# jmackey-astro/PION

Hardware: AMD Instinct MI355X
Metric: Mcell-updates/s on 3D ideal-MHD 512³ uniform grid; achieved HBM GB/s vs peak (higher is better)
Workload: dtype f64; 1 GPU; M1: 3-D GLM-MHD (nvar 9) Stone blast wave 512^3, HLLD + FKJ98 eta 0.1, periodic, OA2/OA2; nvar=9, decomposition=z-slab x1, transport=none; time loop and transport issued from C++ (libpion_host), fp_mode=fast (FMA contraction)

## Files before the change

include/pion_gpu.h:

```cpp
#ifndef PION_GPU_H
#define PION_GPU_H

#ifdef __cplusplus
extern "C" {
#endif

#define PION_MAX_NVAR 16
#define PION_MAX_DIM 3

#define PION_EQEUL 1
#define PION_EQMHD 2
#define PION_EQGLM 3

#define PION_FLUX_LF 0
#define PION_FLUX_RSlinear 1
#define PION_FLUX_RSexact 2
#define PION_FLUX_RShybrid 3
#define PION_FLUX_RSroe 4
#define PION_FLUX_RSroe_pv 5
#define PION_FLUX_FVS 6
#define PION_FLUX_RS_HLLD 7
#define PION_FLUX_RS_HLL 8

#define PION_AV_NONE 0
#define PION_AV_FKJ98_1D 1
#define PION_AV_HCORRECTION 3
#define PION_AV_HCORR_FKJ98 4

#define PION_BC_PERIODIC 1
#define PION_BC_OUTFLOW 2
#define PION_BC_INFLOW 3
#define PION_BC_REFLECTING 4
#define PION_BC_FIXED 5
#define PION_BC_ONEWAY_OUT 6
#define PION_BC_DMACH 7
#define PION_BC_DMACH2 8
#define PION_BC_STWIND 9
#define PION_BC_SLAB 10
#define PION_BC_JET 11
#define PION_BC_JETREFLECT 13
#define PION_BC_AXISYMMETRIC 12

#define PION_COOL_NONE 0
#define PION_COOL_WSS09_CIE_LINE_HEAT_COOL 8

#define PION_CELL_ISGD 1
#define PION_CELL_ISBD 2
#define PION_CELL_ISDOMAIN 4
#define PION_CELL_TIMESTEP 8
#define PION_CELL_ISLEAF 16

#define PION_GPU_OK 0
#define PION_GPU_EINVAL (-1)
#define PION_GPU_EDEVICE (-2)
#define PION_GPU_EPHYSICS (-3)
#define PION_GPU_ENOMEM (-4)

typedef struct pion_gpu_config {
  int ndim;
  int nvar;
  int ntracer;
  int eqntype;
  int solver;
  int artvisc;
  int sp_ooa;
  int tm_ooa;
  int coord_sys;
  int nbc;
  int ng[PION_MAX_DIM];
  double xmin[PION_MAX_DIM];
  double dx;
  double gamma;
  double cfl;
  double etav;
  double min_temp;
  double max_temp;
  double refvec[PION_MAX_NVAR];
  int bc_type[6];
  int bc_dmach2;
  int cooling;
  int mp_timestep_limit;
  int strict_fp;
} pion_gpu_config;


int pion_gpu_create(const pion_gpu_config *cfg, int device, void **handle);
void pion_gpu_destroy(void *handle);
int pion_gpu_last_error(void *handle, char *buf, int len);

long pion_gpu_ncell_all(void *handle);
int pion_gpu_ng_all(void *handle, int axis);


int pion_gpu_upload(void *handle, const double *P_soa);
int pion_gpu_download(void *handle, int which, double *P_soa);
int pion_gpu_bind_device_state(void *handle, void *dP, void *dPh);
void *pion_gpu_device_ptr(void *handle, int which);
int pion_gpu_set_stream(void *handle, void *stream);
int pion_gpu_set_comm_stream(void *handle, void *stream);
void *pion_gpu_get_stream(void *handle, int which);
int pion_gpu_synchronize(void *handle);

int pion_gpu_set_wind_cells(void *handle, long n, const long *idx, const double *states);

#define PION_MAX_WIND_SOURCES 8
typedef struct pion_gpu_wind_source {
  double pos[PION_MAX_DIM];
  double radius;
  int type;
  double mdot;
  double vinf, vrot;
  double Tw, Rstar, Bstar;
  double tracers[PION_MAX_NVAR];
  int npt;
  const double *evo_time, *evo_Teff, *evo_Mdot, *evo_vrot, *evo_vinf, *evo_R;
  const double *evo_X[7];
  int evo_tracer_elem[PION_MAX_NVAR];
  double t_now;
  double update_freq;
  double orbit_ecc_fac;
  double orbit_periastron[2];
  double orbit_period;
} pion_gpu_wind_source;

int pion_gpu_add_wind_source(void *handle, const pion_gpu_wind_source *src, int *id);
int pion_gpu_get_wind_source_pos(void *handle, int id, double *pos);
int pion_gpu_get_flags(void *handle, unsigned char *out);
int pion_gpu_wind_orbit_position(const pion_gpu_wind_source *src, int ndim, double simtime, double *pos);
int pion_gpu_add_rotating_wind_source(void *handle, const pion_gpu_wind_source *src, const double *evo_vcrit,
                                      double xi, int *id);
int pion_gpu_wind_angle_tables(double xi, double *theta, double *omega, double *Teff, double *delta, double *alpha);
int pion_gpu_get_wind_cells(void *handle, int id, long *n, long *idx, double *states);

int pion_gpu_set_jet(void *handle, int jetradius, const double *jetstate);

int pion_gpu_set_cooling_tables(void *handle, int nT, const double *T,
                                const double *tabs, const double *slopes);


int pion_gpu_update_bcs(void *handle, double simtime, int cstep, int maxstep, int assign);

int pion_gpu_calc_dt(void *handle, double *t_dyn, double *t_mp);
int pion_gpu_calc_dt_device(void *handle, void **dptr);
int pion_gpu_read_dt(void *handle, double *t_dyn, double *t_mp);
int pion_gpu_dt_request(void *handle);
int pion_gpu_dt_wait(void *handle, double *t_dyn, double *t_mp);

int pion_gpu_set_glm_speeds(void *handle, double dt, double dx, double cr);

int pion_gpu_stage(void *handle, double dt_stage, int space_ooa, int is_full_step);

#define PION_STAGE_WHOLE 0
#define PION_STAGE_INTERIOR 1
#define PION_STAGE_ZBOUNDARY 2
int pion_gpu_stage_part(void *handle, double dt_stage, int space_ooa, int is_full_step, int part);

int pion_gpu_advance_time(void *handle, double dt, double simtime);


long pion_gpu_halo_count(void *handle);
typedef struct {
  double *send_lo, *send_hi, *recv_lo, *recv_hi;
  long count_per_var, var_stride;
  int nvar;
} pion_gpu_halo_spans_t;
int pion_gpu_halo_spans(void *handle, int which, pion_gpu_halo_spans_t *out);
int pion_gpu_halo_begin(void *handle);
int pion_gpu_halo_end(void *handle);
int pion_gpu_pack_halo(void *handle, int which, int face, void *dbuf);
int pion_gpu_unpack_halo(void *handle, int which, int face, void *dbuf);


int pion_gpu_interface_flux(void *handle, int n, int axis, double dt, const double *Pl,
                            const double *Pr, const double *aux, double *F, double *Pstar);

int pion_gpu_cooling_update(void *handle, int n, double dt, const double *P_in, double *P_out);
int pion_gpu_cooling_edot(void *handle, int n, const double *rho, const double *T, double *edot);
int pion_gpu_cooling_timescale(void *handle, int n, const double *P_in, double *t_cool);

int pion_gpu_enable_timing(void *handle, int on);
int pion_gpu_get_timing(void *handle, double *out, int n);

#ifdef __cplusplus
}
#endif
#endif
```

pion_amd/csrc/kernels.h:

```cpp
#ifndef PION_KERNELS_H
#define PION_KERNELS_H

#include <hip/hip_runtime.h>
#include <stdint.h>

#include "dev_riemann.h"
#include "rows_tiling.h"

namespace pion {

#define PION_MAX_NTR 2
#define PION_COOL_NT_MAX 256

struct GridDesc {
  int ndim;
  int ng[3], nbc[3], nga[3];
  long ncell;
  long sy, sz;
  double dx;
  double xmin[3];
  int cyl;
  const double *sph_vol;
};

struct CoolDev {
  int NT;
  const double *T;
  const double *tab;
  const double *slope;
  double inv_Mu2, inv_Mu2_elec_H, Mu_tot_over_kB;
  double MinT_allowed, MaxT_allowed;
  float lg0, inv_dlg;
};

struct StageArgs {
  GridDesc g;
  const double *S;
  const double *Pc;
  double *out;
  const uint8_t *flags;
  const uint8_t *hllflag;
  const double *eta;
  int *errword;
  FluxCtx fc;
  int eqntype, ntracer, solver;
  int space_ooa;
  int cooling;
  double dt;
  double glm_damp;
  double max_temp;
  int use_march;
  int xwrap;
  int zslope_lds;
  double *dE;
  int zchunk;
  int nzb, zcmax;
  int rows;
  int rows_auto;
  int ncu;
  int kz0, kz1;
  int kz2, kz3;
  unsigned long long *dtres;
  double cfl;
  int dt_mp;
  int plain_cells;
  CoolDev cool;
};

struct PrepassArgs {
  GridDesc g;
  const double *S;
  uint8_t *hllflag;
  double *divv, *gradp;
  double *eta;
  int eqntype, nvar, space_ooa;
  double gamma;
  long c0, c1;
  long c2, c3;
};

struct DtArgs {
  GridDesc g;
  const double *P;
  const double *Ph;
  const uint8_t *flags;
  unsigned long long *result;
  int *errword;
  int eqntype, nvar;
  double gamma, cfl;
  int do_mp;
  CoolDev cool;
};

struct FluxTestArgs {
  int n, axis, eqntype, ntracer, solver;
  const double *Pl, *Pr, *aux;
  double *F, *Pstar;
  int *errword;
  FluxCtx fc;
};

struct CoolTestArgs {
  int n, nvar;
  double dt, gamma;
  const double *Pin;
  double *Pout;
  const double *rho, *T;
  double *edot;
  int *errword;
  CoolDev cool;
};

#define PION_DECLARE_FP(NS)                                        \
  namespace NS {                                                   \
  int launch_stage(const StageArgs &a, hipStream_t s);             \
  int launch_cooling_dE(const StageArgs &a, hipStream_t s);        \
  int launch_prepass(const PrepassArgs &a, hipStream_t s);         \
  int launch_dt(const DtArgs &a, hipStream_t s);                   \
  int launch_dt_mp(const DtArgs &a, hipStream_t s);                \
  int launch_flux_test(const FluxTestArgs &a, hipStream_t s);      \
  int launch_cool_update(const CoolTestArgs &a, hipStream_t s);    \
  int launch_cool_edot(const CoolTestArgs &a, hipStream_t s);      \
  int launch_cool_timescale(const CoolTestArgs &a, hipStream_t s); \
  const char *stage_kernel_name(int eq, int ntr, int solver);      \
  }

PION_DECLARE_FP(fp_strict)
PION_DECLARE_FP(fp_fast)

}
#endif
```

pion_amd/csrc/kernels_fp.hip:

```cpp
#include "dev_cooling.h"
#include "kernels.h"

#ifndef PION_FPNS
#error "PION_FPNS must be defined (fp_strict or fp_fast)"
#endif
#ifndef PION_EQSEL
#define PION_EQSEL 0
#endif

namespace pion {
namespace PION_FPNS {

template <bool MHD>
PDEV int rotvar(const int ax, const int s)
{
  if (s >= 2 && s <= 4) {
    int k = (s - 2) + ax;
    return 2 + (k >= 3 ? k - 3 : k);
  }
  if (MHD && s >= 5 && s <= 7) {
    int k = (s - 5) + ax;
    return 5 + (k >= 3 ? k - 3 : k);
  }
  return s;
// ... 510 lines not shown
#ifdef PION_FAST_MATH
    const double ro = a.Pc[qRO * nc + c], pg = a.Pc[qPG * nc + c];
    const double pnew = Cooling::time_update(cool, ro, pg, a.dt, g, err);
    dE = (pnew - pg) / (g - 1.0);
#else
    double P0[NV], pn[NV], ui[NV], uf[NV];
#pragma unroll
    for (int v = 0; v < NV; v++) pn[v] = P0[v] = a.Pc[v * nc + c];
    pn[qPG] = Cooling::time_update(cool, P0[qRO], P0[qPG], a.dt, g, err);
    E::PtoU(P0, ui, g);
    E::PtoU(pn, uf, g);
    dE = uf[uERG] - ui[uERG];
#endif
    if (err) atomicOr(a.errword, err);
  }
  a.dE[c] = dE;
}
template <int EQ, int NTR>
static int cooling_go(const StageArgs &a, hipStream_t s)
{
  const unsigned gx = (a.g.ng[0] + 63) / 64, gy = (a.g.ng[1] + 3) / 4;
  const unsigned np = (unsigned)(a.kz1 - a.kz0) + ((a.kz3 > a.kz2) ? (unsigned)(a.kz3 - a.kz2) : 0u);
  const unsigned ntile = gx * gy * np;
  hipLaunchKernelGGL((k_cooling_dE<EQ, NTR>), dim3(((ntile + 7) / 8) * 8), dim3(256), 0, s, a);
  return (int)hipGetLastError();
}

template <int EQ, int NTR, int SOLVER>
static int stage_go(const StageArgs &a, hipStream_t s)
{
  if (a.use_march != 0 && ((a.g.ndim == 3 && a.g.nbc[2] >= 2) || (a.g.ndim == 2 && a.g.cyl != 2 && a.g.nbc[1] >= 2)))
    return stage_rows2_go<EQ, NTR, SOLVER>(a, s);
  const int nbx = (a.g.ng[0] + 63) / 64, nby = (a.g.ng[1] + 3) / 4;
  const long ntiles = (long)nbx * nby * a.g.ng[2];
  const long nblocks = ((ntiles + 7) / 8) * 8;
  hipLaunchKernelGGL((k_stage<EQ, NTR, SOLVER>), dim3((unsigned)nblocks), dim3(256), 0, s, a);
  return (int)hipGetLastError();
}
template <int EQ, int NTR, int SOLVER>
static int flux_go(const FluxTestArgs &a, hipStream_t s)
{
  hipLaunchKernelGGL((k_flux_test<EQ, NTR, SOLVER>), dim3((a.n + 255) / 256), dim3(256), 0, s, a);
  return (int)hipGetLastError();
}

#define PION_SOLVER_CASES_HD(FN, EQ, NTR, A, S)          \
  switch (A.solver) {                                    \
    case 0: return FN<EQ, NTR, 0>(A, S);                 \
    case 1: return FN<EQ, NTR, 1>(A, S);                 \
    case 2: return FN<EQ, NTR, 2>(A, S);                 \
    case 3: return FN<EQ, NTR, 3>(A, S);                 \
    case 4: return FN<EQ, NTR, 4>(A, S);                 \
    case 5: return FN<EQ, NTR, 5>(A, S);                 \
    case 6: return FN<EQ, NTR, 6>(A, S);                 \
    case 8: return FN<EQ, NTR, 8>(A, S);                 \
    default: return -1;                                  \
  }
#define PION_SOLVER_CASES_MHD(FN, EQ, NTR, A, S)         \
  switch (A.solver) {                                    \
    case 0: return FN<EQ, NTR, 0>(A, S);                 \
    case 1: return FN<EQ, NTR, 1>(A, S);                 \
    case 4: return FN<EQ, NTR, 4>(A, S);                 \
    case 7: return FN<EQ, NTR, 7>(A, S);                 \
    case 8: return FN<EQ, NTR, 8>(A, S);                 \
    default: return -1;                                  \
  }

#if PION_EQSEL == 1
#define PION_EQ EQEUL
#define PION_CASES PION_SOLVER_CASES_HD
#define PION_SUFFIX hd
#elif PION_EQSEL == 2
#define PION_EQ EQMHD
#define PION_CASES PION_SOLVER_CASES_MHD
#define PION_SUFFIX mhd
#else
#define PION_EQ EQGLM
#define PION_CASES PION_SOLVER_CASES_MHD
#define PION_SUFFIX glm
#endif
#define PION_CAT2(a, b) a##b
#define PION_CAT(a, b) PION_CAT2(a, b)

#ifdef PION_PROBE
int PION_CAT(launch_stage_, PION_SUFFIX)(const StageArgs &a, hipStream_t s)
{
  return stage_rows2_go<PION_EQ, 0, (PION_EQSEL == 1 ? 4 : 7)>(a, s);
}
#else
int PION_CAT(launch_stage_, PION_SUFFIX)(const StageArgs &a, hipStream_t s)
{
  switch (a.ntracer) {
    case 0: PION_CASES(stage_go, PION_EQ, 0, a, s)
    case 1: PION_CASES(stage_go, PION_EQ, 1, a, s)
    case 2: PION_CASES(stage_go, PION_EQ, 2, a, s)
    default: return -1;
  }
}
int PION_CAT(launch_cooling_dE_, PION_SUFFIX)(const StageArgs &a, hipStream_t s)
{
  switch (a.ntracer) {
    case 0: return cooling_go<PION_EQ, 0>(a, s);
    case 1: return cooling_go<PION_EQ, 1>(a, s);
    case 2: return cooling_go<PION_EQ, 2>(a, s);
    default: return -1;
  }
}
int PION_CAT(launch_flux_test_, PION_SUFFIX)(const FluxTestArgs &a, hipStream_t s)
{
  switch (a.ntracer) {
    case 0: PION_CASES(flux_go, PION_EQ, 0, a, s)
    case 1: PION_CASES(flux_go, PION_EQ, 1, a, s)
    case 2: PION_CASES(flux_go, PION_EQ, 2, a, s)
    default: return -1;
  }
}
#endif

#else

int launch_stage_hd(const StageArgs &a, hipStream_t s);
int launch_stage_mhd(const StageArgs &a, hipStream_t s);
int launch_stage_glm(const StageArgs &a, hipStream_t s);
int launch_cooling_dE_hd(const StageArgs &a, hipStream_t s);
int launch_cooling_dE_mhd(const StageArgs &a, hipStream_t s);
int launch_cooling_dE_glm(const StageArgs &a, hipStream_t s);
int launch_flux_test_hd(const FluxTestArgs &a, hipStream_t s);
int launch_flux_test_mhd(const FluxTestArgs &a, hipStream_t s);
int launch_flux_test_glm(const FluxTestArgs &a, hipStream_t s);

int launch_stage(const StageArgs &a, hipStream_t s)
{
  if (a.eqntype == EQEUL) return launch_stage_hd(a, s);
  if (a.eqntype == EQMHD) return launch_stage_mhd(a, s);
  if (a.eqntype == EQGLM) return launch_stage_glm(a, s);
  return -1;
}
int launch_cooling_dE(const StageArgs &a, hipStream_t s)
{
  if (a.eqntype == EQEUL) return launch_cooling_dE_hd(a, s);
  if (a.eqntype == EQMHD) return launch_cooling_dE_mhd(a, s);
  if (a.eqntype == EQGLM) return launch_cooling_dE_glm(a, s);
  return -1;
}
int launch_flux_test(const FluxTestArgs &a, hipStream_t s)
{
  if (a.eqntype == EQEUL) return launch_flux_test_hd(a, s);
  if (a.eqntype == EQMHD) return launch_flux_test_mhd(a, s);
  if (a.eqntype == EQGLM) return launch_flux_test_glm(a, s);
  return -1;
}
const char *stage_kernel_name(int, int, int) { return "k_stage"; }

__global__ __launch_bounds__(256) void k_prepass_hlld(const PrepassArgs a)
{
  const long nc = a.g.ncell;
  const unsigned gx = (a.g.nga[0] + 63) / 64, gy = (a.g.nga[1] + 3) / 4;
  const long plane = (long)a.g.nga[0] * a.g.nga[1];
  const unsigned npl1 = (unsigned)((a.c1 - a.c0) / plane);
  const unsigned npl = npl1 + ((a.c3 > a.c2) ? (unsigned)((a.c3 - a.c2) / plane) : 0u);
  const unsigned ntile = gx * gy * npl;
  const unsigned t = (unsigned)xcd_tile(blockIdx.x, ntile);
  if (t >= ntile) return;
  int i[3];
  i[0] = (int)((t % gx) * 64 + (threadIdx.x & 63));
  i[1] = (int)(((t / gx) % gy) * 4 + (threadIdx.x >> 6));
  const unsigned pz = t / (gx * gy);
  i[2] = (pz < npl1) ? (int)(a.c0 / plane) + (int)pz : (int)(a.c2 / plane) + (int)(pz - npl1);
  if (i[0] >= a.g.nga[0] || i[1] >= a.g.nga[1]) return;
  const long c = (long)i[0] + a.g.sy * i[1] + a.g.sz * i[2];
  const double dx = a.g.dx;
  double divv = 0.0, gradp = 0.0;
  double pp3[3], pn3[3];
  bool steep = (a.gradp != nullptr);
  for (int v = 0; v < a.g.ndim; v++) {
    const long st = (v == 0) ? 1 : ((v == 1) ? a.g.sy : a.g.sz);
    const long n = (i[v] > 0) ? c - st : c;
    const long p = (i[v] < a.g.nga[v] - 1) ? c + st : c;
    pp3[v] = a.S[1 * nc + p];
    pn3[v] = a.S[1 * nc + n];
    if (!(fabs(pp3[v] - pn3[v]) <= 1.6 * fmin(pp3[v], pn3[v]))) steep = true;
  }
  if (steep) {
    for (int v = 0; v < a.g.ndim; v++) gradp += fabs(pp3[v] - pn3[v]) / fmin(pp3[v], pn3[v]);
  }
  if (gradp > 5. || a.divv) {
    for (int v = 0; v < a.g.ndim; v++) {
      const long st = (v == 0) ? 1 : ((v == 1) ? a.g.sy : a.g.sz);
      const long n = (i[v] > 0) ? c - st : c;
      const long p = (i[v] < a.g.nga[v] - 1) ? c + st : c;
      const double ddx = (n == c || p == c) ? dx : 2.0 * dx;
      if (a.g.cyl == 1 && v == 1) {
        const double rn = cyl_Rcom(cyl_R(a.g, (n == c) ? i[1] : i[1] - 1), dx);
        const double rp = cyl_Rcom(cyl_R(a.g, (p == c) ? i[1] : i[1] + 1), dx);
        divv += 2.0 * (rp * a.S[(2 + v) * nc + p] - rn * a.S[(2 + v) * nc + n]) / (rp * rp - rn * rn);
      }
      else divv += (a.S[(2 + v) * nc + p] - a.S[(2 + v) * nc + n]) / ddx;
    }
  }
  if (a.divv) a.divv[c] = divv;
  if (a.gradp) a.gradp[c] = gradp;
  a.hllflag[c] = (divv < 0. && gradp > 5.) ? 1 : 0;
}

#define PION_PREPASS_ZC 16
__global__ __launch_bounds__(256) void k_prepass_hlld_march(const PrepassArgs a)
{
  const long nc = a.g.ncell;
  const unsigned gx = (a.g.nga[0] + 61) / 62, gy = (a.g.nga[1] + 3) / 4;
  const long plane = (long)a.g.nga[0] * a.g.nga[1];
  const int kz0 = (int)(a.c0 / plane), kz1 = (int)(a.c1 / plane);
  const unsigned nch = (unsigned)((kz1 - kz0 + PION_PREPASS_ZC - 1) / PION_PREPASS_ZC);
  const unsigned ntile = gx * gy * nch;
  const unsigned t = (unsigned)xcd_tile(blockIdx.x, ntile);
  if (t >= ntile) return;
  const int lane = (int)(threadIdx.x & 63);
  int ix = (int)((t % gx) * 62) - 1 + lane;
  const bool xwriter = (lane >= 1 && lane <= 62 && ix < a.g.nga[0]);
  if (ix < 0) ix = 0;
  if (ix > a.g.nga[0] - 1) ix = a.g.nga[0] - 1;
  const int iy = (int)(((t / gx) % gy) * 4 + (threadIdx.x >> 6));
  const int k0 = kz0 + (int)(t / (gx * gy)) * PION_PREPASS_ZC;
  const int k1 = (k0 + PION_PREPASS_ZC < kz1) ? k0 + PION_PREPASS_ZC : kz1;
  if (iy >= a.g.nga[1]) return;
  const long sy = a.g.sy, sz = a.g.sz;
  const double dx = a.g.dx;
  const double *P = a.S + 1 * nc;
  const bool xl = ix > 0, xh = ix < a.g.nga[0] - 1, yl = iy > 0, yh = iy < a.g.nga[1] - 1;
  const unsigned cb = (unsigned)((long)ix + sy * iy);
  const unsigned o0 = cb * 8u;
  const unsigned oym = yl ? o0 - (unsigned)sy * 8u : o0, oyp = yh ? o0 + (unsigned)sy * 8u : o0;
  const char *Pk = reinterpret_cast<const char *>(P) + sz * 8 * k0;
  char *Hk = reinterpret_cast<char *>(a.hllflag) + sz * k0;
  double p0 = ldu(Pk, o0), pm = (k0 > 0) ? ldu(Pk - sz * 8, o0) : p0;
  for (int k = k0; k < k1; k++, Pk += sz * 8, Hk += sz) {
    const bool zl = k > 0, zh = k < a.g.nga[2] - 1;
    const unsigned q0 = pin_v(o0), qym = pin_v(oym), qyp = pin_v(oyp);
    const double pz = zh ? ldu(Pk + sz * 8, q0) : p0;
    double pn3[3], pp3[3];
    const double pl_ = lane_prev(p0), pr_ = lane_next(p0);
    pn3[0] = xl ? pl_ : p0;
    pp3[0] = xh ? pr_ : p0;
    pn3[1] = ldu(Pk, qym);
    pp3[1] = ldu(Pk, qyp);
    pn3[2] = zl ? pm : p0;
    pp3[2] = pz;
    bool steep = false;
#pragma unroll
    for (int v = 0; v < 3; v++) {
      const double d = fabs(pp3[v] - pn3[v]);
      if (!(d <= 1.6 * pp3[v]) || !(d <= 1.6 * pn3[v])) steep = true;
    }
    uint8_t flag = 0;
    if (steep) {
      double gradp = 0.0, divv = 0.0;
      for (int v = 0; v < 3; v++) gradp += fabs(pp3[v] - pn3[v]) / fmin(pp3[v], pn3[v]);
      if (gradp > 5.) {
        const long c = (long)cb + sz * ((long)k + opaque_zero());
        const bool lo[3] = {xl, yl, zl}, hi[3] = {xh, yh, zh};
        for (int v = 0; v < 3; v++) {
          const long st = (v == 0) ? 1 : ((v == 1) ? sy : sz);
          const long n = lo[v] ? c - st : c, p = hi[v] ? c + st : c;
          const double ddx = (n == c || p == c) ? dx : 2.0 * dx;
          divv += (a.S[(2 + v) * nc + p] - a.S[(2 + v) * nc + n]) / ddx;
        }
        flag = (divv < 0.) ? 1 : 0;
      }
    }
    if (xwriter) stub(Hk, pin_v(cb), flag);
    pm = p0;
    p0 = pz;
  }
}

template <int NVMAX>
__global__ __launch_bounds__(256) void k_prepass_hcorr(const PrepassArgs a)
{
  const long c = a.c0 + (long)blockIdx.x * blockDim.x + threadIdx.x;
  const long nc = a.g.ncell;
  if (c >= a.c1) return;
  int i[3];
  i[0] = (int)(c % a.g.nga[0]);
  i[1] = (int)((c / a.g.nga[0]) % a.g.nga[1]);
  i[2] = (int)(c / ((long)a.g.nga[0] * a.g.nga[1]));
  const double dx = a.g.dx, g = a.gamma;
  const bool mhd = (a.eqntype != EQEUL);
  const bool oa2 = (a.space_ooa == 2);
  for (int ax = 0; ax < a.g.ndim; ax++) {
    const long st = (ax == 0) ? 1 : ((ax == 1) ? a.g.sy : a.g.sz);
    const int n = a.g.nga[ax], k = i[ax];
    double eta = 0.0;
    if (k < n - 1) {
      double eL[8], eR[8];
      const int nvs = mhd ? 8 : 5;
      for (int s = 0; s < 8; s++) {
        if (s >= nvs) {
          eL[s] = eR[s] = 0.0;
          continue;
        }
        const double *b = a.S + (long)(mhd ? rotvar<true>(ax, s) : rotvar<false>(ax, s)) * nc + c;
        const double q0 = b[0], q1 = b[st];
        double s0 = 0.0, s1 = 0.0;
        if (oa2 && a.g.cyl == 2) {
          const double R0 = sph_R(a.g, k), R1 = sph_R(a.g, k + 1);
          const double c0 = sph_Rcom(R0, dx), c1 = sph_Rcom(R1, dx);
          if (k > 0) s0 = avg_falle((q0 - b[-st]) / (c0 - sph_Rcom(sph_R(a.g, k - 1), dx)), (q1 - q0) / (c1 - c0));
          if (k + 1 < n - 1) s1 = avg_falle((q1 - q0) / (c1 - c0), (b[2 * st] - q1) / (sph_Rcom(sph_R(a.g, k + 2), dx) - c1));
          eL[s] = q0 + s0 * (R0 + 0.5 * dx - c0);
          eR[s] = q1 + s1 * (R1 - 0.5 * dx - c1);
        }
        else if (oa2 && a.g.cyl == 1 && ax == 1) {
          const double R0 = cyl_R(a.g, k), R1 = cyl_R(a.g, k + 1);
          const double c0 = cyl_Rcom(R0, dx), c1 = cyl_Rcom(R1, dx);
          if (k > 0) s0 = avg_falle((q0 - b[-st]) / (c0 - cyl_Rcom(cyl_R(a.g, k - 1), dx)), (q1 - q0) / (c1 - c0));
          if (k + 1 < n - 1) s1 = avg_falle((q1 - q0) / (c1 - c0), (b[2 * st] - q1) / (cyl_Rcom(cyl_R(a.g, k + 2), dx) - c1));
          eL[s] = q0 + s0 * (R0 + dx * 0.5 - c0);
          eR[s] = q1 + s1 * (R1 - dx * 0.5 - c1);
        }
        else if (oa2) {
          if (k > 0) s0 = avg_falle((q0 - b[-st]) / dx, (q1 - q0) / dx);
          if (k + 1 < n - 1) s1 = avg_falle((q1 - q0) / dx, (b[2 * st] - q1) / dx);
          eL[s] = q0 + s0 * dx * 0.5;
          eR[s] = q1 - s1 * dx * 0.5;
        }
        else {
          eL[s] = q0;
          eR[s] = q1;
        }
      }
      double msL, msR;
      if (mhd) {
        msL = Eqn<EQMHD, 0>::cfast(eL, g);
        msR = Eqn<EQMHD, 0>::cfast(eR, g);
      }
      else {
        msL = Eqn<EQEUL, 0>::chydro(eL, g);
        msR = Eqn<EQEUL, 0>::chydro(eR, g);
      }
      eta = 0.5 * (fabs(eR[qVN] - eL[qVN]) + fabs(msR - msL));
    }
    a.eta[ax * nc + c] = eta;
  }
}

int launch_prepass(const PrepassArgs &a, hipStream_t s)
{
  const unsigned nb = (unsigned)((a.c1 - a.c0 + 255) / 256);
  if (a.hllflag) {
    const long plane = (long)a.g.nga[0] * a.g.nga[1];
    const unsigned npl = (unsigned)((a.c1 - a.c0) / plane) + ((a.c3 > a.c2) ? (unsigned)((a.c3 - a.c2) / plane) : 0u);
    const unsigned ntile = (unsigned)((a.g.nga[0] + 63) / 64) * ((a.g.nga[1] + 3) / 4) * npl;
    if (a.g.ndim == 3 && a.g.cyl == 0 && !a.divv && !a.gradp && a.c3 <= a.c2 && npl >= PION_PREPASS_ZC
        && a.g.ncell * 8L < (1L << 32)) {
      const unsigned nch = (npl + PION_PREPASS_ZC - 1) / PION_PREPASS_ZC;
      const unsigned nt = (unsigned)((a.g.nga[0] + 61) / 62) * ((a.g.nga[1] + 3) / 4) * nch;
      hipLaunchKernelGGL(k_prepass_hlld_march, dim3(((nt + 7) / 8) * 8), dim3(256), 0, s, a);
    }
    else hipLaunchKernelGGL(k_prepass_hlld, dim3(((ntile + 7) / 8) * 8), dim3(256), 0, s, a);
  }
  if (a.eta) hipLaunchKernelGGL((k_prepass_hcorr<8>), dim3(nb), dim3(256), 0, s, a);
  return (int)hipGetLastError();
}

PDEV double wave_min(double v)
{
#pragma unroll
  for (int off = 32; off > 0; off >>= 1) {
    const double o = __shfl_xor(v, off, 64);
    v = (o < v) ? o : v;
  }
  return v;
}

__global__ __launch_bounds__(256) void k_dt(const DtArgs a)
{
  const long nc = a.g.ncell;
  const long non = (long)a.g.ng[0] * a.g.ng[1] * a.g.ng[2];
  double tdyn = 1.e100, tmp = 1.0e99;
  int err = 0;
  const bool mhd = (a.eqntype != EQEUL);
  const double g = a.gamma;
  for (long k = (long)blockIdx.x * blockDim.x + threadIdx.x; k < non; k += (long)gridDim.x * blockDim.x) {
    const int ix = (int)(k % a.g.ng[0]), iy = (int)((k / a.g.ng[0]) % a.g.ng[1]),
              iz = (int)(k / ((long)a.g.ng[0] * a.g.ng[1]));
    const long c = (long)(ix + a.g.nbc[0]) + a.g.sy * (iy + a.g.nbc[1]) + a.g.sz * (iz + a.g.nbc[2]);
    const uint8_t fl = a.flags[c];
    if ((fl & 8 ) && !(fl & 2 )) {
      double p[8];
      const int nvs = mhd ? 8 : 5;
      for (int v = 0; v < 8; v++) p[v] = (v < nvs) ? a.P[v * nc + c] : 0.0;
      const double t = mhd ? cell_dt<EQMHD>(p, a.g.ndim, g, a.g.dx, a.cfl) : cell_dt<EQEUL>(p, a.g.ndim, g, a.g.dx, a.cfl);
      if (!(t > 0.0)) err |= ERR_BAD_DT;
      tdyn = (t < tdyn) ? t : tdyn;
    }
    if (a.do_mp && !(fl & 2) && (fl & 16)) {
      const double t = Cooling::timescale(a.cool, a.Ph[0 * nc + c], a.Ph[1 * nc + c], g);
      tmp = (t < tmp) ? t : tmp;
    }
  }
  tdyn = wave_min(tdyn);
  tmp = wave_min(tmp);
  if ((threadIdx.x & 63) == 0) {
    atomicMin(&a.result[0], (unsigned long long)__double_as_longlong(tdyn));
    atomicMin(&a.result[1], (unsigned long long)__double_as_longlong(tmp));
  }
  if (err) atomicOr(a.errword, err);
}

__global__ __launch_bounds__(256) void k_dt_mp(const DtArgs a)
{
  __shared__ double ctab[11 * PION_COOL_NT_MAX];
  const int NT = a.cool.NT;
  for (int i = threadIdx.x; i < NT; i += 256) ctab[i] = a.cool.T[i];
  for (int i = threadIdx.x; i < 5 * NT; i += 256) {
    ctab[NT + i] = a.cool.tab[i];
    ctab[6 * NT + i] = a.cool.slope[i];
  }
  __syncthreads();
  CoolDev cool = a.cool;
  cool.T = ctab;
  cool.tab = ctab + NT;
  cool.slope = ctab + 6 * NT;
  const long nc = a.g.ncell;
  const long non = (long)a.g.ng[0] * a.g.ng[1] * a.g.ng[2];
  double tmp = 1.0e99;
  for (long k = (long)blockIdx.x * blockDim.x + threadIdx.x; k < non; k += (long)gridDim.x * blockDim.x) {
    const int ix = (int)(k % a.g.ng[0]), iy = (int)((k / a.g.ng[0]) % a.g.ng[1]),
              iz = (int)(k / ((long)a.g.ng[0] * a.g.ng[1]));
    const long c = (long)(ix + a.g.nbc[0]) + a.g.sy * (iy + a.g.nbc[1]) + a.g.sz * (iz + a.g.nbc[2]);
    const uint8_t fl = a.flags[c];
    if (!(fl & 2) && (fl & 16)) {
      const double t = Cooling::timescale(cool, a.Ph[0 * nc + c], a.Ph[1 * nc + c], a.gamma);
      tmp = (t < tmp) ? t : tmp;
    }
  }
  tmp = wave_min(tmp);
  if ((threadIdx.x & 63) == 0) atomicMin(&a.result[1], (unsigned long long)__double_as_longlong(tmp));
}
int launch_dt_mp(const DtArgs &a, hipStream_t s)
{
  const long non = (long)a.g.ng[0] * a.g.ng[1] * a.g.ng[2];
  long nb = (non + 255) / 256;
  if (nb > 2048) nb = 2048;
  hipLaunchKernelGGL(k_dt_mp, dim3((unsigned)nb), dim3(256), 0, s, a);
  return (int)hipGetLastError();
}

int launch_dt(const DtArgs &a, hipStream_t s)
{
  const long non = (long)a.g.ng[0] * a.g.ng[1] * a.g.ng[2];
  long nb = (non + 255) / 256;
  if (nb > 2048) nb = 2048;
  hipLaunchKernelGGL(k_dt, dim3((unsigned)nb), dim3(256), 0, s, a);
  return (int)hipGetLastError();
}

__global__ void k_cool_update(const CoolTestArgs a)
{
  const int i = blockIdx.x * blockDim.x + threadIdx.x;
  if (i >= a.n) return;
  int err = 0;
  const double *p = a.Pin + (long)i * a.nvar;
  double *o = a.Pout + (long)i * a.nvar;
  for (int v = 0; v < a.nvar; v++) o[v] = p[v];
  o[1] = Cooling::time_update(a.cool, p[0], p[1], a.dt, a.gamma, err);
  if (err) atomicOr(a.errword, err);
}
__global__ void k_cool_edot(const CoolTestArgs a)
{
  const int i = blockIdx.x * blockDim.x + threadIdx.x;
  if (i >= a.n) return;
  a.edot[i] = Cooling::edot(a.cool, a.rho[i], a.T[i]);
}
__global__ void k_cool_timescale(const CoolTestArgs a)
{
  const int i = blockIdx.x * blockDim.x + threadIdx.x;
  if (i >= a.n) return;
  const double *p = a.Pin + (long)i * a.nvar;
  a.edot[i] = Cooling::timescale(a.cool, p[0], p[1], a.gamma);
}
int launch_cool_timescale(const CoolTestArgs &a, hipStream_t s)
{
  hipLaunchKernelGGL(k_cool_timescale, dim3((a.n + 255) / 256), dim3(256), 0, s, a);
  return (int)hipGetLastError();
}
int launch_cool_update(const CoolTestArgs &a, hipStream_t s)
{
  hipLaunchKernelGGL(k_cool_update, dim3((a.n + 255) / 256), dim3(256), 0, s, a);
  return (int)hipGetLastError();
}
int launch_cool_edot(const CoolTestArgs &a, hipStream_t s)
{
  hipLaunchKernelGGL(k_cool_edot, dim3((a.n + 255) / 256), dim3(256), 0, s, a);
  return (int)hipGetLastError();
}
#endif

}
}
```

pion_amd/csrc/pion_gpu.hip:

```cpp
#include <hip/hip_runtime.h>

#include <cmath>
#include <cstdio>
#include <cstdlib>
#include <cstring>
#include <string>
#include <vector>

#include <hipcub/hipcub.hpp>

#include "../../include/pion_gpu.h"
#include "dev_wind.h"
#include "kernels.h"

using namespace pion;

namespace {

struct BCArgs {
  GridDesc g;
  double *T;
  int nvar, dir, type, eqntype, ntracer;
  double refval[PION_MAX_NVAR];
  double dmr_a0, dmr_t3;
// ... 274 lines not shown
    case PION_BC_INFLOW:
    case PION_BC_FIXED:
      for (int v = 0; v < a.nvar; v++) T[v * nc + c] = a.refval[v];
      break;
    case PION_BC_DMACH: {
      const double x = a.g.xmin[0] + (2 * i[0] + 1) * (0.5 * a.g.dx);
      const double y = a.g.xmin[1] + (2 * i[1] + 1) * (0.5 * a.g.dx);
      const double bpos = a.dmr_a0 + 1.0 / 6.0 + y / a.dmr_t3;
      if (x <= bpos) {
        T[0 * nc + c] = 8.0;
        T[1 * nc + c] = 116.5;
        T[2 * nc + c] = 7.14470958;
        T[3 * nc + c] = -4.125;
        T[4 * nc + c] = 0.0;
        for (int v = a.nvar - a.ntracer; v < a.nvar; v++) T[v * nc + c] = 1.0;
      }
      else {
        for (int v = 0; v < a.nvar; v++) T[v * nc + c] = a.refval[v];
      }
      break;
    }
    default:
      break;
  }
}

__global__ void k_bc_dmr2(const BCArgs a, const int ncols)
{
  const int t = blockIdx.x * blockDim.x + threadIdx.x;
  const int nb = a.g.nbc[1];
  if (t >= ncols * nb) return;
  const int ix = t % ncols, iy = -1 - (t / ncols);
  const long nc = a.g.ncell;
  const long c = (long)(ix + a.g.nbc[0]) + a.g.sy * (iy + a.g.nbc[1]);
  for (int v = 0; v < a.nvar; v++) a.T[v * nc + c] = a.refval[v];
}

__global__ void k_wind(double *T, const long *idx, const double *states, const long n, const int nvar,
                       const long nc)
{
  const long t = (long)blockIdx.x * blockDim.x + threadIdx.x;
  if (t >= n) return;
  const long c = idx[t];
  for (int v = 0; v < nvar; v++) T[v * nc + c] = states[t * nvar + v];
}

__global__ void k_halo(double *A, double *buf, const GridDesc g, const int nvar, const int face, const int pack)
{
  const long plane = (long)g.nga[0] * g.nga[1];
  const long per = plane * g.nbc[2];
  const long t = (long)blockIdx.x * blockDim.x + threadIdx.x;
  if (t >= per * nvar) return;
  const int v = (int)(t / per);
  const long r = t % per;
  const int k = (int)(r / plane);
  const long xy = r % plane;
  int izall;
  if (pack) izall = (face == 4) ? g.nbc[2] + k : g.ng[2] + k;
  else izall = (face == 4) ? k : g.nbc[2] + g.ng[2] + k;
  const long c = xy + plane * izall;
  if (pack) buf[t] = A[v * g.ncell + c];
  else A[v * g.ncell + c] = buf[t];
}

struct AngleTables {
  double xi = 0.0;
  double theta[PION_ANGLE_NTHETA], omega[PION_ANGLE_NOMEGA], Teff[PION_ANGLE_NTEFF];
  std::vector<double> delta;
  std::vector<double> alpha;
};

struct WindSource {
  int type = 0;
  double pos[3] = {0.0, 0.0, 0.0};
  double radius = 0.0, Bstar = 0.0;
  std::vector<double> t, Teff, Mdot, vrot, vinf, R, X[7];
  std::vector<double> vcrit;
  int elem[PION_MAX_NVAR];
  double Mdot_c = 0.0, Vinf_c = 0.0, vrot_c = 0.0, Tw_c = 0.0, Rstar_c = 0.0;
  double vcrit_c = 0.0;
  double tr[PION_MAX_NVAR];
  bool active = true;
  double tstart = 0.0, tfinish = 0.0, t_next_update = 1.0e99;
  long off = 0, n = 0;
  bool moving = false;
  pion_gpu_wind_source orbit;
  int box_w[3] = {1, 1, 1};
  long *dn = nullptr;
  void *dscan = nullptr;
  size_t scan_bytes = 0;
};

struct Handle {
  pion_gpu_config cfg;
  GridDesc g;
  int device = 0;
  int ncu = 0;
  hipStream_t stream = 0;
  hipStream_t comm_stream = 0;
  hipEvent_t ev_packed_src = nullptr, ev_unpacked = nullptr;
  hipStream_t bstream = 0;
  hipEvent_t ev_pre = nullptr, ev_bdone = nullptr;
  bool ev_pre_valid = false;
  bool concurrent_strips = true;
  bool ev_unpacked_valid = false;
  double *dP = nullptr, *dPh = nullptr;
  bool own_state = true;
  uint8_t *dflags = nullptr, *dhll = nullptr;
  double *deta = nullptr;
  double *dsphvol = nullptr;
  int *derr = nullptr;
  unsigned long long *ddt = nullptr;
  unsigned long long *ddt_init = nullptr;
  double *hdt = nullptr;
  hipEvent_t ev_dt = nullptr;
  bool dt_requested = false;
  std::vector<uint8_t> hflags;
  double refval[6][PION_MAX_NVAR];
  int dmr2_cols = 0;
  long nwind = 0;
  long njet = 0;
  long *djet_idx = nullptr;
  double *djet_state = nullptr;
  long *dwind_idx = nullptr;
  double *dwind_state = nullptr;
  std::vector<WindSource> wsrc;
  long nws = 0;
  long *dws_idx = nullptr;
  double *dws_dist = nullptr, *dws_off = nullptr, *dws_state = nullptr;
  double *dws_theta = nullptr;
  bool have_angle = false;
  AngleTables angle;
  CoolDev cool;
  double *dcoolT = nullptr, *dcooltab = nullptr, *dcoolslope = nullptr;
  bool have_tables = false;
  double glm_chyp = 0.0, glm_cr = 0.0;
  double refvec_avg[PION_MAX_NVAR];
  bool ph_valid = false;
  bool dt_cached = false;
  std::string err;
  bool timing = false;
  std::vector<hipEvent_t> ev[4];
  double Mu_tot_over_kB = 0.0;
  int use_march = 3, zchunk = 0, rows = 0;
  int rows1 = 0;
  const double *xghost_fresh = nullptr;
  int zslope_lds = 1;
  double *ddE = nullptr;
  bool fuse_dt = true;
  bool uneven_chunks = true;
  bool dt_mp_pending = false;
  bool split_dt_mp = true;
  bool fuse_bc = true;
};

#define HCHECK(h, call)                                                            \
  do {                                                                             \
    hipError_t e_ = (call);                                                        \
    if (e_ != hipSuccess) {                                                        \
      (h)->err = std::string(#call) + ": " + hipGetErrorString(e_);                \
      return PION_GPU_EDEVICE;                                                     \
    }                                                                              \
  } while (0)

static inline Handle *use(void *handle)
{
  Handle *h = (Handle *)handle;
  if (h) (void)hipSetDevice(h->device);
  return h;
}

int order_after_unpack(Handle *h)
{
  if (h->comm_stream && h->comm_stream != h->stream && h->ev_unpacked_valid) {
    HCHECK(h, hipStreamWaitEvent(h->stream, h->ev_unpacked, 0));
    h->ev_unpacked_valid = false;
  }
  return 0;
}

long cell_id(const GridDesc &g, int ix, int iy, int iz)
{
  return (long)(ix + g.nbc[0]) + g.sy * (iy + g.nbc[1]) + g.sz * (iz + g.nbc[2]);
}

void time_begin(Handle *h, int slot)
{
  if (!h->timing) return;
  hipEvent_t e;
  hipEventCreate(&e);
  hipEventRecord(e, h->stream);
  h->ev[slot].push_back(e);
}
void time_end(Handle *h, int slot) { time_begin(h, slot); }

FluxCtx make_fluxctx(const Handle *h, double fv_dt)
{
  FluxCtx fc;
  fc.gamma = h->cfg.gamma;
  fc.dx = h->cfg.dx;
  fc.fv_dt = fv_dt;
  fc.etav = h->cfg.etav;
  fc.chyp = h->glm_chyp;
  fc.min_temp = h->cfg.min_temp;
  fc.refRO = h->refvec_avg[0];
  fc.refPG = h->refvec_avg[1];
  fc.refV = h->refvec_avg[2];
  fc.refB = h->refvec_avg[5];
  fc.gndim = h->cfg.ndim;
  fc.artvisc = h->cfg.artvisc;
  fc.mp.present = (h->cfg.cooling != 0);
  fc.mp.Mu_tot_over_kB = h->Mu_tot_over_kB;
  return fc;
}

int check_errword(Handle *h)
{
  int e = 0;
  HCHECK(h, hipMemcpyAsync(&e, h->derr, sizeof(int), hipMemcpyDeviceToHost, h->stream));
  HCHECK(h, hipStreamSynchronize(h->stream));
  if (e) {
    char b[400];
    snprintf(b, sizeof b, "device physics error word 0x%x:%s%s%s%s%s", e,
             (e & ERR_NEG_DENSITY) ? " negative density (reference: rep.error -> exit)" : "",
             (e & ERR_RIEMANN_INPUT) ? " density/pressure too small in Riemann solver" : "",
             (e & ERR_COOLING) ? " cooling integration failed" : "", (e & ERR_BAD_DT) ? " invalid cell timestep" : "",
             (e & ERR_MHD_RIEMANN) ? " linear MHD Riemann solver: bad wave speeds (reference: rep.error -> exit)" : "");
    h->err = b;
    int z = 0;
    hipMemcpyAsync(h->derr, &z, sizeof(int), hipMemcpyHostToDevice, h->stream);
    return PION_GPU_EPHYSICS;
  }
  return 0;
}

static inline bool mp_dt_limited(const pion_gpu_config &cfg)
{
  return cfg.cooling != 0 && cfg.mp_timestep_limit >= 1 && cfg.mp_timestep_limit <= 3;
}

static inline bool any_wind(const Handle *h) { return h->nwind > 0 || h->nws > 0; }

static bool equalD(const double a, const double b)
{
  if (a == b) return true;
  if (fabs(a) + fabs(b) < 1.0e-100) return true;
  return (fabs(a - b) / (fabs(a) + fabs(b) + 1.0e-100)) < 1.0e-12;
}

static double root_find_linear_vec(const std::vector<double> &xarr, const std::vector<double> &yarr, const double xreq)
{
  const size_t len = xarr.size();
  size_t ihi = len - 1, ilo = 0, imid = 0;
  do {
    imid = ilo + (size_t)floor((ihi - ilo) / 2.0);
    if (xarr[imid] < xreq) ilo = imid;
    else ihi = imid;
  } while (ihi - ilo > 1);
  double xval = 0.0;
  if (xreq > xarr[ihi]) xval = xarr[ihi];
  else if (xreq < xarr[ilo]) xval = xarr[ilo];
  else xval = xreq;
  return yarr[ilo] + (yarr[ihi] - yarr[ilo]) * (xval - xarr[ilo]) / (xarr[ihi] - xarr[ilo]);
}

static int wind_lists_grow(Handle *h, const long n)
{
  const long o = h->nws, ntot = o + n;
  const int nvar = h->cfg.nvar;
  long *nidx = nullptr;
  double *ndist = nullptr, *noff = nullptr, *nstate = nullptr, *ntheta = nullptr;
  if (ntot > 0) {
    HCHECK(h, hipMalloc(&nidx, sizeof(long) * ntot));
    HCHECK(h, hipMalloc(&ndist, sizeof(double) * ntot));
    HCHECK(h, hipMalloc(&ntheta, sizeof(double) * ntot));
    HCHECK(h, hipMemsetAsync(ntheta, 0, sizeof(double) * ntot, h->stream));
    HCHECK(h, hipMalloc(&noff, sizeof(double) * 3 * ntot));
    HCHECK(h, hipMalloc(&nstate, sizeof(double) * ntot * nvar));
    HCHECK(h, hipMemsetAsync(nstate, 0, sizeof(double) * ntot * nvar, h->stream));
  }
  if (o > 0) {
    HCHECK(h, hipMemcpyAsync(nidx, h->dws_idx, sizeof(long) * o, hipMemcpyDeviceToDevice, h->stream));
    HCHECK(h, hipMemcpyAsync(ndist, h->dws_dist, sizeof(double) * o, hipMemcpyDeviceToDevice, h->stream));
    HCHECK(h, hipMemcpyAsync(ntheta, h->dws_theta, sizeof(double) * o, hipMemcpyDeviceToDevice, h->stream));
    for (int a = 0; a < 3; a++)
      HCHECK(h, hipMemcpyAsync(noff + a * ntot, h->dws_off + a * o, sizeof(double) * o, hipMemcpyDeviceToDevice,
                               h->stream));
    HCHECK(h, hipMemcpyAsync(nstate, h->dws_state, sizeof(double) * o * nvar, hipMemcpyDeviceToDevice, h->stream));
  }
  HCHECK(h, hipStreamSynchronize(h->stream));
  hipFree(h->dws_idx);
  hipFree(h->dws_dist);
  hipFree(h->dws_off);
  hipFree(h->dws_state);
  hipFree(h->dws_theta);
  h->dws_idx = nidx;
  h->dws_theta = ntheta;
  h->dws_dist = ndist;
  h->dws_off = noff;
  h->dws_state = nstate;
  h->nws = ntot;
  return 0;
}

static void wind_orbit_position(const pion_gpu_wind_source &s, const int ndim, const double simtime, double *pos)
{
#pragma clang fp contract(off)
// ... 89 lines not shown

static void setup_tables(const double xi, AngleTables &T)
{
#pragma clang fp contract(off)
  T.xi = xi;
  const int nth = PION_ANGLE_NTHETA, nom = PION_ANGLE_NOMEGA, nT = PION_ANGLE_NTEFF;
  const double theta_min = 0.1, theta_mid = 60.0, theta_max = 89.9;
  for (int k = 0; k < nth; k++) {
    if (k <= 4) T.theta[k] = (theta_min + k * ((theta_mid - theta_min) / 4.0)) * (pi / 180.0);
    else T.theta[k] = (theta_mid + (k - 4) * ((theta_max - theta_mid) / (nth - 5))) * (pi / 180.0);
  }
  double log_mu[PION_ANGLE_NOMEGA];
  for (int i = 0; i < nom; i++) log_mu[nom - i - 1] = -4.0 + i * (4.0 / (nom - 1));
  for (int j = 0; j < nom; j++) T.omega[j] = 1 - pow_fast(10, log_mu[j]);
  const double T0 = 1000.0, T1 = 3600.0, T2 = 6000.0, T3 = 8000.0, T4 = 10000.0, T5 = 20000.0, T6 = 22000.0,
               T7 = 150000.0;
  for (int i = 0; i < nT; i++) {
    if (i == 0) T.Teff[i] = T0;
    if (i == 1) T.Teff[i] = T1;
    if (2 <= i && i <= 6) T.Teff[i] = T1 + i * ((T2 - T1) / 6);
    if (i == 7) T.Teff[i] = T2;
    if (8 <= i && i <= 10) T.Teff[i] = T2 + (i - 6) * ((T3 - T2) / 4);
    if (i == 11) T.Teff[i] = T3;
    if (12 <= i && i <= 14) T.Teff[i] = T3 + (i - 10) * ((T4 - T3) / 4);
    if (i == 15) T.Teff[i] = T4;
    if (i == 16) T.Teff[i] = T5;
    if (17 <= i && i <= 19) T.Teff[i] = T5 + (i - 15) * ((T6 - T5) / 4);
    if (i == 20) T.Teff[i] = T6;
    if (i == 21) T.Teff[i] = T7;
  }
  T.delta.assign((size_t)nom * nT, 0.0);
  for (int i = 0; i < nom; i++)
    for (int j = 0; j < nT; j++) T.delta[(size_t)i * nT + j] = fn_delta(T.omega[i], T.Teff[j], xi);
  T.alpha.assign((size_t)nom * nth * nT, 0.0);
  for (int i = 0; i < nom; i++)
    for (int j = 0; j < nth; j++)
      for (int k = 0; k < nT; k++) T.alpha[((size_t)i * nth + j) * nT + k] = fn_alpha(T.omega[i], T.theta[j], T.Teff[k]);
}

static double delta_interp(const AngleTables &T, const double xr, const double yr)
{
#pragma clang fp contract(off)
  const double *x = T.omega, *y = T.Teff;
  size_t ihi = PION_ANGLE_NOMEGA - 1, jhi = PION_ANGLE_NTEFF - 1, ilo = 0, jlo = 0, imid = 0, jmid = 0;
  do {
    imid = ilo + (size_t)floor((ihi - ilo) / 2.0);
    if (x[imid] < xr) ilo = imid;
    else ihi = imid;
  } while (ihi - ilo > 1);
  do {
    jmid = jlo + (size_t)floor((jhi - jlo) / 2.0);
    if (y[jmid] < yr) jlo = jmid;
    else jhi = jmid;
  } while (jhi - jlo > 1);
  double xval, yval;
  if (xr > x[ihi]) xval = x[ihi];
  else if (xr < x[ilo]) xval = x[ilo];
  else xval = xr;
  if (yr > y[jhi]) yval = y[jhi];
  else if (yr < y[jlo]) yval = y[jlo];
  else yval = yr;
  const size_t nT = PION_ANGLE_NTEFF;
  const std::vector<double> &f = T.delta;
  double result = (f[ilo * nT + jlo] * (x[ihi] - xval) * (y[jhi] - yval) + f[ihi * nT + jlo] * (xval - x[ilo]) * (y[jhi] - yval) +
                   f[ilo * nT + jhi] * (x[ihi] - xval) * (yval - y[jlo]) + f[ihi * nT + jhi] * (xval - x[ilo]) * (yval - y[jlo]));
  result /= ((x[ihi] - x[ilo]) * (y[jhi] - y[jlo]));
  return result;
}
}

static WindBox wind_box(const Handle *h, const WindSource &W, const double *pos)
{
  const GridDesc &g = h->g;
  WindBox b;
  b.n = 1;
  for (int a = 0; a < 3; a++) {
    b.w[a] = W.box_w[a];
    b.lo[a] = 0;
    if (a < g.ndim && b.w[a] < g.nga[a]) {
      double t = (pos[a] - W.radius - g.xmin[a]) / g.dx - 0.5 + g.nbc[a];
      if (!(t == t)) t = 0.0;
      t = std::min(std::max(t, -2.0 * g.nga[a]), 2.0 * g.nga[a]);
      b.lo[a] = (int)floor(t) - 1;
    }
    b.n *= b.w[a];
  }
  return b;
}

static WindMember wind_member(const Handle *h, const WindSource &W)
{
  WindMember m;
  m.g = h->g;
  for (int a = 0; a < 3; a++) m.pos[a] = W.pos[a];
  m.radius = W.radius;
  return m;
}

typedef hipcub::TransformInputIterator<long, WindBoxCell, hipcub::CountingInputIterator<long>> WindBoxIter;

static int wind_add_cells_box(Handle *h, const WindSource &W)
{
  const WindMember m = wind_member(h, W);
  WindBoxCell bc;
  bc.g = h->g;
  bc.b = wind_box(h, W, W.pos);
  WindBoxMember pred;
  pred.m = m;
  WindBoxIter cells(hipcub::CountingInputIterator<long>(0), bc);
  size_t bytes = W.scan_bytes;
  HCHECK(h, hipcub::DeviceSelect::If(W.dscan, bytes, cells, h->dws_idx + W.off, W.dn, (int)W.n, pred, h->stream));
  hipLaunchKernelGGL(k_wind_cells_dn, dim3((unsigned)((W.n + 255) / 256)), dim3(256), 0, h->stream, m,
                     h->dws_idx + W.off, W.dn, h->dws_dist + W.off, h->dws_off + W.off, h->nws, h->dflags);
  return 0;
}

static int add_moving_wind_source(Handle *h, WindSource &W, int *id)
{
  const GridDesc &g = h->g;
  long cap = 1;
  for (int a = 0; a < 3; a++) {
    W.box_w[a] = 1;
    if (a < g.ndim) {
      const double w = floor(2.0 * W.radius / g.dx) + 5.0;
      W.box_w[a] = (w >= (double)g.nga[a]) ? g.nga[a] : (int)w;
    }
    cap *= W.box_w[a];
  }
  if (cap > 0x7fffffffL) {
    h->err = "wind source: the orbit box is too large";
    return PION_GPU_EINVAL;
  }
  if (int rc = wind_lists_grow(h, cap)) return rc;
  W.off = h->nws - cap;
  W.n = cap;
  HCHECK(h, hipMalloc(&W.dn, sizeof(long)));
  HCHECK(h, hipMemsetAsync(W.dn, 0, sizeof(long), h->stream));
  {
    WindBoxCell bc;
    bc.g = g;
    bc.b = wind_box(h, W, W.pos);
    WindBoxMember pred;
    pred.m = wind_member(h, W);
    WindBoxIter cells(hipcub::CountingInputIterator<long>(0), bc);
    W.scan_bytes = 0;
    HCHECK(h, hipcub::DeviceSelect::If(nullptr, W.scan_bytes, cells, h->dws_idx + W.off, W.dn, (int)cap, pred,
                                       h->stream));
    HCHECK(h, hipMalloc(&W.dscan, W.scan_bytes > 0 ? W.scan_bytes : 1));
  }
  h->wsrc.push_back(W);
  if (int rc = wind_add_cells_box(h, h->wsrc.back())) return rc;
  HCHECK(h, hipGetLastError());
  HCHECK(h, hipStreamSynchronize(h->stream));
  h->dt_cached = false;
  if (id) *id = (int)h->wsrc.size() - 1;
  return 0;
}

static int wind_sources_move(Handle *h, const double simtime)
{
  bool moved = false;
  for (size_t s = 0; s < h->wsrc.size(); s++) {
    WindSource &W = h->wsrc[s];
    if (!W.moving) continue;
    const WindBox ob = wind_box(h, W, W.pos);
    hipLaunchKernelGGL(k_wind_unflag, dim3((unsigned)((ob.n + 255) / 256)), dim3(256), 0, h->stream,
                       wind_member(h, W), ob, h->dflags);
    double np[3];
    wind_orbit_position(W.orbit, h->cfg.ndim, simtime, np);
    for (int a = 0; a < 3; a++) {
      moved = moved || !(np[a] == W.pos[a]);
      W.pos[a] = np[a];
    }
    if (int rc = wind_add_cells_box(h, W)) return rc;
  }
  if (moved) h->dt_cached = false;
  return 0;
}

static double angle_omega(const double vrot, const double vcrit)
{
  const double r = vrot / vcrit;
  const double o = (r < 0.9999) ? r : 0.9999;
  return (0.999 < o) ? 0.999 : o;
}

static bool angle_values_at(const Handle *h, const WindSource &W, const double simtime, double *Tw, double *omega)
{
  const bool due = simtime >= W.t_next_update;
  if (!(W.active || due)) return false;
  double tw = W.Tw_c, vrot = W.vrot_c, vcrit = W.vcrit_c;
  if (due) {
    const double T = root_find_linear_vec(W.t, W.Teff, simtime), Tmax = h->angle.Teff[PION_ANGLE_NTEFF - 1];
    tw = (Tmax < T) ? Tmax : T;
    vrot = root_find_linear_vec(W.t, W.vrot, simtime);
    vcrit = root_find_linear_vec(W.t, W.vcrit, simtime);
  }
  *Tw = tw;
  *omega = angle_omega(vrot, vcrit);
  return true;
}

static int wind_angle_check(Handle *h, const double simtime)
{
  for (size_t s = 0; s < h->wsrc.size(); s++) {
    const WindSource &W = h->wsrc[s];
    double Tw, omega;
    if (W.type != 2 || !angle_values_at(h, W, simtime, &Tw, &omega)) continue;
    if (!(omega > h->angle.omega[0]) || !(Tw > h->angle.Teff[0])) {
      h->err = "rotating wind source: omega <= 0 or Tw <= 1000 K (stellar_wind_angle look-up out of range)";
      return PION_GPU_EINVAL;
    }
  }
  return 0;
}

static void wind_angle_launch(Handle *h, const WindSource &W, const WindStateArgs &a)
{
#pragma clang fp contract(off)
  const AngleTables &T = h->angle;
  WindAngleArgs g;
  memset(&g, 0, sizeof g);
  g.P = a.P;
  g.Ph = a.Ph;
  g.states = a.states;
  g.idx = a.idx;
  g.dist = a.dist;
  g.off = a.off;
  g.theta = h->dws_theta;
  g.ntot = a.ntot;
  g.ncell = a.ncell;
  g.nvar = a.nvar;
  g.ntracer = a.ntracer;
  g.ndim = a.ndim;
  g.eqntype = a.eqntype;
  g.cooling = a.cooling;
  g.Tmin = a.Tmin;
  g.Mu_tot_over_kB = a.Mu_tot_over_kB;
  WindAngleDev &d = g.s;
  d.Mdot = W.Mdot_c;
  d.Vinf = W.Vinf_c;
  d.v_rot = W.vrot_c;
  d.Tw = W.Tw_c;
  d.Rstar = W.Rstar_c;
  d.Bstar = W.Bstar;
  d.radius = W.radius;
  d.xi = T.xi;
  const double om = angle_omega(W.vrot_c, W.vcrit_c), Tw = W.Tw_c;
  d.omega = om;
  d.delta = lgm99::delta_interp(T, om, Tw);
  int xi = 0, zi = 0;
  while (xi < PION_ANGLE_NOMEGA - 1 && om > T.omega[xi]) xi++;
  while (zi < PION_ANGLE_NTEFF - 1 && Tw > T.Teff[zi]) zi++;
  xi = std::max(xi, 1);
  zi = std::max(zi, 1);
  d.dx = (om - T.omega[xi - 1]) / (T.omega[xi] - T.omega[xi - 1]);
  d.dz = (Tw - T.Teff[zi - 1]) / (T.Teff[zi] - T.Teff[zi - 1]);
  const int nth = PION_ANGLE_NTHETA, nT = PION_ANGLE_NTEFF;
  for (int j = 0; j < nth; j++) {
    d.theta[j] = T.theta[j];
    d.a[0][j] = T.alpha[((size_t)(xi - 1) * nth + j) * nT + zi - 1];
    d.a[1][j] = T.alpha[((size_t)(xi - 1) * nth + j) * nT + zi];
    d.a[2][j] = T.alpha[((size_t)xi * nth + j) * nT + zi - 1];
    d.a[3][j] = T.alpha[((size_t)xi * nth + j) * nT + zi];
  }
  for (int v = 0; v < PION_MAX_NTR; v++) d.tr[v] = (v < h->cfg.ntracer) ? W.tr[v] : 0.0;
  d.off = W.off;
  d.n = W.n;
  hipLaunchKernelGGL(k_wind_state_angle, dim3((unsigned)((W.n + 255) / 256)), dim3(256), 0, h->stream, g);
}

int wind_sources_update(Handle *h, const double simtime)
{
  if (int rc = wind_sources_move(h, simtime)) return rc;
  WindStateArgs a;
  memset(&a, 0, sizeof a);
  for (size_t s = 0; s < h->wsrc.size(); s++) {
    WindSource &W = h->wsrc[s];
    if ((W.type == 1 || W.type == 2) && simtime >= W.t_next_update) {
      W.active = true;
      W.t_next_update = std::min(simtime, W.tfinish);
      W.Tw_c = root_find_linear_vec(W.t, W.Teff, simtime);
      W.Mdot_c = root_find_linear_vec(W.t, W.Mdot, simtime);
      W.vrot_c = root_find_linear_vec(W.t, W.vrot, simtime);
      W.Vinf_c = root_find_linear_vec(W.t, W.vinf, simtime);
      W.Rstar_c = root_find_linear_vec(W.t, W.R, simtime);
      for (int v = 0; v < h->cfg.ntracer; v++)
        if (W.elem[v] >= 0) W.tr[v] = root_find_linear_vec(W.t, W.X[W.elem[v]], simtime);
      if (W.type == 2) {
        const double Tmax = h->angle.Teff[PION_ANGLE_NTEFF - 1];
        W.Tw_c = (Tmax < W.Tw_c) ? Tmax : W.Tw_c;
        W.vcrit_c = root_find_linear_vec(W.t, W.vcrit, simtime);
      }
    }
    WindSrcDev &d = a.s[s];
    d.Mdot = W.Mdot_c;
    d.Vinf = W.Vinf_c;
    d.v_rot = W.vrot_c;
    d.Tw = W.Tw_c;
    d.Rstar = W.Rstar_c;
    d.Bstar = W.Bstar;
    d.radius = W.radius;
    for (int v = 0; v < PION_MAX_NTR; v++) d.tr[v] = (v < h->cfg.ntracer) ? W.tr[v] : 0.0;
    d.off = W.off;
    d.n = W.n;
    d.dn = W.moving ? W.dn : nullptr;
    d.active = W.active ? 1 : 0;
  }
  a.P = h->dP;
  a.Ph = h->dPh;
  a.states = h->dws_state;
  a.idx = h->dws_idx;
  a.dist = h->dws_dist;
  a.off = h->dws_off;
  a.ntot = h->nws;
  a.ncell = h->g.ncell;
  a.nsrc = (int)h->wsrc.size();
  a.nvar = h->cfg.nvar;
  a.ntracer = h->cfg.ntracer;
  a.ndim = h->cfg.ndim;
  a.cart2d = (h->cfg.ndim == 2 && h->cfg.coord_sys == 1) ? 1 : 0;
  a.eqntype = h->cfg.eqntype;
  a.cooling = (h->cfg.cooling != 0) ? 1 : 0;
  a.Tmin = h->cfg.min_temp;
  a.Mu_tot_over_kB = h->Mu_tot_over_kB;
  for (int s = 0; s < a.nsrc; s++) {
    if (!(a.s[s].active && a.s[s].n > 0)) continue;
    if (h->wsrc[s].type == 2) wind_angle_launch(h, h->wsrc[s], a);
    else hipLaunchKernelGGL(k_wind_state, dim3((unsigned)((a.s[s].n + 255) / 256)), dim3(256), 0, h->stream, a, s);
  }
  return 0;
}

static int add_fixed_wind_source(Handle *h, WindSource &W, int *id)
{
  const GridDesc &g = h->g;
  const WindMember m = wind_member(h, W);
  unsigned long long *dcount = nullptr;
  HCHECK(h, hipMalloc(&dcount, sizeof(unsigned long long)));
  HCHECK(h, hipMemsetAsync(dcount, 0, sizeof(unsigned long long), h->stream));
  hipLaunchKernelGGL(k_wind_count, dim3((unsigned)((g.ncell + 255) / 256)), dim3(256), 0, h->stream, m, dcount);
  unsigned long long cnt = 0;
  HCHECK(h, hipMemcpyAsync(&cnt, dcount, sizeof cnt, hipMemcpyDeviceToHost, h->stream));
  HCHECK(h, hipStreamSynchronize(h->stream));
  hipFree(dcount);
  const long n = (long)cnt;
  if (int rc = wind_lists_grow(h, n)) return rc;
  const long o = h->nws - n, ntot = h->nws;
  if (n > 0) {
    hipcub::CountingInputIterator<long> cells(0);
    long *dsel = nullptr;
    HCHECK(h, hipMalloc(&dsel, sizeof(long)));
    size_t tmp_bytes = 0;
    HCHECK(h, hipcub::DeviceSelect::If(nullptr, tmp_bytes, cells, h->dws_idx + o, dsel, g.ncell, m, h->stream));
    void *tmp = nullptr;
    HCHECK(h, hipMalloc(&tmp, tmp_bytes));
    HCHECK(h, hipcub::DeviceSelect::If(tmp, tmp_bytes, cells, h->dws_idx + o, dsel, g.ncell, m, h->stream));
    long nsel = 0;
    HCHECK(h, hipMemcpyAsync(&nsel, dsel, sizeof nsel, hipMemcpyDeviceToHost, h->stream));
    HCHECK(h, hipStreamSynchronize(h->stream));
    hipFree(tmp);
    hipFree(dsel);
    if (nsel != n) {
      h->err = "wind source: membership count and compaction disagree";
      return PION_GPU_EDEVICE;
    }
    hipLaunchKernelGGL(k_wind_cells, dim3((unsigned)((n + 255) / 256)), dim3(256), 0, h->stream, m, h->dws_idx + o,
                       n, h->dws_dist + o, h->dws_off + o, h->dws_theta + o, ntot, h->dflags);
  }
  HCHECK(h, hipGetLastError());
  HCHECK(h, hipStreamSynchronize(h->stream));
  W.off = o;
  W.n = n;
  h->wsrc.push_back(W);
  h->dt_cached = false;
  if (id) *id = (int)h->wsrc.size() - 1;
  return 0;
}

struct DevBuf {
  double *p = nullptr;
  ~DevBuf()
  {
    if (p) (void)hipFree(p);
  }
};

}

extern "C" {

int pion_gpu_create(const pion_gpu_config *cfg, int device, void **handle)
{
  if (!cfg || !handle) return PION_GPU_EINVAL;
  if (cfg->ndim < 1 || cfg->ndim > 3 || cfg->nvar > PION_MAX_NVAR) return PION_GPU_EINVAL;
  if (!(cfg->coord_sys == 1 || (cfg->coord_sys == 2 && cfg->ndim == 2)
        || (cfg->coord_sys == 3 && cfg->ndim == 1 && cfg->eqntype == PION_EQEUL)))
    return PION_GPU_EINVAL;
  for (int d = 0; d < 2 * cfg->ndim; d++)
    if (cfg->bc_type[d] == PION_BC_AXISYMMETRIC && !(cfg->coord_sys == 2 && d == 2)) return PION_GPU_EINVAL;
  const int base = (cfg->eqntype == PION_EQEUL) ? 5 : (cfg->eqntype == PION_EQMHD ? 8 : (cfg->eqntype == PION_EQGLM ? 9 : -1));
  if (base < 0 || cfg->nvar != base + cfg->ntracer || cfg->ntracer > PION_MAX_NTR) return PION_GPU_EINVAL;
  if (cfg->sp_ooa == 2 && cfg->nbc < 2) return PION_GPU_EINVAL;
  if (cfg->nbc < 1) return PION_GPU_EINVAL;
  if (cfg->eqntype == PION_EQEUL) {
    if (cfg->solver == 7 || cfg->solver < 0 || cfg->solver > 8) return PION_GPU_EINVAL;
  }
  else if (!(cfg->solver == 0 || cfg->solver == 1 || cfg->solver == 4 || cfg->solver == 7 || cfg->solver == 8))
    return PION_GPU_EINVAL;
  if (cfg->cooling != 0 && cfg->cooling != PION_COOL_WSS09_CIE_LINE_HEAT_COOL) return PION_GPU_EINVAL;
  if (cfg->mp_timestep_limit < 0 || cfg->mp_timestep_limit > 4) return PION_GPU_EINVAL;

  Handle *h = new Handle;
  h->cfg = *cfg;
  if (const char *e = getenv("PION_STAGE_KERNEL"))
    h->use_march = (strcmp(e, "cell") == 0) ? 0 : 3;
  if (const char *e = getenv("PION_ZSLOPE_LDS")) h->zslope_lds = (atoi(e) != 0);
  if (const char *e = getenv("PION_CONCURRENT_STRIPS")) h->concurrent_strips = (atoi(e) != 0);
  if (const char *e = getenv("PION_FUSE_DT")) h->fuse_dt = (atoi(e) != 0);
  if (const char *e = getenv("PION_FUSE_BC")) h->fuse_bc = (atoi(e) != 0);
  if (const char *e = getenv("PION_UNEVEN_CHUNKS")) h->uneven_chunks = (atoi(e) != 0);
  if (const char *e = getenv("PION_SPLIT_DT_MP")) h->split_dt_mp = (atoi(e) != 0);
  if (const char *e = getenv("PION_ROWS")) h->rows = h->rows1 = (atoi(e) >= 1 && atoi(e) <= 64) ? atoi(e) : 0;
  if (const char *e = getenv("PION_ROWS1")) h->rows1 = (atoi(e) >= 1 && atoi(e) <= 8) ? atoi(e) : 0;
  if (const char *e = getenv("PION_ZCHUNK")) h->zchunk = atoi(e) > 0 ? atoi(e) : 0;
  h->device = device;
  if (hipSetDevice(device) != hipSuccess) {
    delete h;
    return PION_GPU_EDEVICE;
  }
  {
    int ncu = 0;
    if (hipDeviceGetAttribute(&ncu, hipDeviceAttributeMultiprocessorCount, device) == hipSuccess) h->ncu = ncu;
  }
  GridDesc &g = h->g;
  g.ndim = cfg->ndim;
  g.ncell = 1;
  for (int a = 0; a < 3; a++) {
    g.ng[a] = (a < cfg->ndim) ? cfg->ng[a] : 1;
    g.nbc[a] = (a < cfg->ndim) ? cfg->nbc : 0;
    g.nga[a] = g.ng[a] + 2 * g.nbc[a];
    g.ncell *= g.nga[a];
    g.xmin[a] = cfg->xmin[a];
  }
  g.sy = g.nga[0];
  g.sz = (long)g.nga[0] * g.nga[1];
  g.dx = cfg->dx;
  g.cyl = (cfg->coord_sys == 2) ? 1 : ((cfg->coord_sys == 3) ? 2 : 0);
  g.sph_vol = nullptr;
  *handle = h;
  const bool rows3d = (g.ndim == 3 && g.nbc[2] >= 2);
  bool rows2d = (g.ndim == 2 && g.cyl != 2 && g.nbc[1] >= 2 && g.nbc[0] >= 2);
  if (const char *e = getenv("PION_ROWS_2D")) rows2d = rows2d && (atoi(e) != 0);
  if (!((rows3d || rows2d) && (unsigned long long)g.ncell * 8ull < (1ull << 32))) h->use_march = 0;

  const size_t nb = sizeof(double) * (size_t)cfg->nvar * g.ncell;
  HCHECK(h, hipMalloc(&h->dP, nb));
  HCHECK(h, hipMalloc(&h->dPh, nb));
  HCHECK(h, hipMemset(h->dP, 0, nb));
  HCHECK(h, hipMemset(h->dPh, 0, nb));
  HCHECK(h, hipMalloc(&h->dflags, g.ncell));
  if (g.cyl == 2) {
    std::vector<double> vol(g.nga[0]);
    for (int i = 0; i < g.nga[0]; i++) {
      double rc = g.xmin[0] + (2 * (i - g.nbc[0]) + 1) * (0.5 * g.dx);
      const double rp = rc + 0.5 * g.dx;
      const double rn = rp - g.dx;
      vol[i] = (pow(rp, 3.0) - pow(rn, 3.0)) / 3.0;
    }
    HCHECK(h, hipMalloc(&h->dsphvol, sizeof(double) * vol.size()));
    HCHECK(h, hipMemcpy(h->dsphvol, vol.data(), sizeof(double) * vol.size(), hipMemcpyHostToDevice));
    g.sph_vol = h->dsphvol;
  }
  HCHECK(h, hipMalloc(&h->derr, 64));
  HCHECK(h, hipMemset(h->derr, 0, 64));
  HCHECK(h, hipMalloc(&h->ddt, 2 * sizeof(unsigned long long)));
  HCHECK(h, hipMalloc(&h->ddt_init, 2 * sizeof(unsigned long long)));
  {
    const double init[2] = {1.e100, 1.0e99};
    HCHECK(h, hipMemcpy(h->ddt_init, init, sizeof init, hipMemcpyHostToDevice));
  }
  if (cfg->eqntype != PION_EQEUL && cfg->solver == PION_FLUX_RS_HLLD) {
    HCHECK(h, hipMalloc(&h->dhll, g.ncell));
    HCHECK(h, hipMemset(h->dhll, 0, g.ncell));
  }
  if (cfg->cooling != 0) {
    HCHECK(h, hipMalloc(&h->ddE, sizeof(double) * g.ncell));
    HCHECK(h, hipMemset(h->ddE, 0, sizeof(double) * g.ncell));
  }
  if (cfg->artvisc == PION_AV_HCORRECTION || cfg->artvisc == PION_AV_HCORR_FKJ98) {
    HCHECK(h, hipMalloc(&h->deta, sizeof(double) * cfg->ndim * g.ncell));
    HCHECK(h, hipMemset(h->deta, 0, sizeof(double) * cfg->ndim * g.ncell));
  }

  h->hflags.assign(g.ncell, 0);
  for (long c = 0; c < g.ncell; c++) {
    int i[3];
    i[0] = (int)(c % g.nga[0]) - g.nbc[0];
    i[1] = (int)((c / g.nga[0]) % g.nga[1]) - g.nbc[1];
    i[2] = (int)(c / g.sz) - g.nbc[2];
    bool on = true;
    bool all_periodic_offgrid = true;
    for (int a = 0; a < cfg->ndim; a++) {
      if (i[a] < 0) {
        on = false;
        if (cfg->bc_type[2 * a] != PION_BC_PERIODIC) all_periodic_offgrid = false;
      }
      else if (i[a] >= g.ng[a]) {
        on = false;
        if (cfg->bc_type[2 * a + 1] != PION_BC_PERIODIC) all_periodic_offgrid = false;
      }
    }
    uint8_t f = PION_CELL_ISLEAF | PION_CELL_TIMESTEP;
    if (on) f |= PION_CELL_ISGD | PION_CELL_ISDOMAIN;
    else {
      f |= PION_CELL_ISBD;
      (void)all_periodic_offgrid;
    }
    h->hflags[c] = f;
  }
  HCHECK(h, hipMemcpy(h->dflags, h->hflags.data(), g.ncell, hipMemcpyHostToDevice));

  const double m_p = 1.672621898e-24, kB = 1.38064852e-16;
  const double Mu = 1.40 * m_p, Mu_tot = 0.609 * m_p, Mu_elec = 1.167 * m_p;
  h->Mu_tot_over_kB = Mu_tot / kB;
  memset(&h->cool, 0, sizeof h->cool);
  h->cool.inv_Mu2 = 1.0 / (Mu * Mu);
  h->cool.inv_Mu2_elec_H = 1.0 / (Mu_elec * Mu);
  h->cool.Mu_tot_over_kB = h->Mu_tot_over_kB;
  h->cool.MinT_allowed = cfg->min_temp;
  h->cool.MaxT_allowed = cfg->max_temp;
  if (h->cool.MinT_allowed < 1.0 || h->cool.MinT_allowed > 1.0e6) h->cool.MinT_allowed = 1.0;
  if (h->cool.MaxT_allowed < 1.0e2 || h->cool.MaxT_allowed > 3.0e10) h->cool.MaxT_allowed = 1.0e8;

  for (int v = 0; v < PION_MAX_NVAR; v++) h->refvec_avg[v] = cfg->refvec[v];
  if (cfg->eqntype == PION_EQEUL) {
    const double refvel = sqrt(cfg->gamma * cfg->refvec[1] / cfg->refvec[0]);
    h->refvec_avg[2] = h->refvec_avg[3] = h->refvec_avg[4] = 0.1 * refvel;
  }
  else {
    double *rv = h->refvec_avg;
    const double gam = cfg->gamma;
    auto cfast = [&](const double *p) {
      const double ch = sqrt(gam * p[1] / p[0]);
      const double t1 = ch * ch + (p[5] * p[5] + p[6] * p[6] + p[7] * p[7]) / p[0];
      double t2 = 4. * ch * ch * p[5] * p[5] / p[0];
      t2 = std::max(5.e-16, t1 * t1 - t2);
      return sqrt((t1 + sqrt(t2)) / 2.);
    };
    auto rotate_xy = [&](double *v, double theta) {
      const double ct = cos(theta), st = sin(theta);
      double a = v[2] * ct - v[3] * st, b = v[2] * st + v[3] * ct;
      v[2] = a;
      v[3] = b;
      a = v[5] * ct - v[6] * st;
      b = v[5] * st + v[6] * ct;
      v[5] = a;
      v[6] = b;
    };
    double angle = rv[6] * rv[6] + rv[5] * rv[5], refvel;
    if (angle > 10. * 5.e-16) {
      angle = M_PI / 2. - asin(rv[6] / sqrt(angle));
      if (rv[5] < 0) angle = -angle;
      rotate_xy(rv, angle);
      refvel = cfast(rv);
      rotate_xy(rv, -angle);
    }
    else refvel = cfast(rv);
    const double refB = sqrt(rv[5] * rv[5] + rv[6] * rv[6] + rv[7] * rv[7]);
    rv[2] = rv[3] = rv[4] = 0.1 * refvel;
    rv[5] = rv[6] = rv[7] = refB;
  }
  for (int d = 0; d < 6; d++)
    for (int v = 0; v < PION_MAX_NVAR; v++) h->refval[d][v] = 0.0;

  if (cfg->bc_dmach2) {
    int n = 0;
    for (int ix = 0; ix < g.ng[0]; ix++) {
      const double x = g.xmin[0] + (2 * ix + 1) * (0.5 * g.dx);
      if (x <= 1. / 6.) n++;
      else break;
    }
    h->dmr2_cols = n;
  }
  return PION_GPU_OK;
}

void pion_gpu_destroy(void *handle)
{
  Handle *h = use(handle);
  if (!h) return;
  hipSetDevice(h->device);
  hipDeviceSynchronize();
  if (h->own_state) {
    hipFree(h->dP);
    hipFree(h->dPh);
  }
  hipFree(h->dflags);
  hipFree(h->dhll);
  hipFree(h->ddE);
  if (h->bstream) hipStreamDestroy(h->bstream);
  if (h->ev_pre) hipEventDestroy(h->ev_pre);
  if (h->ev_bdone) hipEventDestroy(h->ev_bdone);
  if (h->hdt) hipHostFree(h->hdt);
  if (h->ev_dt) hipEventDestroy(h->ev_dt);
  hipFree(h->deta);
  hipFree(h->dsphvol);
  hipFree(h->derr);
  hipFree(h->ddt);
  hipFree(h->ddt_init);
  hipFree(h->dwind_idx);
  hipFree(h->dwind_state);
  hipFree(h->dws_idx);
  hipFree(h->dws_dist);
  hipFree(h->dws_off);
  hipFree(h->dws_state);
  hipFree(h->dws_theta);
  for (WindSource &W : h->wsrc) {
    hipFree(W.dn);
    hipFree(W.dscan);
  }
  hipFree(h->djet_idx);
  hipFree(h->djet_state);
  hipFree(h->dcoolT);
  hipFree(h->dcooltab);
  hipFree(h->dcoolslope);
  for (int s = 0; s < 4; s++)
    for (hipEvent_t e : h->ev[s]) hipEventDestroy(e);
  if (h->ev_packed_src) hipEventDestroy(h->ev_packed_src);
  if (h->ev_unpacked) hipEventDestroy(h->ev_unpacked);
  delete h;
}

int pion_gpu_last_error(void *handle, char *buf, int len)
{
  Handle *h = use(handle);
  if (!h || !buf || len <= 0) return PION_GPU_EINVAL;
  snprintf(buf, len, "%s", h->err.c_str());
  return 0;
}

long pion_gpu_ncell_all(void *handle) { return ((Handle *)handle)->g.ncell; }
int pion_gpu_ng_all(void *handle, int axis) { return ((Handle *)handle)->g.nga[axis]; }

int pion_gpu_upload(void *handle, const double *P_soa)
{
  Handle *h = use(handle);
  h->xghost_fresh = nullptr;
  const size_t nb = sizeof(double) * (size_t)h->cfg.nvar * h->g.ncell;
  HCHECK(h, hipMemcpyAsync(h->dP, P_soa, nb, hipMemcpyHostToDevice, h->stream));
  HCHECK(h, hipMemcpyAsync(h->dPh, h->dP, nb, hipMemcpyDeviceToDevice, h->stream));
  HCHECK(h, hipStreamSynchronize(h->stream));
  h->ph_valid = false;
  h->dt_cached = false;
  h->dt_requested = false;
  h->dt_mp_pending = false;
  return 0;
}

int pion_gpu_download(void *handle, int which, double *P_soa)
{
  Handle *h = use(handle);
  const size_t nb = sizeof(double) * (size_t)h->cfg.nvar * h->g.ncell;
  const double *src = (which == 1 && h->ph_valid) ? h->dPh : h->dP;
  if (int rc = order_after_unpack(h)) return rc;
  HCHECK(h, hipMemcpyAsync(P_soa, src, nb, hipMemcpyDeviceToHost, h->stream));
  HCHECK(h, hipStreamSynchronize(h->stream));
  return check_errword(h);
}

int pion_gpu_bind_device_state(void *handle, void *dP, void *dPh)
{
  Handle *h = use(handle);
  h->xghost_fresh = nullptr;
  if (!dP || !dPh) return PION_GPU_EINVAL;
  if (h->own_state) {
    hipFree(h->dP);
    hipFree(h->dPh);
  }
  h->own_state = false;
  h->dP = (double *)dP;
  h->dPh = (double *)dPh;
  h->ph_valid = false;
  h->dt_cached = false;
  h->dt_requested = false;
  return 0;
}
void *pion_gpu_device_ptr(void *handle, int which)
{
  Handle *h = use(handle);
  h->xghost_fresh = nullptr;
  h->dt_cached = false;
  return which == 0 ? (void *)h->dP : (void *)h->dPh;
}
int pion_gpu_set_stream(void *handle, void *stream)
{
  ((Handle *)handle)->stream = (hipStream_t)stream;
  return 0;
}
int pion_gpu_set_comm_stream(void *handle, void *stream)
{
  Handle *h = use(handle);
  h->comm_stream = (hipStream_t)stream;
  h->ev_unpacked_valid = false;
  return 0;
}
int pion_gpu_synchronize(void *handle)
{
  Handle *h = use(handle);
  HCHECK(h, hipStreamSynchronize(h->stream));
  if (h->comm_stream && h->comm_stream != h->stream) HCHECK(h, hipStreamSynchronize(h->comm_stream));
  if (h->bstream) HCHECK(h, hipStreamSynchronize(h->bstream));
  return 0;
}

int pion_gpu_set_wind_cells(void *handle, long n, const long *idx, const double *states)
{
  Handle *h = use(handle);
  h->dt_cached = false;
  hipFree(h->dwind_idx);
  hipFree(h->dwind_state);
  h->dwind_idx = nullptr;
  h->dwind_state = nullptr;
  h->nwind = n;
  if (n > 0) {
    for (long k = 0; k < n; k++) {
      if (idx[k] < 0 || idx[k] >= h->g.ncell) {
        h->nwind = 0;
        return PION_GPU_EINVAL;
      }
    }
    HCHECK(h, hipMalloc(&h->dwind_idx, sizeof(long) * n));
    HCHECK(h, hipMalloc(&h->dwind_state, sizeof(double) * n * h->cfg.nvar));
    HCHECK(h, hipMemcpy(h->dwind_idx, idx, sizeof(long) * n, hipMemcpyHostToDevice));
    HCHECK(h, hipMemcpy(h->dwind_state, states, sizeof(double) * n * h->cfg.nvar, hipMemcpyHostToDevice));
    hipLaunchKernelGGL(k_flag_wind_list, dim3((unsigned)((n + 255) / 256)), dim3(256), 0, h->stream, h->dwind_idx, n,
                       h->dflags);
    HCHECK(h, hipGetLastError());
    HCHECK(h, hipStreamSynchronize(h->stream));
  }
  return 0;
}

int pion_gpu_add_wind_source(void *handle, const pion_gpu_wind_source *src, int *id)
{
  Handle *h = use(handle);
  if (!h || !src) return PION_GPU_EINVAL;
  const pion_gpu_config &cfg = h->cfg;
  const GridDesc &g = h->g;
  auto fail = [&](const char *m) {
    h->err = m;
    return PION_GPU_EINVAL;
  };
  if (h->wsrc.size() >= PION_MAX_WIND_SOURCES) return fail("wind source: at most PION_MAX_WIND_SOURCES sources");
  if (src->type == 2 || src->type == 3) return fail("wind source: angle / latitude-dependent winds are not supported");
  if (src->type != 0 && src->type != 1) return fail("What type of source is this?  add a new type?");
  if (src->type == 1)
    for (const WindSource &o : h->wsrc)
      if (o.type == 2) return fail("wind source: evolving and rotating sources cannot share a grid");
  if (!(src->radius > 0.0)) return fail("wind source: radius must be > 0");
  if (cfg.coord_sys == 3 && !equalD(src->pos[0], 0.0)) return fail("Spherical symmetry but source not at origin!");
  if (cfg.coord_sys == 2 && cfg.ndim == 2 && !equalD(src->pos[1], 0.0))
    return fail("Axisymmetry but source not at R=0!");
  if (cfg.ndim == 1 && cfg.eqntype != PION_EQEUL) return fail("1D spherical but MHD?");
  if (src->orbit_period != 0 && (cfg.ndim < 2 || cfg.coord_sys != 1))
    return fail("wind source: orbital motion needs a 2-D or 3-D Cartesian grid");
  if (src->type == 1) {
    if (src->npt < 2) return fail("evolving wind source: the table needs at least 2 rows");
    if (!src->evo_time || !src->evo_Teff || !src->evo_Mdot || !src->evo_vrot || !src->evo_vinf || !src->evo_R)
      return fail("evolving wind source: missing table column");
    for (int v = 0; v < cfg.ntracer; v++) {
      const int e = src->evo_tracer_elem[v];
      if (e < -1 || e > 6 || (e >= 0 && !src->evo_X[e])) return fail("evolving wind source: bad tracer selector");
    }
  }
  WindSource W;
  W.type = src->type;
  for (int a = 0; a < 3; a++) W.pos[a] = (a < cfg.ndim) ? src->pos[a] : 0.0;
  W.radius = src->radius;
  W.Bstar = src->Bstar;
  for (int v = 0; v < PION_MAX_NVAR; v++) {
    W.tr[v] = (v < cfg.ntracer) ? src->tracers[v] : 0.0;
    W.elem[v] = (src->type == 1 && v < cfg.ntracer) ? src->evo_tracer_elem[v] : -1;
  }
  double mdot = src->mdot, vinf = src->vinf, vrot = src->vrot, Tw = src->Tw, Rstar = src->Rstar;
  if (src->type == 1) {
    const int n = src->npt;
    W.t.assign(src->evo_time, src->evo_time + n);
    W.Teff.assign(src->evo_Teff, src->evo_Teff + n);
    W.Mdot.assign(src->evo_Mdot, src->evo_Mdot + n);
    W.vrot.assign(src->evo_vrot, src->evo_vrot + n);
    W.vinf.assign(src->evo_vinf, src->evo_vinf + n);
    W.R.assign(src->evo_R, src->evo_R + n);
    for (int e = 0; e < 7; e++)
      if (src->evo_X[e]) W.X[e].assign(src->evo_X[e], src->evo_X[e] + n);
    W.tstart = W.t[0];
    W.tfinish = W.t[n - 1];
    const double t_now = src->t_now;
    W.t_next_update = std::max(W.tstart, t_now);
    double x[7] = {0, 0, 0, 0, 0, 0, 0};
    if (((t_now + src->update_freq) > W.tstart || equalD(W.tstart, t_now)) && t_now < W.tfinish) {
      W.active = true;
      Tw = root_find_linear_vec(W.t, W.Teff, t_now);
      mdot = root_find_linear_vec(W.t, W.Mdot, t_now);
      vinf = root_find_linear_vec(W.t, W.vinf, t_now);
      vrot = root_find_linear_vec(W.t, W.vrot, t_now);
      Rstar = root_find_linear_vec(W.t, W.R, t_now);
      for (int e = 0; e < 7; e++)
        if (!W.X[e].empty()) x[e] = root_find_linear_vec(W.t, W.X[e], t_now);
    }
    else {
      W.active = false;
      mdot = -100.0;
      vinf = -100.0;
      Tw = -100.0;
      vrot = 0.0;
      Rstar = 0.0;
    }
    for (int v = 0; v < cfg.ntracer; v++)
      if (W.elem[v] >= 0) W.tr[v] = x[W.elem[v]];
  }
  W.Mdot_c = mdot * 1.9891e33 / 3.1558150e7;
  W.Vinf_c = vinf * 1.0e5;
  W.vrot_c = vrot * 1.0e5;
  W.Tw_c = Tw;
  W.Rstar_c = Rstar;

  if (src->orbit_period != 0) {
    W.moving = true;
    W.orbit = *src;
    for (int a = 0; a < 3; a++) W.orbit.pos[a] = W.pos[a];
    return add_moving_wind_source(h, W, id);
  }

  return add_fixed_wind_source(h, W, id);
}

int pion_gpu_add_rotating_wind_source(void *handle, const pion_gpu_wind_source *src, const double *evo_vcrit,
                                      double xi, int *id)
{
  Handle *h = use(handle);
  if (!h || !src) return PION_GPU_EINVAL;
  const pion_gpu_config &cfg = h->cfg;
  auto fail = [&](const char *m) {
    h->err = m;
    return PION_GPU_EINVAL;
  };
  if (h->wsrc.size() >= PION_MAX_WIND_SOURCES) return fail("wind source: at most PION_MAX_WIND_SOURCES sources");
  if (src->type != 2) return fail("Bad wind type for evolving stellar wind (rotating star)!");
  if (cfg.ndim < 2) return fail("rotating wind source: needs a 2-D or 3-D grid (theta = 0 in 1-D)");
  if (cfg.coord_sys == 2 && !equalD(src->pos[1], 0.0)) return fail("Axisymmetry but source not at R=0!");
  if (src->orbit_period != 0) return fail("rotating wind source: add_rotating_source takes no orbit");
  if (!(src->radius > 0.0)) return fail("wind source: radius must be > 0");
  if (src->npt < 2) return fail("evolving wind source: the table needs at least 2 rows");
  if (!src->evo_time || !src->evo_Teff || !src->evo_Mdot || !src->evo_vrot || !src->evo_vinf || !src->evo_R ||
      !evo_vcrit)
    return fail("evolving wind source: missing table column");
  for (int v = 0; v < cfg.ntracer; v++) {
    const int e = src->evo_tracer_elem[v];
    if (e < -1 || e > 6 || (e >= 0 && !src->evo_X[e])) return fail("evolving wind source: bad tracer selector");
  }
  for (const WindSource &o : h->wsrc) {
    if (o.type == 1) return fail("wind source: evolving and rotating sources cannot share a grid");
    if (o.type == 2 && !(xi == h->angle.xi)) return fail("rotating wind source: xi differs from an earlier source's");
  }
  if (!h->have_angle || !(xi == h->angle.xi)) {
    lgm99::setup_tables(xi, h->angle);
    h->have_angle = true;
  }
  const AngleTables &T = h->angle;
  WindSource W;
  W.type = 2;
  for (int a = 0; a < 3; a++) W.pos[a] = (a < cfg.ndim) ? src->pos[a] : 0.0;
  W.radius = src->radius;
  W.Bstar = src->Bstar;
  for (int v = 0; v < PION_MAX_NVAR; v++) {
    W.tr[v] = (v < cfg.ntracer) ? src->tracers[v] : 0.0;
    W.elem[v] = (v < cfg.ntracer) ? src->evo_tracer_elem[v] : -1;
  }
  {
    const WindMember m = wind_member(h, W);
    unsigned long long *dcount = nullptr, cnt = 0;
    HCHECK(h, hipMalloc(&dcount, sizeof(unsigned long long)));
    HCHECK(h, hipMemsetAsync(dcount, 0, sizeof(unsigned long long), h->stream));
    hipLaunchKernelGGL(k_wind_theta_bad, dim3((unsigned)((h->g.ncell + 255) / 256)), dim3(256), 0, h->stream, m,
                       T.theta[0], T.theta[PION_ANGLE_NTHETA - 1], dcount);
    HCHECK(h, hipGetLastError());
    HCHECK(h, hipMemcpyAsync(&cnt, dcount, sizeof cnt, hipMemcpyDeviceToHost, h->stream));
    HCHECK(h, hipStreamSynchronize(h->stream));
    hipFree(dcount);
    if (cnt > 0) return fail("rotating wind source: a member cell's theta lies outside the LGM99 table");
  }
  const int n = src->npt;
  W.t.assign(src->evo_time, src->evo_time + n);
  W.Teff.assign(src->evo_Teff, src->evo_Teff + n);
  W.Mdot.assign(src->evo_Mdot, src->evo_Mdot + n);
  W.vrot.assign(src->evo_vrot, src->evo_vrot + n);
  W.vinf.assign(src->evo_vinf, src->evo_vinf + n);
  W.vcrit.assign(evo_vcrit, evo_vcrit + n);
  W.R.assign(src->evo_R, src->evo_R + n);
  for (int e = 0; e < 7; e++)
    if (src->evo_X[e]) W.X[e].assign(src->evo_X[e], src->evo_X[e] + n);
  W.tstart = W.t[0];
  W.tfinish = W.t[n - 1];
  const double t_now = src->t_now;
  W.t_next_update = std::max(W.tstart, t_now);
  double mdot = 0.0, vinf = 0.0, Twind = 0.0, vrot = 0.0, rstar = 0.0, vcrt = 0.0;
  double x[7] = {0, 0, 0, 0, 0, 0, 0};
  if (((t_now + src->update_freq) > W.tstart || equalD(W.tstart, t_now)) && t_now < W.tfinish) {
    W.active = true;
    Twind = root_find_linear_vec(W.t, W.Teff, t_now);
    mdot = root_find_linear_vec(W.t, W.Mdot, t_now);
    vinf = root_find_linear_vec(W.t, W.vinf, t_now);
    vrot = root_find_linear_vec(W.t, W.vrot, t_now);
    vcrt = root_find_linear_vec(W.t, W.vcrit, t_now);
    rstar = root_find_linear_vec(W.t, W.R, t_now);
    for (int e = 0; e < 7; e++)
      if (!W.X[e].empty()) x[e] = root_find_linear_vec(W.t, W.X[e], t_now);
  }
  else {
    W.active = false;
    mdot = -100.0;
    vinf = -100.0;
    vrot = -100.0;
    Twind = -100.0;
  }
  for (int v = 0; v < cfg.ntracer; v++)
    if (W.elem[v] >= 0) W.tr[v] = x[W.elem[v]];
  const double Tmax = T.Teff[PION_ANGLE_NTEFF - 1];
  W.Mdot_c = mdot;
  W.Vinf_c = vinf;
  W.vrot_c = vrot;
  W.vcrit_c = vcrt;
  W.Tw_c = (Tmax < Twind) ? Tmax : Twind;
  W.Rstar_c = rstar;
  return add_fixed_wind_source(h, W, id);
}

int pion_gpu_wind_angle_tables(double xi, double *theta, double *omega, double *Teff, double *delta, double *alpha)
{
  AngleTables T;
  lgm99::setup_tables(xi, T);
  if (theta) memcpy(theta, T.theta, sizeof T.theta);
  if (omega) memcpy(omega, T.omega, sizeof T.omega);
  if (Teff) memcpy(Teff, T.Teff, sizeof T.Teff);
  if (delta) memcpy(delta, T.delta.data(), sizeof(double) * T.delta.size());
  if (alpha) memcpy(alpha, T.alpha.data(), sizeof(double) * T.alpha.size());
  return 0;
}

int pion_gpu_get_wind_source_pos(void *handle, int id, double *pos)
{
  Handle *h = use(handle);
  if (!h || !pos || id < 0 || id >= (int)h->wsrc.size()) return PION_GPU_EINVAL;
  for (int a = 0; a < PION_MAX_DIM; a++) pos[a] = (a < 3) ? h->wsrc[id].pos[a] : 0.0;
  return 0;
}

int pion_gpu_get_flags(void *handle, unsigned char *out)
{
  Handle *h = use(handle);
  if (!h || !out) return PION_GPU_EINVAL;
  HCHECK(h, hipMemcpyAsync(out, h->dflags, h->g.ncell, hipMemcpyDeviceToHost, h->stream));
  HCHECK(h, hipStreamSynchronize(h->stream));
  return 0;
}

int pion_gpu_wind_orbit_position(const pion_gpu_wind_source *src, int ndim, double simtime, double *pos)
{
  if (!src || !pos || ndim < 2 || ndim > 3) return PION_GPU_EINVAL;
  double p[3];
  wind_orbit_position(*src, ndim, simtime, p);
  for (int a = 0; a < PION_MAX_DIM; a++) pos[a] = (a < 3) ? p[a] : 0.0;
  return 0;
}

int pion_gpu_get_wind_cells(void *handle, int id, long *n, long *idx, double *states)
{
  Handle *h = use(handle);
  if (!h || !n || id < 0 || id >= (int)h->wsrc.size()) return PION_GPU_EINVAL;
  const WindSource &W = h->wsrc[id];
  long cnt = W.n;
  if (W.moving) {
    HCHECK(h, hipMemcpyAsync(&cnt, W.dn, sizeof cnt, hipMemcpyDeviceToHost, h->stream));
    HCHECK(h, hipStreamSynchronize(h->stream));
    if (cnt < 0 || cnt > W.n) {
      h->err = "wind source: device cell count out of range";
      return PION_GPU_EDEVICE;
    }
  }
  *n = cnt;
  if (!idx || cnt == 0) return 0;
  HCHECK(h, hipMemcpyAsync(idx, h->dws_idx + W.off, sizeof(long) * cnt, hipMemcpyDeviceToHost, h->stream));
  if (states)
    HCHECK(h, hipMemcpyAsync(states, h->dws_state + W.off * h->cfg.nvar, sizeof(double) * cnt * h->cfg.nvar,
                             hipMemcpyDeviceToHost, h->stream));
  HCHECK(h, hipStreamSynchronize(h->stream));
  return 0;
}

int pion_gpu_set_jet(void *handle, int jetradius, const double *jetstate)
{
  Handle *h = use(handle);
  h->dt_cached = false;
  const pion_gpu_config &cfg = h->cfg;
  const GridDesc &g = h->g;
  const bool cart3d = (cfg.ndim == 3 && cfg.coord_sys == 1 && cfg.eqntype == PION_EQEUL);
  const bool cyl2d = (cfg.ndim == 2 && cfg.coord_sys == 2);
  if ((!cart3d && !cyl2d) || !jetstate) {
    h->err = "jet boundary: 3-D Cartesian Euler or 2-D cylindrical only (jet_boundaries.cpp:88-91,203-206)";
    return PION_GPU_EINVAL;
  }
  std::vector<long> idx;
  if (cart3d) {
    const double jr = jetradius * g.dx;
    for (int iz = 0; iz < g.ng[2]; iz++)
      for (int iy = 0; iy < g.ng[1]; iy++) {
        const double y = g.xmin[1] + (2 * iy + 1) * (0.5 * g.dx), z = g.xmin[2] + (2 * iz + 1) * (0.5 * g.dx);
        if (sqrt(y * y + z * z) <= jr)
          for (int k = 1; k <= g.nbc[0]; k++) idx.push_back(cell_id(g, -k, iy, iz));
      }
  }
  else {
    if (jetradius > g.ng[1]) {
      h->err = "Not enough cells for jet";
      return PION_GPU_EINVAL;
    }
    for (int iy = 0; iy < jetradius; iy++)
      for (int k = 1; k <= g.nbc[0]; k++) idx.push_back(cell_id(g, -k, iy, 0));
  }
  std::vector<double> rv(jetstate, jetstate + cfg.nvar);
  if (cfg.eqntype != PION_EQEUL) {
    rv[5] = jetstate[5];
    rv[6] = 0.0;
    rv[7] = jetstate[6];
  }
  hipFree(h->djet_idx);
  hipFree(h->djet_state);
  h->djet_idx = nullptr;
  h->djet_state = nullptr;
  h->njet = (long)idx.size();
  std::vector<double> st((size_t)h->njet * cfg.nvar);
  for (long k = 0; k < h->njet; k++)
    for (int v = 0; v < cfg.nvar; v++) st[(size_t)k * cfg.nvar + v] = rv[v];
  if (h->njet > 0) {
    HCHECK(h, hipMalloc(&h->djet_idx, sizeof(long) * h->njet));
    HCHECK(h, hipMalloc(&h->djet_state, sizeof(double) * st.size()));
    HCHECK(h, hipMemcpy(h->djet_idx, idx.data(), sizeof(long) * h->njet, hipMemcpyHostToDevice));
    HCHECK(h, hipMemcpy(h->djet_state, st.data(), sizeof(double) * st.size(), hipMemcpyHostToDevice));
  }
  return 0;
}

int pion_gpu_set_cooling_tables(void *handle, int nT, const double *T, const double *tabs, const double *slopes)
{
  Handle *h = use(handle);
  h->dt_cached = false;
  if (nT < 2 || nT > PION_COOL_NT_MAX) {
    h->err = "cooling tables: 2 <= nT <= 256 required";
    return PION_GPU_EINVAL;
  }
  hipFree(h->dcoolT);
  hipFree(h->dcooltab);
  hipFree(h->dcoolslope);
  HCHECK(h, hipMalloc(&h->dcoolT, sizeof(double) * nT));
  HCHECK(h, hipMalloc(&h->dcooltab, sizeof(double) * 5 * nT));
  HCHECK(h, hipMalloc(&h->dcoolslope, sizeof(double) * 5 * nT));
  HCHECK(h, hipMemcpy(h->dcoolT, T, sizeof(double) * nT, hipMemcpyHostToDevice));
  HCHECK(h, hipMemcpy(h->dcooltab, tabs, sizeof(double) * 5 * nT, hipMemcpyHostToDevice));
  HCHECK(h, hipMemcpy(h->dcoolslope, slopes, sizeof(double) * 5 * nT, hipMemcpyHostToDevice));
  h->cool.lg0 = 0.0f;
  h->cool.inv_dlg = 0.0f;
  if (T[0] > 0.0 && T[nT - 1] > T[0]) {
    const double l0 = log2(T[0]), inv = (nT - 1) / (log2(T[nT - 1]) - l0);
    bool ok = true;
    for (int i = 0; i < nT && ok; i++) {
      if (!(T[i] > 0.0) || (i > 0 && !(T[i] > T[i - 1]))) ok = false;
      else if (fabs((log2(T[i]) - l0) * inv - i) > 0.25) ok = false;
    }
    if (ok) {
      h->cool.lg0 = (float)l0;
      h->cool.inv_dlg = (float)inv;
    }
  }
  if (const char *e = getenv("PION_COOL_BISECT")) {
    if (atoi(e) != 0) h->cool.inv_dlg = 0.0f;
  }
  h->cool.NT = nT;
  h->cool.T = h->dcoolT;
  h->cool.tab = h->dcooltab;
  h->cool.slope = h->dcoolslope;
  h->have_tables = true;
  return 0;
}

int pion_gpu_update_bcs(void *handle, double simtime, int cstep, int maxstep, int assign)
{
  Handle *h = use(handle);
  const pion_gpu_config &cfg = h->cfg;
  const GridDesc &g = h->g;
  const bool full = (cstep == maxstep);
  double *T = full ? h->dP : h->dPh;
  if (h->nws > 0 && h->have_angle) {
    if (int rc = wind_angle_check(h, simtime)) return rc;
  }
  time_begin(h, 2);

  if (h->nwind > 0) {
    hipLaunchKernelGGL(k_wind, dim3((unsigned)((h->nwind + 255) / 256)), dim3(256), 0, h->stream, T, h->dwind_idx,
                       h->dwind_state, h->nwind, cfg.nvar, g.ncell);
  }
  if (h->nws > 0) {
    if (int rc = wind_sources_update(h, simtime)) return rc;
  }
  bool all_periodic = (!any_wind(h) && !cfg.bc_dmach2 && h->fuse_bc);
  for (int d = 0; d < 2 * cfg.ndim && all_periodic; d++) {
    const bool zface = (d >= 4);
    if (!(cfg.bc_type[d] == PION_BC_PERIODIC || (zface && cfg.bc_type[d] == PION_BC_SLAB))) all_periodic = false;
  }
  if (all_periodic && cfg.ndim == 3 && cfg.bc_type[4] != cfg.bc_type[5]) all_periodic = false;
  if (all_periodic) {
    const int zwrap = (cfg.ndim == 3 && cfg.bc_type[4] == PION_BC_PERIODIC) ? 1 : 0;
    const int skipx = (h->xghost_fresh == T) ? 1 : 0;
    const long n = (zwrap ? (long)2 * g.nbc[2] * g.nga[0] * g.nga[1] : 0) + (long)g.ng[2] * 2 * g.nbc[1] * g.nga[0]
                   + (skipx ? 0 : (long)g.ng[2] * g.ng[1] * 2 * g.nbc[0]);
    hipLaunchKernelGGL(k_bc_periodic_all, dim3((unsigned)((n + 255) / 256)), dim3(256), 0, h->stream, T, g, cfg.nvar,
                       zwrap, skipx);
  }
  h->xghost_fresh = nullptr;
  const bool one_launch = (!all_periodic && !assign && h->fuse_bc);
  if (one_launch) {
    BCAllArgs a;
    a.g = g;
    a.T = T;
    a.nvar = cfg.nvar;
    a.eqntype = cfg.eqntype;
    a.ntracer = cfg.ntracer;
    a.ndim = cfg.ndim;
    for (int d = 0; d < 6; d++) {
      a.type[d] = (d < 2 * cfg.ndim) ? cfg.bc_type[d] : 0;
      for (int v = 0; v < PION_MAX_NVAR; v++) a.refval[d][v] = h->refval[d][v];
    }
    a.dmr_a0 = 10.0 * simtime / sin(M_PI / 3.0);
    a.dmr_t3 = tan(M_PI / 3.0);
    a.dmr2_cols = (cfg.bc_dmach2 && h->dmr2_cols > 0) ? h->dmr2_cols : 0;
    for (int v = 0; v < PION_MAX_NVAR; v++) a.dmr2_val[v] = 0.0;
    a.dmr2_val[0] = 8.0;
    a.dmr2_val[1] = 116.5;
    a.dmr2_val[2] = 7.14470958;
    a.dmr2_val[3] = -4.125;
    for (int v = cfg.nvar - cfg.ntracer; v < cfg.nvar; v++) a.dmr2_val[v] = 1.0;
    const long n = ((cfg.ndim == 3) ? (long)2 * g.nbc[2] * g.nga[0] * g.nga[1] : 0)
                   + ((cfg.ndim >= 2) ? (long)g.ng[2] * 2 * g.nbc[1] * g.nga[0] : 0) + (long)g.ng[2] * g.ng[1] * 2 * g.nbc[0];
    hipLaunchKernelGGL(k_bc_all, dim3((unsigned)((n + 255) / 256)), dim3(256), 0, h->stream, a);
  }
  for (int d = 0; d < 2 * cfg.ndim && !all_periodic && !one_launch; d++) {
    const int type = cfg.bc_type[d];
    if (type == 0 || type == PION_BC_SLAB) continue;
    if (assign) {
      const int ax = d / 2;
      const bool pos = d & 1;
      if (type == PION_BC_INFLOW || type == PION_BC_FIXED) {
        int i[3] = {0, 0, 0};
        const bool last = (type == PION_BC_INFLOW);
        for (int a = 0; a < 3; a++) {
          if (a == ax) i[a] = pos ? g.ng[a] - 1 : 0;
          else if (a < ax || a >= cfg.ndim) i[a] = last ? g.ng[a] + g.nbc[a] - 1 : -g.nbc[a];
          else i[a] = last ? g.ng[a] - 1 : 0;
        }
        const long c = cell_id(g, i[0], i[1], i[2]);
        HCHECK(h, hipStreamSynchronize(h->stream));
        for (int v = 0; v < cfg.nvar; v++)
          HCHECK(h, hipMemcpy(&h->refval[d][v], h->dP + v * g.ncell + c, sizeof(double), hipMemcpyDeviceToHost));
      }
      else if (type == PION_BC_DMACH) {
        for (int v = 0; v < PION_MAX_NVAR; v++) h->refval[d][v] = 0.0;
        h->refval[d][0] = 1.4;
        h->refval[d][1] = 1.0;
        for (int v = cfg.nvar - cfg.ntracer; v < cfg.nvar; v++) h->refval[d][v] = -1.0;
      }
    }
    BCArgs a;
    a.g = g;
    a.T = T;
    a.nvar = cfg.nvar;
    a.dir = d;
    a.type = type;
    a.eqntype = cfg.eqntype;
    a.ntracer = cfg.ntracer;
    for (int v = 0; v < PION_MAX_NVAR; v++) a.refval[v] = h->refval[d][v];
    a.dmr_a0 = 10.0 * simtime / sin(M_PI / 3.0);
    a.dmr_t3 = tan(M_PI / 3.0);
    const int ax = d / 2;
    long total = g.nbc[ax];
    for (int a2 = 0; a2 < 3; a2++) {
      if (a2 == ax) continue;
      total *= (a2 < ax || a2 >= cfg.ndim) ? g.nga[a2] : g.ng[a2];
    }
    hipLaunchKernelGGL(k_bc_face, dim3((unsigned)((total + 255) / 256)), dim3(256), 0, h->stream, a);
  }
  if (cfg.bc_dmach2 && h->dmr2_cols > 0 && !one_launch) {
    BCArgs a;
    a.g = g;
    a.T = T;
    a.nvar = cfg.nvar;
    a.dir = -1;
    a.type = PION_BC_DMACH2;
    a.eqntype = cfg.eqntype;
    a.ntracer = cfg.ntracer;
    for (int v = 0; v < PION_MAX_NVAR; v++) a.refval[v] = 0.0;
    a.refval[0] = 8.0;
    a.refval[1] = 116.5;
    a.refval[2] = 7.14470958;
    a.refval[3] = -4.125;
    a.refval[4] = 0.0;
    for (int v = cfg.nvar - cfg.ntracer; v < cfg.nvar; v++) a.refval[v] = 1.0;
    a.dmr_a0 = a.dmr_t3 = 0.0;
    const int n = h->dmr2_cols * g.nbc[1];
    hipLaunchKernelGGL(k_bc_dmr2, dim3((n + 255) / 256), dim3(256), 0, h->stream, a, h->dmr2_cols);
  }
  if (h->njet > 0) {
    hipLaunchKernelGGL(k_wind, dim3((unsigned)((h->njet + 255) / 256)), dim3(256), 0, h->stream, T, h->djet_idx,
                       h->djet_state, h->njet, cfg.nvar, g.ncell);
  }
  time_end(h, 2);
  HCHECK(h, hipGetLastError());
  if (full) h->ph_valid = false;
  return 0;
}

int pion_gpu_calc_dt_device(void *handle, void **dptr)
{
  Handle *h = use(handle);
  DtArgs a;
  a.g = h->g;
  a.P = h->dP;
  a.Ph = h->ph_valid ? h->dPh : h->dP;
  a.flags = h->dflags;
  a.result = h->ddt;
  a.errword = h->derr;
  a.eqntype = h->cfg.eqntype;
  a.nvar = h->cfg.nvar;
  a.gamma = h->cfg.gamma;
  a.cfl = h->cfg.cfl;
  a.do_mp = mp_dt_limited(h->cfg) ? 1 : 0;
  a.cool = h->cool;
  if (a.do_mp && !h->have_tables) {
    h->err = "cooling tables not set";
    return PION_GPU_EINVAL;
  }
  if (!h->dt_cached) {
    HCHECK(h, hipMemcpyAsync(h->ddt, h->ddt_init, 2 * sizeof(double), hipMemcpyDeviceToDevice, h->stream));
    time_begin(h, 3);
    const int rc = h->cfg.strict_fp ? fp_strict::launch_dt(a, h->stream) : fp_fast::launch_dt(a, h->stream);
    time_end(h, 3);
    if (rc != 0) {
      h->err = "dt kernel launch failed";
      return PION_GPU_EDEVICE;
    }
    h->dt_cached = true;
  }
  if (dptr) *dptr = h->ddt;
  return 0;
}

int pion_gpu_dt_request(void *handle)
{
  Handle *h = use(handle);
  if (!h->hdt) HCHECK(h, hipHostMalloc((void **)&h->hdt, 4 * sizeof(double), hipHostMallocDefault));
  if (!h->ev_dt) HCHECK(h, hipEventCreateWithFlags(&h->ev_dt, hipEventDisableTiming));
  HCHECK(h, hipMemcpyAsync(h->hdt, h->ddt, 2 * sizeof(double), hipMemcpyDeviceToHost, h->stream));
  HCHECK(h, hipMemcpyAsync(h->hdt + 2, h->derr, sizeof(int), hipMemcpyDeviceToHost, h->stream));
  HCHECK(h, hipEventRecord(h->ev_dt, h->stream));
  h->dt_requested = true;
  return 0;
}

int pion_gpu_dt_wait(void *handle, double *t_dyn, double *t_mp)
{
  Handle *h = use(handle);
  if (!h->dt_requested) {
    h->err = "pion_gpu_dt_wait without pion_gpu_dt_request";
    return PION_GPU_EINVAL;
  }
  HCHECK(h, hipEventSynchronize(h->ev_dt));
  h->dt_requested = false;
  *t_dyn = h->hdt[0];
  *t_mp = h->hdt[1];
  int e;
  memcpy(&e, h->hdt + 2, sizeof e);
  if (e) return check_errword(h);
  return 0;
}

int pion_gpu_read_dt(void *handle, double *t_dyn, double *t_mp)
{
  if (int rc = pion_gpu_dt_request(handle)) return rc;
  return pion_gpu_dt_wait(handle, t_dyn, t_mp);
}

int pion_gpu_calc_dt(void *handle, double *t_dyn, double *t_mp)
{
  if (int rc = pion_gpu_calc_dt_device(handle, nullptr)) return rc;
  return pion_gpu_read_dt(handle, t_dyn, t_mp);
}

void *pion_gpu_get_stream(void *handle, int which)
{
  Handle *h = use(handle);
  return (void *)(which == 0 ? h->stream : (h->comm_stream ? h->comm_stream : h->stream));
}

int pion_gpu_set_glm_speeds(void *handle, double dt, double dx, double cr)
{
  Handle *h = use(handle);
  h->glm_chyp = h->cfg.cfl * dx / dt;
  h->glm_cr = cr;
  return 0;
}

static bool stage_can_split(const Handle *h)
{
  return h->use_march != 0 && !h->deta && h->g.ndim == 3
         && h->g.ng[2] > 2 * h->g.nbc[2] && !(h->cfg.tm_ooa == 1 && h->cfg.sp_ooa == 1);
}

static int launch_cooling_time(Handle *h, hipStream_t s)
{
  const pion_gpu_config &cfg = h->cfg;
  DtArgs d;
  d.g = h->g;
  d.P = h->dP;
  d.Ph = h->dP;
  d.flags = h->dflags;
  d.result = h->ddt;
  d.errword = h->derr;
  d.eqntype = cfg.eqntype;
  d.nvar = cfg.nvar;
  d.gamma = cfg.gamma;
  d.cfl = cfg.cfl;
  d.do_mp = 1;
  d.cool = h->cool;
  time_begin(h, 3);
  const int rc = cfg.strict_fp ? fp_strict::launch_dt_mp(d, s) : fp_fast::launch_dt_mp(d, s);
  time_end(h, 3);
  if (rc != 0) {
    h->err = "cooling-time kernel launch failed";
    return PION_GPU_EDEVICE;
  }
  return 0;
}

static int stage_launch(Handle *h, double dt_stage, int space_ooa, int is_full_step, int kz0, int kz1,
                        bool first, bool last, int kz2 = 0, int kz3 = 0, hipStream_t ls = 0, bool use_ls = false)
{
  if (!use_ls) ls = h->stream;
  const pion_gpu_config &cfg = h->cfg;
  if (cfg.cooling != 0 && !h->have_tables) {
    h->err = "cooling tables not set";
    return PION_GPU_EINVAL;
  }
  const double *S = h->ph_valid ? h->dPh : h->dP;
  int rc = 0;
  if (h->dhll || h->deta) {
    PrepassArgs p;
    p.g = h->g;
    p.S = S;
    p.hllflag = h->dhll;
    p.divv = nullptr;
    p.gradp = nullptr;
    p.eta = h->deta;
    p.eqntype = cfg.eqntype;
    p.nvar = cfg.nvar;
    p.space_ooa = space_ooa;
    p.gamma = cfg.gamma;
    p.c0 = 0;
    p.c1 = h->g.ncell;
    p.c2 = p.c3 = 0;
    if (!(first && last)) {
      const int nb = h->g.nbc[2], nz = h->g.ng[2];
      int lo = kz0 - 1, hi = kz1 + 1;
      if (kz0 == 0) {
        lo = -1;
        hi = nb - 1;
      }
      else if (kz1 == nz) {
        lo = nz - nb + 1;
        hi = nz + 1;
      }
      p.c0 = (long)(lo + nb) * h->g.sz;
      p.c1 = (long)(hi + nb) * h->g.sz;
    }
    if (kz3 > kz2) {
      const int nb = h->g.nbc[2], nz = h->g.ng[2];
      p.c2 = (long)(nz - nb + 1 + nb) * h->g.sz;
      p.c3 = (long)(nz + 1 + nb) * h->g.sz;
    }
    time_begin(h, 1);
    rc = cfg.strict_fp ? fp_strict::launch_prepass(p, ls) : fp_fast::launch_prepass(p, ls);
    time_end(h, 1);
    if (rc != 0) {
      h->err = "prepass launch failed";
      return PION_GPU_EDEVICE;
    }
  }
  StageArgs a;
  a.g = h->g;
  a.S = S;
  a.Pc = h->dP;
  a.out = is_full_step ? h->dP : h->dPh;
  if (is_full_step && !h->ph_valid && cfg.sp_ooa == 2 && space_ooa == 2) {
    h->err = "full-step stage requires a preceding half-step stage";
    return PION_GPU_EINVAL;
  }
  if (is_full_step && S == h->dP) {
    a.out = h->dPh;
  }
  a.flags = h->dflags;
  a.hllflag = h->dhll;
  a.eta = h->deta;
  a.errword = h->derr;
  a.fc = make_fluxctx(h, dt_stage);
  a.eqntype = cfg.eqntype;
  a.ntracer = cfg.ntracer;
  a.solver = cfg.solver;
  a.space_ooa = space_ooa;
  a.cooling = cfg.cooling;
  a.dt = dt_stage;
  a.glm_damp = exp(-dt_stage * h->glm_chyp * h->glm_cr);
  a.max_temp = cfg.max_temp;
  a.cool = h->cool;
  a.use_march = h->use_march;
  a.kz0 = kz0;
  a.kz1 = kz1;
  a.kz2 = kz2;
  a.kz3 = (kz3 > kz2) ? kz3 : kz2;
  a.zslope_lds = h->zslope_lds;
  a.plain_cells = any_wind(h) ? 0 : 1;
  a.dE = nullptr;
  a.xwrap = (a.use_march != 0 && h->fuse_bc && cfg.bc_type[0] == PION_BC_PERIODIC
             && cfg.bc_type[1] == PION_BC_PERIODIC && h->g.ng[0] >= 2 * h->g.nbc[0]) ? 1 : 0;
  a.ncu = h->ncu;
  {
    Rows2PlanIn p;
    p.ndim = h->g.ndim;
    p.nx = h->g.ng[0];
    p.ny = h->g.ng[1];
    p.np = kz1 - kz0;
    p.ncu = h->ncu;
    p.nv = cfg.nvar;
    p.euler = (cfg.eqntype == PION_EQEUL);
    p.march = (a.use_march != 0);
    p.zslope_lds = (a.zslope_lds != 0);
    p.second_order = (space_ooa == 2);
    p.uneven = h->uneven_chunks;
    p.want_rows = h->rows;
    p.want_rows1 = h->rows1;
    p.want_zchunk = h->zchunk;
    const Rows2Plan pl = rows2_plan(p);
    a.rows = pl.rows;
    a.rows_auto = pl.rows_auto;
    a.zchunk = pl.zchunk;
    a.zcmax = pl.zcmax;
    a.nzb = pl.nzb;
  }
  if (cfg.cooling != 0 && a.use_march != 0) {
    a.dE = h->ddE;
    time_begin(h, 1);
    rc = cfg.strict_fp ? fp_strict::launch_cooling_dE(a, ls) : fp_fast::launch_cooling_dE(a, ls);
    time_end(h, 1);
    if (rc != 0) {
      h->err = "cooling kernel launch failed";
      return PION_GPU_EDEVICE;
    }
  }
  const bool fuse_dt = h->fuse_dt && is_full_step && space_ooa == 2 && a.use_march != 0
                       && ((h->g.ndim == 3 && h->g.nbc[2] >= 2) || h->g.ndim == 2) && a.out == h->dP;
  a.dtres = nullptr;
  a.cfl = cfg.cfl;
  const bool split_mp = fuse_dt && mp_dt_limited(cfg) && h->split_dt_mp;
  a.dt_mp = (mp_dt_limited(cfg) && !split_mp) ? 1 : 0;
  h->dt_cached = false;
  if (fuse_dt) {
    if (first)
      HCHECK(h, hipMemcpyAsync(h->ddt, h->ddt_init, 2 * sizeof(double), hipMemcpyDeviceToDevice, ls));
    a.dtres = h->ddt;
  }
  if (first && !last && h->concurrent_strips && !h->timing && h->comm_stream && h->comm_stream != h->stream) {
    if (!h->ev_pre) HCHECK(h, hipEventCreateWithFlags(&h->ev_pre, hipEventDisableTiming));
    HCHECK(h, hipEventRecord(h->ev_pre, ls));
    h->ev_pre_valid = true;
  }
  time_begin(h, 0);
  rc = cfg.strict_fp ? fp_strict::launch_stage(a, ls) : fp_fast::launch_stage(a, ls);
  time_end(h, 0);
  if (rc != 0) {
    h->err = "stage kernel launch failed (unsupported eqn/solver/tracer combination?)";
    return PION_GPU_EDEVICE;
  }
  if (!last) return 0;
  if (split_mp) {
    if (use_ls) h->dt_mp_pending = true;
    else if (int rc2 = launch_cooling_time(h, ls)) return rc2;
  }
  if (is_full_step && a.out == h->dPh) {
    const size_t nb = sizeof(double) * (size_t)cfg.nvar * h->g.ncell;
    HCHECK(h, hipMemcpyAsync(h->dP, h->dPh, nb, hipMemcpyDeviceToDevice, ls));
  }
  h->ph_valid = !is_full_step;
  h->dt_cached = fuse_dt;
  h->xghost_fresh = a.xwrap ? ((is_full_step && a.out == h->dPh) ? h->dP : a.out) : nullptr;
  return 0;
}

int pion_gpu_stage_part(void *handle, double dt_stage, int space_ooa, int is_full_step, int part)
{
  Handle *h = use(handle);
  const int nz = h->g.ng[2], nb = h->g.nbc[2];
  if (part == PION_STAGE_WHOLE) {
    if (int rc = order_after_unpack(h)) return rc;
    return stage_launch(h, dt_stage, space_ooa, is_full_step, 0, nz, true, true);
  }
  const bool split = stage_can_split(h);
  if (part == PION_STAGE_INTERIOR) {
    if (!split) return 0;
    return stage_launch(h, dt_stage, space_ooa, is_full_step, nb, nz - nb, true, false);
  }
  if (part != PION_STAGE_ZBOUNDARY) return PION_GPU_EINVAL;
  if (split && h->ev_pre_valid && h->ev_unpacked_valid) {
    h->ev_pre_valid = false;
    if (!h->bstream) HCHECK(h, hipStreamCreateWithFlags(&h->bstream, hipStreamNonBlocking));
    if (!h->ev_bdone) HCHECK(h, hipEventCreateWithFlags(&h->ev_bdone, hipEventDisableTiming));
    HCHECK(h, hipStreamWaitEvent(h->bstream, h->ev_pre, 0));
    HCHECK(h, hipStreamWaitEvent(h->bstream, h->ev_unpacked, 0));
    const int rc = stage_launch(h, dt_stage, space_ooa, is_full_step, 0, nb, false, true, nz - nb, nz, h->bstream, true);
    if (rc) return rc;
    HCHECK(h, hipEventRecord(h->ev_bdone, h->bstream));
    HCHECK(h, hipStreamWaitEvent(h->stream, h->ev_bdone, 0));
    if (h->dt_mp_pending) {
      h->dt_mp_pending = false;
      if (int rc2 = launch_cooling_time(h, h->stream)) return rc2;
    }
    return order_after_unpack(h);
  }
  h->ev_pre_valid = false;
  if (int rc = order_after_unpack(h)) return rc;
  if (!split) return stage_launch(h, dt_stage, space_ooa, is_full_step, 0, nz, true, true);
  return stage_launch(h, dt_stage, space_ooa, is_full_step, 0, nb, false, true, nz - nb, nz);
}

int pion_gpu_stage(void *handle, double dt_stage, int space_ooa, int is_full_step)
{
  return pion_gpu_stage_part(handle, dt_stage, space_ooa, is_full_step, PION_STAGE_WHOLE);
}

int pion_gpu_advance_time(void *handle, double dt, double simtime)
{
  Handle *h = use(handle);
  int rc;
  if (h->cfg.tm_ooa == 1 && h->cfg.sp_ooa == 1) {
    if ((rc = pion_gpu_stage(handle, dt, 1, 1))) return rc;
    return pion_gpu_update_bcs(handle, simtime, 1, 1, 0);
  }
  if (h->cfg.tm_ooa == 2 && h->cfg.sp_ooa == 2) {
    if ((rc = pion_gpu_stage(handle, 0.5 * dt, 1, 0))) return rc;
    if ((rc = pion_gpu_update_bcs(handle, simtime, 1, 2, 0))) return rc;
    if ((rc = pion_gpu_stage(handle, dt, 2, 1))) return rc;
    return pion_gpu_update_bcs(handle, simtime, 2, 2, 0);
  }
  h->err = "Bad OOA requests; choose (1,1) or (2,2)";
  return PION_GPU_EINVAL;
}

long pion_gpu_halo_count(void *handle)
{
  Handle *h = use(handle);
  return (long)h->cfg.nvar * h->g.nbc[2] * h->g.nga[0] * h->g.nga[1];
}
static int halo_go(Handle *h, int which, int face, void *dbuf, int pack)
{
  if (h->cfg.ndim != 3 || (face != 4 && face != 5)) return PION_GPU_EINVAL;
  double *A = (which == 0) ? h->dP : h->dPh;
  const long n = pion_gpu_halo_count(h);
  hipStream_t cs = h->comm_stream ? h->comm_stream : h->stream;
  if (cs != h->stream && pack) {
    if (!h->ev_packed_src) HCHECK(h, hipEventCreateWithFlags(&h->ev_packed_src, hipEventDisableTiming));
    HCHECK(h, hipEventRecord(h->ev_packed_src, h->stream));
    HCHECK(h, hipStreamWaitEvent(cs, h->ev_packed_src, 0));
  }
  hipLaunchKernelGGL(k_halo, dim3((unsigned)((n + 255) / 256)), dim3(256), 0, cs, A, (double *)dbuf, h->g,
                     h->cfg.nvar, face, pack);
  HCHECK(h, hipGetLastError());
  if (cs != h->stream && !pack) {
    if (!h->ev_unpacked) HCHECK(h, hipEventCreateWithFlags(&h->ev_unpacked, hipEventDisableTiming));
    HCHECK(h, hipEventRecord(h->ev_unpacked, cs));
    h->ev_unpacked_valid = true;
  }
  return 0;
}
int pion_gpu_halo_spans(void *handle, int which, pion_gpu_halo_spans_t *out)
{
  Handle *h = use(handle);
  if (h->cfg.ndim != 3 || !out) return PION_GPU_EINVAL;
  double *A = (which == 0) ? h->dP : h->dPh;
  const long nb = h->g.nbc[2], nz = h->g.ng[2], sz = h->g.sz;
  out->recv_lo = A;
  out->send_lo = A + nb * sz;
  out->send_hi = A + nz * sz;
  out->recv_hi = A + (nz + nb) * sz;
  out->count_per_var = nb * sz;
  out->var_stride = h->g.ncell;
  out->nvar = h->cfg.nvar;
  return 0;
}
int pion_gpu_halo_begin(void *handle)
{
  Handle *h = use(handle);
  hipStream_t cs = h->comm_stream ? h->comm_stream : h->stream;
  if (cs != h->stream) {
    if (!h->ev_packed_src) HCHECK(h, hipEventCreateWithFlags(&h->ev_packed_src, hipEventDisableTiming));
    HCHECK(h, hipEventRecord(h->ev_packed_src, h->stream));
    HCHECK(h, hipStreamWaitEvent(cs, h->ev_packed_src, 0));
  }
  return 0;
}
int pion_gpu_halo_end(void *handle)
{
  Handle *h = use(handle);
  hipStream_t cs = h->comm_stream ? h->comm_stream : h->stream;
  if (cs != h->stream) {
    if (!h->ev_unpacked) HCHECK(h, hipEventCreateWithFlags(&h->ev_unpacked, hipEventDisableTiming));
    HCHECK(h, hipEventRecord(h->ev_unpacked, cs));
    h->ev_unpacked_valid = true;
  }
  return 0;
}
int pion_gpu_pack_halo(void *handle, int which, int face, void *dbuf) { return halo_go(use(handle), which, face, dbuf, 1); }
int pion_gpu_unpack_halo(void *handle, int which, int face, void *dbuf) { return halo_go(use(handle), which, face, dbuf, 0); }

int pion_gpu_interface_flux(void *handle, int n, int axis, double dt, const double *Pl, const double *Pr,
                            const double *aux, double *F, double *Pstar)
{
  Handle *h = use(handle);
  const int nv = h->cfg.nvar;
  DevBuf bl, br, ba, bf, bp;
  const size_t nb = sizeof(double) * (size_t)n * nv;
  HCHECK(h, hipMalloc(&bl.p, nb));
  HCHECK(h, hipMalloc(&br.p, nb));
  HCHECK(h, hipMalloc(&bf.p, nb));
  HCHECK(h, hipMalloc(&bp.p, nb));
  HCHECK(h, hipMalloc(&ba.p, sizeof(double) * 4 * n));
  double *dl = bl.p, *dr = br.p, *da = ba.p, *df = bf.p, *dp = bp.p;
  HCHECK(h, hipMemcpy(dl, Pl, nb, hipMemcpyHostToDevice));
  HCHECK(h, hipMemcpy(dr, Pr, nb, hipMemcpyHostToDevice));
  HCHECK(h, hipMemcpy(da, aux, sizeof(double) * 4 * n, hipMemcpyHostToDevice));
  FluxTestArgs a;
  a.n = n;
  a.axis = axis;
  a.eqntype = h->cfg.eqntype;
  a.ntracer = h->cfg.ntracer;
  a.solver = h->cfg.solver;
  a.Pl = dl;
  a.Pr = dr;
// ... 118 lines not shown
```

pion_amd/csrc/stage_helpers.h:

```cpp
#ifndef PION_STAGE_HELPERS_H
#define PION_STAGE_HELPERS_H

template <int NV, bool MHD>
PDEV void load_rot(const double *S, const long nc, const int ax, const long c, double *q)
{
#pragma unroll
  for (int s = 0; s < NV; s++) q[s] = S[(long)rotvar<MHD>(ax, s) * nc + c];
}

template <int NV>
PDEV void slope3(const double *qm, const double *q0, const double *qp, const double dx, const bool oa2, double *s)
{
#pragma unroll
  for (int v = 0; v < NV; v++) s[v] = oa2 ? avg_falle((q0[v] - qm[v]) / dx, (qp[v] - q0[v]) / dx) : 0.0;
}

template <int EQ, int NV>
PDEV void apply_axis(double *d, const double *q0, const double bnm, const double sim, const double bnp,
                     const double sip, const double *Fm, const double *Fp, const double dt, const double dx)
{
#ifdef PION_FAST_MATH
  const double dtdx = dt / dx;
  if constexpr (EQ != EQEUL) {
    const double uB = q0[qBN] * q0[qVN] + q0[qBT1] * q0[qVT1] + q0[qBT2] * q0[qVT2];
    const double kb = dtdx * (0.5 * (bnm - bnp));
    d[uMN] += kb * q0[qBN];
    d[uMT1] += kb * q0[qBT1];
    d[uMT2] += kb * q0[qBT2];
    d[uERG] += kb * uB;
    d[uBN] += kb * q0[qVN];
    d[uBT1] += kb * q0[qVT1];
    d[uBT2] += kb * q0[qVT2];
    if constexpr (EQ == EQGLM) {
      const double ks = dtdx * (0.5 * (sim - sip)) * q0[qVN];
      d[uERG] += ks * q0[qSI];
      d[uPSI] += ks;
    }
  }
#pragma unroll
  for (int s = 0; s < NV; s++) d[s] += dtdx * (Fm[s] - Fp[s]);
  return;
#endif
  if constexpr (EQ != EQEUL) {
    const double uB = q0[qBN] * q0[qVN] + q0[qBT1] * q0[qVT1] + q0[qBT2] * q0[qVT2];
    const double bm0 = 0.5 * (bnm + q0[qBN]);
    d[uMN] += dt * bm0 * (q0[qBN]) / dx;
    d[uMT1] += dt * bm0 * (q0[qBT1]) / dx;
    d[uMT2] += dt * bm0 * (q0[qBT2]) / dx;
    d[uERG] += dt * bm0 * (uB) / dx;
    d[uBN] += dt * bm0 * (q0[qVN]) / dx;
    d[uBT1] += dt * bm0 * (q0[qVT1]) / dx;
    d[uBT2] += dt * bm0 * (q0[qVT2]) / dx;
    if constexpr (EQ == EQGLM) {
      const double sm0 = 0.5 * (sim + q0[qSI]);
      d[uERG] += dt * sm0 * (q0[qVN] * q0[qSI]) / dx;
      d[uPSI] += dt * sm0 * q0[qVN] / dx;
    }
    const double bm1 = 0.5 * (q0[qBN] + bnp);
    d[uMN] -= dt * bm1 * (q0[qBN]) / dx;
    d[uMT1] -= dt * bm1 * (q0[qBT1]) / dx;
    d[uMT2] -= dt * bm1 * (q0[qBT2]) / dx;
    d[uERG] -= dt * bm1 * (uB) / dx;
    d[uBN] -= dt * bm1 * (q0[qVN]) / dx;
    d[uBT1] -= dt * bm1 * (q0[qVT1]) / dx;
    d[uBT2] -= dt * bm1 * (q0[qVT2]) / dx;
    if constexpr (EQ == EQGLM) {
      const double sm1 = 0.5 * (q0[qSI] + sip);
      d[uERG] -= dt * sm1 * (q0[qVN] * q0[qSI]) / dx;
      d[uPSI] -= dt * sm1 * q0[qVN] / dx;
    }
  }
#pragma unroll
  for (int s = 0; s < NV; s++) {
    const double u1 = (Fm[s] - Fp[s]) / dx;
    d[s] += dt * u1;
  }
}

template <int EQ, int NTR>
PDEV void cell_update(const StageArgs &a, const double *P0, const double *dU, int &err, double *Pf,
                      const bool no_mp = false)
{
  typedef Eqn<EQ, NTR> E;
  constexpr int NV = E::NV;
  const double g = a.fc.gamma;
  double u1[NV];
  MPd mp = a.fc.mp;
  if (no_mp) mp.present = false;
  if (mp.present) {
    double Pi[NV];
#pragma unroll
    for (int v = 0; v < NV; v++) Pi[v] = P0[v];
    E::apply_sCMA(Pi);
    E::PtoU(Pi, u1, g);
  }
  else E::PtoU(P0, u1, g);
#pragma unroll
  for (int v = 0; v < NV; v++) u1[v] += dU[v];
  E::UtoP(u1, Pf, a.fc.min_temp, g, mp, err);
  if (mp.present) E::apply_sCMA(Pf);
  if constexpr (EQ == EQGLM) Pf[qSI] *= a.glm_damp;
  if (mp.present) {
    const double T = Pf[qPG] * mp.Mu_tot_over_kB / Pf[qRO];
    if (T > a.max_temp) Pf[qPG] = Pf[qRO] * a.max_temp / mp.Mu_tot_over_kB;
  }
}
template <int EQ, int NTR>
PDEV void cell_update_store(const StageArgs &a, const long c, const double *P0, const double *dU, int &err,
                           double *Pfout = nullptr, const bool no_mp = false)
{
  constexpr int NV = Eqn<EQ, NTR>::NV;
  const long nc = a.g.ncell;
  double Pf[NV];
  cell_update<EQ, NTR>(a, P0, dU, err, Pf, no_mp);
#pragma unroll
  for (int v = 0; v < NV; v++) a.out[v * nc + c] = Pf[v];
  if (Pfout) {
#pragma unroll
    for (int v = 0; v < NV; v++) Pfout[v] = Pf[v];
  }
}

PDEV double wave_min64(double v)
{
#pragma unroll
  for (int o = 32; o > 0; o >>= 1) {
    const double w = __shfl_xor(v, o, 64);
    v = (w < v) ? w : v;
  }
  return v;
}

#endif
```

pion_amd/csrc/stage_rows2.h:

```cpp
#ifndef PION_STAGE_ROWS2_H
#define PION_STAGE_ROWS2_H

#ifndef PION_ROWS2_NT
#define PION_ROWS2_NT 1
#endif

PDEV void stu(char *ubase, const unsigned off, const double x)
{
  typedef __attribute__((address_space(1))) char *gc;
  typedef __attribute__((address_space(1))) double *gp;
#if PION_ROWS2_NT
  __builtin_nontemporal_store(x, (gp)((gc)uni(ubase) + off));
#else
  *(gp)((gc)uni(ubase) + off) = x;
#endif
}
PDEV double ldu_once(const char *ubase, const unsigned off)
{
  typedef const __attribute__((address_space(1))) char *gc;
  typedef const __attribute__((address_space(1))) double *gp;
#if PION_ROWS2_NT
  return __builtin_nontemporal_load((gp)((gc)uni(ubase) + off));
#else
  return *(gp)((gc)uni(ubase) + off);
// ... 16 lines not shown
PDEV void hslope3(const double *qm, const double *q0, const double *qp, const double dx, const double thr, double *hs)
{
#pragma unroll
  for (int v = 0; v < NV; v++) {
#ifdef PION_FAST_MATH
    const double a = q0[v] - qm[v], b = qp[v] - q0[v];
    hs[v] = fmx(fmn(a, b), fmn(fmx(a, b), 0.0));
#else
    hs[v] = avg_falle((q0[v] - qm[v]) / dx, (qp[v] - q0[v]) / dx) * dx;
#endif
  }
}

template <int NV>
PDEV void cyl_slope3(const double *qm, const double *q0, const double *qp, const double cm, const double c0, const double cp,
                     const bool oa2, double *s)
{
#pragma unroll
  for (int v = 0; v < NV; v++) s[v] = oa2 ? avg_falle((q0[v] - qm[v]) / (c0 - cm), (qp[v] - q0[v]) / (cp - c0)) : 0.0;
}
template <int EQ, int NV>
PDEV void apply_axis_cyl(double *d, const double *q0, const double bnm, const double sim, const double bnp, const double sip,
                         const double *Fm, const double *Fp, const double *s0, const double dt, const double dx,
                         const double Rm1, const double R0, const double Rc, const bool oa2, const double chyp)
{
  constexpr bool MHD = (EQ != EQEUL);
#ifdef PION_FAST_MATH
  {
    const double rn = R0 - dx * 0.5, rp = R0 + dx * 0.5;
    const double idn = 2.0 * dt / (rp * rp - rn * rn);
    const double wn = idn * rn, wp = idn * rp;
    if constexpr (MHD) {
      const double uB = q0[qBN] * q0[qVN] + q0[qBT1] * q0[qVT1] + q0[qBT2] * q0[qVT2];
      const double kb = wn * (0.5 * (bnm + q0[qBN])) - wp * (0.5 * (q0[qBN] + bnp));
      d[uMN] += kb * q0[qBN];
      d[uMT1] += kb * q0[qBT1];
      d[uMT2] += kb * q0[qBT2];
      d[uERG] += kb * uB;
      d[uBN] += kb * q0[qVN];
      d[uBT1] += kb * q0[qVT1];
      d[uBT2] += kb * q0[qVT2];
      if constexpr (EQ == EQGLM) {
        const double ks = (dt / dx) * (0.5 * (sim - sip)) * q0[qVN];
        d[uERG] += ks * q0[qSI];
        d[uPSI] += ks;
      }
    }
#pragma unroll
    for (int s = 0; s < NV; s++) d[s] += wn * Fm[s] - wp * Fp[s];
    const double iR0 = dt / R0;
    if constexpr (!MHD) {
      d[uMN] += iR0 * (oa2 ? (q0[qPG] + (R0 - Rc) * s0[qPG]) : q0[qPG]);
    }
    else {
      const double pm = (q0[qBN] * q0[qBN] + q0[qBT1] * q0[qBT1] + q0[qBT2] * q0[qBT2]) * 0.5;
      if (oa2) {
        d[uMN] += iR0 * (q0[qPG] + pm + (R0 - Rc) * (s0[qPG] + q0[qBN] * s0[qBN] + q0[qBT1] * s0[qBT1] + q0[qBT2] * s0[qBT2]));
        if constexpr (EQ == EQGLM) d[uBN] += iR0 * chyp * (q0[qSI] + (R0 - Rc) * s0[qSI]);
      }
      else {
        d[uMN] += iR0 * (q0[qPG] + pm);
        if constexpr (EQ == EQGLM) d[uBN] += iR0 * chyp * q0[qSI];
      }
    }
    return;
  }
#endif
  if constexpr (MHD) {
    const double uB = q0[qBN] * q0[qVN] + q0[qBT1] * q0[qVT1] + q0[qBT2] * q0[qVT2];
    const double bm0 = 0.5 * (bnm + q0[qBN]);
    {
      double rp = Rm1 + dx * 0.5;
      const double rn = rp;
      rp += dx;
      d[uMN] += dt * bm0 * (q0[qBN]) * 2.0 * rn / (rp * rp - rn * rn);
      d[uMT1] += dt * bm0 * (q0[qBT1]) * 2.0 * rn / (rp * rp - rn * rn);
      d[uMT2] += dt * bm0 * (q0[qBT2]) * 2.0 * rn / (rp * rp - rn * rn);
      d[uERG] += dt * bm0 * (uB) * 2.0 * rn / (rp * rp - rn * rn);
      d[uBN] += dt * bm0 * (q0[qVN]) * 2.0 * rn / (rp * rp - rn * rn);
      d[uBT1] += dt * bm0 * (q0[qVT1]) * 2.0 * rn / (rp * rp - rn * rn);
      d[uBT2] += dt * bm0 * (q0[qVT2]) * 2.0 * rn / (rp * rp - rn * rn);
    }
    if constexpr (EQ == EQGLM) {
      const double sm0 = 0.5 * (sim + q0[qSI]);
      d[uERG] += dt * sm0 * (q0[qVN] * q0[qSI]) / dx;
      d[uPSI] += dt * sm0 * q0[qVN] / dx;
    }
    const double bm1 = 0.5 * (q0[qBN] + bnp);
    {
      const double rp = R0 + dx * 0.5;
      const double rn = rp - dx;
      d[uMN] -= dt * bm1 * (q0[qBN]) * 2.0 * rp / (rp * rp - rn * rn);
      d[uMT1] -= dt * bm1 * (q0[qBT1]) * 2.0 * rp / (rp * rp - rn * rn);
      d[uMT2] -= dt * bm1 * (q0[qBT2]) * 2.0 * rp / (rp * rp - rn * rn);
      d[uERG] -= dt * bm1 * (uB) * 2.0 * rp / (rp * rp - rn * rn);
      d[uBN] -= dt * bm1 * (q0[qVN]) * 2.0 * rp / (rp * rp - rn * rn);
      d[uBT1] -= dt * bm1 * (q0[qVT1]) * 2.0 * rp / (rp * rp - rn * rn);
      d[uBT2] -= dt * bm1 * (q0[qVT2]) * 2.0 * rp / (rp * rp - rn * rn);
    }
    if constexpr (EQ == EQGLM) {
      const double sm1g = 0.5 * (q0[qSI] + sip);
      d[uERG] -= dt * sm1g * (q0[qVN] * q0[qSI]) / dx;
      d[uPSI] -= dt * sm1g * q0[qVN] / dx;
    }
  }
  double u1[NV];
  const double rp = R0 + dx * 0.5;
  const double rn = rp - dx;
#pragma unroll
  for (int s = 0; s < NV; s++) u1[s] = 2.0 * (rn * Fm[s] - rp * Fp[s]) / (rp * rp - rn * rn);
  if constexpr (!MHD) {
    if (oa2) u1[uMN] += (q0[qPG] + (R0 - Rc) * s0[qPG]) / R0;
    else u1[uMN] += q0[qPG] / R0;
  }
  else {
    const double pm = (q0[qBN] * q0[qBN] + q0[qBT1] * q0[qBT1] + q0[qBT2] * q0[qBT2]) / 2.;
    if (oa2) {
      u1[uMN] += (q0[qPG] + pm +
                  (R0 - Rc) * (s0[qPG] + q0[qBN] * s0[qBN] + q0[qBT1] * s0[qBT1] + q0[qBT2] * s0[qBT2])) /
                 R0;
      if constexpr (EQ == EQGLM) u1[uBN] += chyp * (q0[qSI] + (R0 - Rc) * s0[qSI]) / R0;
    }
    else {
      u1[uMN] += (q0[qPG] + pm) / R0;
      if constexpr (EQ == EQGLM) u1[uBN] += chyp * q0[qSI] / R0;
    }
  }
#pragma unroll
  for (int s = 0; s < NV; s++) d[s] += dt * u1[s];
}

#ifndef PION_ROWS2_PF
#define PION_ROWS2_PF 1
#endif
#ifndef PION_ROWS2_COPIES
#define PION_ROWS2_COPIES 1
#endif
#ifndef PION_ROWS2_U0
#define PION_ROWS2_U0 2
#endif

#ifndef PION_ROWS2_MINWG
#define PION_ROWS2_MINWG(EQ) 2
#endif
template <int EQ, int NTR, int SOLVER, int OAMODE, bool PLAIN, bool ZSL, bool CYL = false>
__global__ __launch_bounds__(256, PION_ROWS2_MINWG(EQ)) void k_stage_rows2(const StageArgs a)
{
  typedef Eqn<EQ, NTR> E;
  typedef Flux<EQ, NTR, SOLVER> FX;
  constexpr int NV = E::NV;
  constexpr bool MHD = E::MHD;
  constexpr int NZ = ZSL ? 2 * NV : NV;
  constexpr bool PF = PION_ROWS2_PF && (OAMODE == 1);
  extern __shared__ double lds[];

  const int R = a.rows;
  const RowsTiling tl = rows_tiling(a);
  const int nyg = tl.nyg;
  const int nzc1 = (a.nzb > 0) ? a.nzb : (a.kz1 - a.kz0 + a.zchunk - 1) / a.zchunk;
  const int nzc = nzc1 + (a.kz3 - a.kz2 + a.zchunk - 1) / a.zchunk;
  const int wave = __builtin_amdgcn_readfirstlane((int)(threadIdx.x >> 6));
  const int nb4 = (tl.per_chunk + 3) / 4, nb8 = (nb4 + 7) / 8;
  const int lb = (int)(blockIdx.x >> 3);
  const int cz = lb / nb8, bq = (int)(blockIdx.x & 7) * nb8 + lb % nb8;
  const int tt = bq * 4 + wave;
  if (cz >= nzc || bq >= nb4 || tt >= tl.per_chunk) return;
  const int lane = threadIdx.x & 63;
  int ix, jg, jg_first;
  bool writer;
  if (tt < tl.nfull) {
#if PION_ROWS2_YWG
    const int per4 = 4 * tl.ntx_full, g4 = tt / per4, r4 = tt - g4 * per4;
    const int m = (nyg - 4 * g4 < 4) ? nyg - 4 * g4 : 4;
    const int tx = r4 / m;
    jg = jg_first = 4 * g4 + r4 % m;
#else
    const int tx = tt % tl.ntx_full;
    jg = jg_first = tt / tl.ntx_full;
#endif
    ix = tx * PION_MARCH_XT - 1 + lane;
    writer = (lane >= 1 && lane <= PION_MARCH_XT && ix < a.g.ng[0]);
  }
  else {
    const int seg = lane / (tl.rem + 2), pos = lane % (tl.rem + 2);
    jg_first = (tt - tl.nfull) * tl.spw;
    jg = jg_first + seg;
    ix = tl.ntx_full * PION_MARCH_XT - 1 + pos;
    writer = (seg < tl.spw && jg < nyg && pos >= 1 && pos <= tl.rem);
    if (jg >= nyg) jg = nyg - 1;
  }
  if (ix > a.g.ng[0]) ix = a.g.ng[0];
  const int j0 = jg * R;
  const int nrows = (jg_first * R + R <= a.g.ng[1]) ? R : a.g.ng[1] - jg_first * R;
  const int nrows_l = (j0 + R <= a.g.ng[1]) ? R : a.g.ng[1] - j0;
  int k0, k1;
  if (a.nzb > 0 && cz < nzc1) {
    zchunk_bounds(a.kz1 - a.kz0, a.zcmax, cz, &k0, &k1);
    k0 += a.kz0;
    k1 += a.kz0;
  }
  else {
    k0 = (cz < nzc1) ? a.kz0 + cz * a.zchunk : a.kz2 + (cz - nzc1) * a.zchunk;
    const int kend = (cz < nzc1) ? a.kz1 : a.kz3;
    k1 = (k0 + a.zchunk < kend) ? k0 + a.zchunk : kend;
  }

  const long nc = a.g.ncell, sy = a.g.sy, sz = a.g.sz;
  const long ncb = nc * 8, syb = sy * 8, szb = sz * 8;
  const char *const Sb = reinterpret_cast<const char *>(a.S);
  const char *const Hb = reinterpret_cast<const char *>(a.hllflag);
  const double g = a.fc.gamma, dx = a.g.dx, dt = a.dt;
  const bool oa2 = (OAMODE == 0) ? (a.space_ooa == 2) : (OAMODE == 2);
  const bool noz = (a.g.ndim == 2);
  const double thr = PION_VERY_TINY_VALUE * dx * dx;
  const bool hcorr = PLAIN ? false : (a.fc.artvisc == AV_HCORRECTION || a.fc.artvisc == AV_HCORR_FKJ98);
  const bool same_pc = (OAMODE == 1) ? true : (a.S == a.Pc);
  FluxCtx fc = a.fc;
  if (PLAIN) fc.mp.present = 0;
  int err = 0;
  double tdyn = 1.e100, tmp = 1.0e99;

  const int zbase = wave * R * NZ * 64 + lane;
#define ZS2(r, s) lds[zbase + ((r) * NZ + (s)) * 64]

  const long crow0 = (long)(ix + a.g.nbc[0]) + sy * (j0 + a.g.nbc[1]) + sz * (k0 - 1 + a.g.nbc[2]);

#pragma unroll 1
  for (int r = 0; r < (noz ? 0 : nrows); r++) {
    if constexpr (ZSL) {
      const long c = crow0 + sy * ((r < nrows_l) ? r : nrows_l - 1);
      const unsigned off = pin_v((unsigned)c * 8u);
      double qa[NV], qb[NV], qc[NV], s[NV];
      load_rot2<NV, MHD>(Sb, ncb, 2, -szb, off, qa);
      load_rot2<NV, MHD>(Sb, ncb, 2, 0, off, qb);
      load_rot2<NV, MHD>(Sb, ncb, 2, szb, off, qc);
      if (oa2) hslope3<NV>(qa, qb, qc, dx, thr, s);
      else {
#pragma unroll
        for (int v = 0; v < NV; v++) s[v] = 0.0;
      }
#pragma unroll
      for (int v = 0; v < NV; v++) ZS2(r, v) = s[v];
    }
#pragma unroll
    for (int v = 0; v < NV; v++) ZS2(r, NZ - NV + v) = 0.0;
  }

  double pf[NV], pfb = 0.0, pfs = 0.0;
  unsigned pfh = 0;
  bool pf_valid = false;
#pragma unroll
  for (int v = 0; v < NV; v++) pf[v] = 0.0;

#pragma unroll 1
  for (int k = noz ? k0 : k0 - 1; k < k1; k++) {
    const bool prime = !noz && (k == k0 - 1);
    double Fy[NV], ysn[NV];
#pragma unroll
    for (int v = 0; v < NV; v++) Fy[v] = ysn[v] = 0.0;
    double cyc[4] = {0.0, 0.0, 0.0, 0.0};

#pragma unroll 1
    for (int r = 0; r < nrows; r++) {
      const bool row_ok = (r < nrows_l);
      const long c = crow0 + sy * (row_ok ? r : nrows_l - 1) + sz * (k - (k0 - 1));
      const unsigned off_r = (unsigned)c * 8u, offb_r = (unsigned)c;
      const int jy_r = j0 + (row_ok ? r : nrows_l - 1) + a.g.nbc[1];
      if constexpr (CYL) {
        if (r == 0 || !row_ok) {
          cyc[0] = cyl_Rcom(cyl_R(a.g, jy_r - 1), dx);
          cyc[1] = cyl_Rcom(cyl_R(a.g, jy_r), dx);
          cyc[2] = cyl_Rcom(cyl_R(a.g, jy_r + 1), dx);
        }
        else {
          cyc[0] = cyc[1];
          cyc[1] = cyc[2];
          cyc[2] = cyc[3];
        }
        cyc[3] = cyl_Rcom(cyl_R(a.g, jy_r + 2), dx);
      }
      const double cy_m1 = cyc[0], cy_0 = cyc[1], cy_p1 = cyc[2], cy_p2 = cyc[3];
      const long cn = (r + 1 < nrows) ? crow0 + sy * ((r + 1 < nrows_l) ? r + 1 : nrows_l - 1) + sz * (k - (k0 - 1))
                                      : (noz ? c : crow0 + sz * (k + 1 - (k0 - 1)));
      const unsigned offn_r = (unsigned)cn * 8u, offnb_r = (unsigned)cn;
      const unsigned doff_n = offn_r - off_r, doffb_n = offnb_r - offb_r;
      double q0[NV], dU[NV];
      if (PF && pf_valid && !prime) {
#pragma unroll
        for (int v = 0; v < NV; v++) q0[v] = pf[v];
      }
      else {
        const unsigned o = pin_v(off_r);
#pragma unroll
        for (int v = 0; v < NV; v++) q0[v] = ldu(Sb + v * ncb, o);
      }
#pragma unroll
      for (int v = 0; v < NV; v++) dU[v] = 0.0;
#if defined(PION_FAST_MATH) && PION_ROWS2_U0
      const bool u0 = PLAIN && !same_pc && !prime && a.plain_cells;
#if PION_ROWS2_U0 == 1
      if (u0) {
        const unsigned o = pin_v(off_r);
        const unsigned zu0 = opaque_zero();
        const char *const Pcb0 = reinterpret_cast<const char *>(a.Pc) + zu0;
        double P0[NV];
#pragma unroll
        for (int v = 0; v < NV; v++) P0[v] = ldu_once(Pcb0 + v * ncb, o);
        E::PtoU(P0, dU, g);
      }
#endif
#else
      const bool u0 = false;
#endif
      if (!PLAIN && !prime && a.dE) {
        dU[uERG] += ldu(reinterpret_cast<const char *>(a.dE), pin_v(off_r));
      }

      auto task = [&, c, off_r, offb_r, doff_n, doffb_n, r, row_ok, prime, k, noz, u0, jy_r, cy_m1, cy_0, cy_p1, cy_p2](auto tc, const int t_run, const bool lower) __attribute__((always_inline)) {
        constexpr int TC = decltype(tc)::value;
        const int t = (TC < 0) ? t_run : TC;
        double eL[NV], eR[NV], f[NV], pstar[NV];
        double s0y[NV];
        if constexpr (CYL) {
#pragma unroll
          for (int v = 0; v < NV; v++) s0y[v] = 0.0;
        }
        double bnm = 0.0, sim = 0.0, bnp = 0.0, sip = 0.0;
        long cl, st;
        int ax;
        unsigned hfl = 0, hfr = 0;
        const unsigned zt = opaque_zero();
        const char *const St = Sb + zt, *const Ht = Hb + zt;
        if (t == 0) {
          const unsigned off = pin_v(off_r), offb = pin_v(offb_r);
          ax = 0;
          st = 1;
          cl = c;
          if constexpr (MHD && SOLVER == FLUX_RS_HLLD) {
            if (PF && pf_valid) hfl = pfh;
            else {
              hfl = ldub(Ht, offb);
              hfr = ldub(Ht + 1, offb);
            }
          }
          if (oa2) {
            double qm[NV], qp[NV], sx[NV];
#pragma unroll
            for (int v = 0; v < NV; v++) {
              qm[v] = ldu(St + v * ncb - 8, off);
              qp[v] = ldu(St + v * ncb + 8, off);
            }
#if defined(PION_FAST_MATH) && PION_ROWS2_U0 == 2
            if (u0) {
              const char *const Pcb0 = reinterpret_cast<const char *>(a.Pc) + zt;
#pragma unroll
              for (int v = 0; v < NV; v++) dU[v] = ldu_once(Pcb0 + v * ncb, off);
            }
#endif
            hslope3<NV>(qm, q0, qp, dx, thr, sx);
#pragma unroll
            for (int v = 0; v < NV; v++) {
              eL[v] = q0[v] + sx[v] * 0.5;
              const double em = q0[v] - sx[v] * 0.5;
              eR[v] = lane_next(em);
            }
            if constexpr (MHD) {
              bnm = qm[qBN];
              bnp = qp[qBN];
              if constexpr (EQ == EQGLM) {
                sim = qm[qSI];
                sip = qp[qSI];
              }
            }
// ... 176 lines not shown
          }
          if constexpr (MHD) {
            bnp = qp1[qBN];
            if constexpr (EQ == EQGLM) sip = qp1[qSI];
          }
        }

        double hc_eta = 0.0;
        if (hcorr) hc_eta = select_hcorr_eta(a, ax, cl, st);
        const bool use_hll = (hfl | hfr) != 0;
        if (PF) {
          const unsigned zp = opaque_zero();
          const char *const Sp = Sb + zp, *const Hp = Hb + zp;
          int pax;
          long psh, bsh = 0;
          long hs1, hs2;
          bool wb = true, nextcell = false;
          if (t == 3 || (noz && t == 2 && !lower)) {
            nextcell = true;
            if (prime && r + 1 < nrows) {
              pax = 2;
              psh = szb;
              bsh = -szb;
              hs1 = 0;
              hs2 = sz;
            }
            else {
              pax = 0;
              psh = 0;
              wb = false;
              hs1 = 0;
              hs2 = 1;
            }
          }
          else if (t == 0 && r == 0) {
            pax = 1;
            psh = -syb;
            wb = false;
            hs1 = -sy;
            hs2 = 0;
          }
          else if (t == 0 || lower) {
            pax = 1;
            psh = syb;
            bsh = -syb;
            hs1 = 0;
            hs2 = sy;
          }
          else {
            pax = 2;
            psh = szb;
            bsh = -szb;
            hs1 = 0;
            hs2 = sz;
          }
          const unsigned off = pin_v(off_r + (nextcell ? doff_n : 0u)), offb = pin_v(offb_r + (nextcell ? doffb_n : 0u));
          load_rot2<NV, MHD>(Sp, ncb, pax, psh, off, pf);
          if constexpr (MHD) {
            if (wb) {
              pfb = ldu(Sp + (long)rotvar<MHD>(pax, qBN) * ncb + bsh, off);
              if constexpr (EQ == EQGLM) pfs = ldu(Sp + (long)qSI * ncb + bsh, off);
            }
          }
          if constexpr (MHD && SOLVER == FLUX_RS_HLLD) pfh = ldub(Hp + hs1, offb) | ldub(Hp + hs2, offb);
          pf_valid = true;
        }
        FX::intercell_flux(eL, eR, f, pstar, fc, hc_eta, use_hll, err);

        if (t == 0) {
          double Fm[NV];
#pragma unroll
          for (int v = 0; v < NV; v++) Fm[v] = lane_prev(f[v]);
#if defined(PION_FAST_MATH) && PION_ROWS2_U0 == 2
          if (u0) {
            double P0[NV];
#pragma unroll
            for (int v = 0; v < NV; v++) P0[v] = dU[v];
            E::PtoU(P0, dU, g);
          }
#endif
          apply_axis<EQ, NV>(dU, q0, bnm, sim, bnp, sip, Fm, f, dt, dx);
        }
        else if (t == 2) {
          if (!lower) {
            double d[NV], yq0[NV];
            to_sweep<NV, MHD>(1, q0, yq0);
            to_sweep<NV, MHD>(1, dU, d);
            if constexpr (CYL)
              apply_axis_cyl<EQ, NV>(d, yq0, bnm, sim, bnp, sip, Fy, f, s0y, dt, dx, cyl_R(a.g, jy_r - 1), cyl_R(a.g, jy_r), cy_0,
                                     oa2, a.fc.chyp);
            else apply_axis<EQ, NV>(d, yq0, bnm, sim, bnp, sip, Fy, f, dt, dx);
            from_sweep<NV, MHD>(1, d, dU);
          }
#pragma unroll
          for (int v = 0; v < NV; v++) Fy[v] = f[v];
        }
        else {
          if (!prime) {
            double d[NV], zq0[NV], Fzl[NV];
            to_sweep<NV, MHD>(2, q0, zq0);
            to_sweep<NV, MHD>(2, dU, d);
#pragma unroll
            for (int v = 0; v < NV; v++) Fzl[v] = ZS2(r, NZ - NV + v);
            apply_axis<EQ, NV>(d, zq0, bnm, sim, bnp, sip, Fzl, f, dt, dx);
            from_sweep<NV, MHD>(2, d, dU);
          }
#pragma unroll
          for (int v = 0; v < NV; v++) ZS2(r, NZ - NV + v) = f[v];
        }
      };
#if PION_ROWS2_COPIES
      if (!prime) {
        task(std::integral_constant<int, 0>{}, 0, false);
#pragma unroll 1
        for (int m = (r == 0) ? 1 : 0; m >= 0; m--) task(std::integral_constant<int, 2>{}, 2, m != 0);
      }
      if (!noz) task(std::integral_constant<int, 3>{}, 3, false);
#else
#pragma unroll 1
      for (int t = prime ? 3 : 0; t < 4; t++) {
        if ((t == 1 && r > 0) || (t == 3 && noz)) continue;
        task(std::integral_constant<int, -1>{}, (t == 1) ? 2 : t, t == 1);
      }
#endif

      if (!prime && writer && row_ok) {
        const unsigned off = pin_v(off_r), offb = pin_v(offb_r);
        const unsigned zu = opaque_zero();
        const char *const Pcb = reinterpret_cast<const char *>(a.Pc) + zu;
        char *const Ob = reinterpret_cast<char *>(a.out) + zu;
        const unsigned fl = (PLAIN && a.plain_cells) ? 29u : ldub(reinterpret_cast<const char *>(a.flags) + zu, offb);
        double P0[NV], Pf[NV];
        if (u0) {
          E::UtoP(dU, Pf, a.fc.min_temp, g, MPd{}, err);
          if constexpr (EQ == EQGLM) Pf[qSI] *= a.glm_damp;
        }
        else {
        if (same_pc) {
#pragma unroll
          for (int v = 0; v < NV; v++) P0[v] = q0[v];
        }
        else {
#pragma unroll
          for (int v = 0; v < NV; v++) P0[v] = ldu_once(Pcb + v * ncb, off);
        }
        if (!(fl & 4) || !(fl & 16)) {
#pragma unroll
          for (int v = 0; v < NV; v++) Pf[v] = P0[v];
        }
        else cell_update<EQ, NTR>(a, P0, dU, err, Pf, PLAIN);
        }
#pragma unroll
        for (int v = 0; v < NV; v++) stu(Ob + v * ncb, off, Pf[v]);
        if (a.xwrap) {
          const long xs = (long)a.g.ng[0] * 8;
          if (ix < a.g.nbc[0]) {
#pragma unroll
            for (int v = 0; v < NV; v++) stu(Ob + v * ncb + xs, off, Pf[v]);
          }
          else if (ix >= a.g.ng[0] - a.g.nbc[0]) {
#pragma unroll
            for (int v = 0; v < NV; v++) stu(Ob + v * ncb - xs, off, Pf[v]);
          }
        }
        if (a.dtres) {
          if ((fl & 8) && !(fl & 2)) {
            const double t = cell_dt<EQ>(Pf, a.g.ndim, g, dx, a.cfl);
            if (!(t > 0.0)) err |= ERR_BAD_DT;
            tdyn = (t < tdyn) ? t : tdyn;
          }
          if (a.dt_mp && !(fl & 2) && (fl & 16)) {
            const double t = Cooling::timescale(a.cool, Pf[qRO], Pf[qPG], g);
            tmp = (t < tmp) ? t : tmp;
          }
        }
      }
    }
  }
#undef ZS2
  if (a.dtres) {
    tdyn = wave_min64(tdyn);
    tmp = wave_min64(tmp);
    if (lane == 0) {
      atomicMin(&a.dtres[0], (unsigned long long)__double_as_longlong(tdyn));
      atomicMin(&a.dtres[1], (unsigned long long)__double_as_longlong(tmp));
    }
  }
  if (err) atomicOr(a.errword, err);
}

template <int NV, bool ZSL>
__host__ inline int rows2_rmax()
{
  return rows2_rmax_lds(NV, ZSL);
}

template <void (*KERNEL)(const StageArgs)>
static int rows2_pick_rows_2d(const StageArgs &a)
{
  static int wg_per_cu = 0;
  if (wg_per_cu == 0) {
    int n = 0;
    if (hipOccupancyMaxActiveBlocksPerMultiprocessor(&n, KERNEL, 256, 0) != hipSuccess || n < 1) n = 2;
    wg_per_cu = n;
  }
  return rows2_pick_rows_2d_rule(a.g.ng[0], a.g.ng[1], a.rows, wg_per_cu, a.ncu);
}
template <void (*KERNEL)(const StageArgs)>
static int rows2_launch(StageArgs a, const int rmax, const size_t lds_bytes_per_row, hipStream_t s)
{
  const bool noz = (a.g.ndim == 2);
  if (noz && a.rows_auto) a.rows = rows2_pick_rows_2d<KERNEL>(a);
  if (a.rows > rmax) a.rows = rmax;
  if (a.rows < 1) a.rows = 1;
  const long nblocks = rows2_nblocks(a);
  const size_t shmem = noz ? 0 : lds_bytes_per_row * a.rows;
  hipLaunchKernelGGL(KERNEL, dim3((unsigned)nblocks), dim3(256), shmem, s, a);
  return (int)hipGetLastError();
}

template <int EQ, int NTR, int SOLVER, bool ZSL>
static int stage_rows2_go_z(const StageArgs &a, hipStream_t s)
{
  constexpr int NV = Eqn<EQ, NTR>::NV;
  constexpr int NZ = ZSL ? 2 * NV : NV;
  const bool noz = (a.g.ndim == 2);
  const int rmax = noz ? 64 : rows2_rmax<NV, ZSL>();
  constexpr size_t lds_row = sizeof(double) * 4 * NZ * 64, lds_row1 = sizeof(double) * 4 * NV * 64;
  const int rmax1 = noz ? 64 : rows2_rmax<NV, false>();
  constexpr bool specialise = (SOLVER == FLUX_RS_HLLD && EQ != EQEUL)
                              || ((SOLVER == FLUX_RSroe || SOLVER == FLUX_FVS) && EQ == EQEUL);
  if constexpr (specialise) {
    const bool plain = (a.cooling == 0 && !a.fc.mp.present && a.fc.artvisc != AV_HCORRECTION
                        && a.fc.artvisc != AV_HCORR_FKJ98);
    if (plain) {
      if (a.space_ooa == 2) return rows2_launch<k_stage_rows2<EQ, NTR, SOLVER, 2, true, ZSL>>(a, rmax, lds_row, s);
      return rows2_launch<k_stage_rows2<EQ, NTR, SOLVER, 1, true, false>>(a, rmax1, lds_row1, s);
    }
    if (a.space_ooa == 2) return rows2_launch<k_stage_rows2<EQ, NTR, SOLVER, 2, false, ZSL>>(a, rmax, lds_row, s);
    return rows2_launch<k_stage_rows2<EQ, NTR, SOLVER, 1, false, false>>(a, rmax1, lds_row1, s);
  }
  else
    return rows2_launch<k_stage_rows2<EQ, NTR, SOLVER, 0, false, ZSL>>(a, rmax, lds_row, s);
}

template <int EQ, int NTR, int SOLVER>
static int stage_rows2_go_cyl(const StageArgs &a, hipStream_t s)
{
  constexpr bool specialise = (SOLVER == FLUX_RS_HLLD && EQ != EQEUL)
                              || ((SOLVER == FLUX_RSroe || SOLVER == FLUX_FVS) && EQ == EQEUL);
  if constexpr (specialise) {
    const bool plain = (a.cooling == 0 && !a.fc.mp.present && a.fc.artvisc != AV_HCORRECTION
                        && a.fc.artvisc != AV_HCORR_FKJ98);
    if (plain && a.space_ooa == 2) return rows2_launch<k_stage_rows2<EQ, NTR, SOLVER, 2, true, false, true>>(a, 64, 0, s);
    if (plain && a.space_ooa == 1) return rows2_launch<k_stage_rows2<EQ, NTR, SOLVER, 1, true, false, true>>(a, 64, 0, s);
  }
  return rows2_launch<k_stage_rows2<EQ, NTR, SOLVER, 0, false, false, true>>(a, 64, 0, s);
}

template <int EQ, int NTR, int SOLVER>
static int stage_rows2_go(const StageArgs &a, hipStream_t s)
{
  if (a.g.ndim == 2 && a.g.cyl == 1) return stage_rows2_go_cyl<EQ, NTR, SOLVER>(a, s);
  if (a.zslope_lds && a.space_ooa == 2) return stage_rows2_go_z<EQ, NTR, SOLVER, true>(a, s);
  return stage_rows2_go_z<EQ, NTR, SOLVER, false>(a, s);
}

#endif
```

pion_amd/lib.py:

```python
import ctypes as C
import os

import numpy as np

from . import abi

_dp = C.POINTER(C.c_double)
_lib = None


class PionGpuError(RuntimeError):
    def __init__(self, what, rc, msg):
        super().__init__("pion_gpu_%s failed rc=%d: %s" % (what, rc, msg))
        self.rc = rc


def load_library():
    global _lib
    if _lib is not None:
        return _lib
    path = abi.library_path()
    if not os.path.exists(path):
        raise ImportError(
            "%s not found: build it with `make -C pion_amd/csrc` (or __graft_entry__.build()); "
            "pion_amd has no CPU fallback" % path)
    abi.share_torch_hip_runtime()
    lib = C.CDLL(path)
    lib.pion_gpu_create.argtypes = [C.POINTER(abi.PionGpuConfig), C.c_int, C.POINTER(C.c_void_p)]
    lib.pion_gpu_destroy.argtypes = [C.c_void_p]
    lib.pion_gpu_destroy.restype = None
    lib.pion_gpu_last_error.argtypes = [C.c_void_p, C.c_char_p, C.c_int]
    lib.pion_gpu_ncell_all.argtypes = [C.c_void_p]
    lib.pion_gpu_ncell_all.restype = C.c_long
    lib.pion_gpu_upload.argtypes = [C.c_void_p, _dp]
    lib.pion_gpu_download.argtypes = [C.c_void_p, C.c_int, _dp]
    lib.pion_gpu_bind_device_state.argtypes = [C.c_void_p, C.c_void_p, C.c_void_p]
    lib.pion_gpu_device_ptr.argtypes = [C.c_void_p, C.c_int]
    lib.pion_gpu_device_ptr.restype = C.c_void_p
    lib.pion_gpu_set_stream.argtypes = [C.c_void_p, C.c_void_p]
    lib.pion_gpu_set_comm_stream.argtypes = [C.c_void_p, C.c_void_p]
    lib.pion_gpu_set_jet.argtypes = [C.c_void_p, C.c_int, _dp]
    lib.pion_gpu_stage_part.argtypes = [C.c_void_p, C.c_double, C.c_int, C.c_int, C.c_int]
    lib.pion_gpu_synchronize.argtypes = [C.c_void_p]
    lib.pion_gpu_set_wind_cells.argtypes = [C.c_void_p, C.c_long, C.POINTER(C.c_long), _dp]
    lib.pion_gpu_add_wind_source.argtypes = [C.c_void_p, C.c_void_p, C.POINTER(C.c_int)]
    lib.pion_gpu_add_rotating_wind_source.argtypes = [C.c_void_p, C.c_void_p, _dp, C.c_double, C.POINTER(C.c_int)]
    lib.pion_gpu_wind_angle_tables.argtypes = [C.c_double, _dp, _dp, _dp, _dp, _dp]
    lib.pion_gpu_get_wind_cells.argtypes = [C.c_void_p, C.c_int, C.POINTER(C.c_long), C.POINTER(C.c_long), _dp]
    lib.pion_gpu_get_wind_source_pos.argtypes = [C.c_void_p, C.c_int, _dp]
    lib.pion_gpu_wind_orbit_position.argtypes = [C.c_void_p, C.c_int, C.c_double, _dp]
    lib.pion_gpu_get_flags.argtypes = [C.c_void_p, C.c_void_p]
    lib.pion_gpu_set_cooling_tables.argtypes = [C.c_void_p, C.c_int, _dp, _dp, _dp]
    lib.pion_gpu_update_bcs.argtypes = [C.c_void_p, C.c_double, C.c_int, C.c_int, C.c_int]
    lib.pion_gpu_calc_dt.argtypes = [C.c_void_p, _dp, _dp]
    lib.pion_gpu_set_glm_speeds.argtypes = [C.c_void_p, C.c_double, C.c_double, C.c_double]
    lib.pion_gpu_stage.argtypes = [C.c_void_p, C.c_double, C.c_int, C.c_int]
    lib.pion_gpu_advance_time.argtypes = [C.c_void_p, C.c_double, C.c_double]
    lib.pion_gpu_halo_count.argtypes = [C.c_void_p]
    lib.pion_gpu_halo_count.restype = C.c_long
    lib.pion_gpu_pack_halo.argtypes = [C.c_void_p, C.c_int, C.c_int, C.c_void_p]
    lib.pion_gpu_unpack_halo.argtypes = [C.c_void_p, C.c_int, C.c_int, C.c_void_p]
    lib.pion_gpu_interface_flux.argtypes = [C.c_void_p, C.c_int, C.c_int, C.c_double, _dp, _dp, _dp, _dp, _dp]
    lib.pion_gpu_cooling_update.argtypes = [C.c_void_p, C.c_int, C.c_double, _dp, _dp]
    lib.pion_gpu_cooling_edot.argtypes = [C.c_void_p, C.c_int, _dp, _dp, _dp]
    lib.pion_gpu_cooling_timescale.argtypes = [C.c_void_p, C.c_int, _dp, _dp]
    lib.pion_gpu_enable_timing.argtypes = [C.c_void_p, C.c_int]
    lib.pion_gpu_get_timing.argtypes = [C.c_void_p, _dp, C.c_int]
    _lib = lib
    return lib


EXPORTED_SYMBOLS = [
    "pion_gpu_create", "pion_gpu_destroy", "pion_gpu_last_error", "pion_gpu_ncell_all",
    "pion_gpu_ng_all", "pion_gpu_upload", "pion_gpu_download", "pion_gpu_bind_device_state",
    "pion_gpu_device_ptr", "pion_gpu_set_stream", "pion_gpu_synchronize", "pion_gpu_set_wind_cells",
    "pion_gpu_set_cooling_tables", "pion_gpu_update_bcs", "pion_gpu_calc_dt",
    "pion_gpu_set_glm_speeds", "pion_gpu_stage", "pion_gpu_advance_time", "pion_gpu_halo_count",
    "pion_gpu_pack_halo", "pion_gpu_unpack_halo", "pion_gpu_interface_flux",
    "pion_gpu_cooling_update", "pion_gpu_cooling_edot", "pion_gpu_cooling_timescale", "pion_gpu_enable_timing",
    "pion_gpu_calc_dt_device", "pion_gpu_read_dt", "pion_gpu_get_stream", "pion_gpu_dt_request", "pion_gpu_dt_wait",
    "pion_gpu_halo_spans", "pion_gpu_halo_begin", "pion_gpu_halo_end",
    "pion_gpu_get_timing", "pion_gpu_stage_part", "pion_gpu_set_comm_stream", "pion_gpu_set_jet",
    "pion_gpu_add_wind_source", "pion_gpu_get_wind_cells", "pion_gpu_get_wind_source_pos",
    "pion_gpu_wind_orbit_position", "pion_gpu_get_flags", "pion_gpu_add_rotating_wind_source",
    "pion_gpu_wind_angle_tables",
]


def _p(a):
    return a.ctypes.data_as(_dp)


class GpuSim:

    def __init__(self, cfg, device=0, borrowed_handle=None):
        self.lib = load_library()
        self.cfg = cfg
        self.owner = borrowed_handle is None
        if borrowed_handle is not None:
            self.h = C.c_void_p(borrowed_handle)
        else:
            self.h = C.c_void_p()
            rc = self.lib.pion_gpu_create(C.byref(cfg), device, C.byref(self.h))
            if rc != 0:
                msg = self._err() if self.h else "invalid configuration"
                self.h = None
                raise PionGpuError("create", rc, msg)
        self.nvar = cfg.nvar
        self.ncell = abi.ncell_all(cfg)
        nga = abi.ng_all(cfg)
        self.shape = (cfg.nvar, nga[2], nga[1], nga[0])

    def _err(self):
        buf = C.create_string_buffer(512)
        self.lib.pion_gpu_last_error(self.h, buf, 512)
        return buf.value.decode()

    def _chk(self, rc, what):
        if rc != 0:
            raise PionGpuError(what, rc, self._err())

    def close(self):
        if getattr(self, "h", None):
            if self.owner:
                self.lib.pion_gpu_destroy(self.h)
            self.h = None

    def __enter__(self):
        return self

    def __exit__(self, *a):
        self.close()

    def __del__(self):
        try:
            self.close()
        except Exception:
            pass

    def upload(self, P):
        P = np.ascontiguousarray(P, dtype=np.float64).reshape(-1)
        assert P.size == self.nvar * self.ncell
        self._chk(self.lib.pion_gpu_upload(self.h, _p(P)), "upload")

    def download(self, which=0):
        out = np.empty(self.nvar * self.ncell)
        self._chk(self.lib.pion_gpu_download(self.h, which, _p(out)), "download")
        return out.reshape(self.shape)

    def bind_device_state(self, dP_ptr, dPh_ptr):
        self._chk(self.lib.pion_gpu_bind_device_state(self.h, C.c_void_p(dP_ptr), C.c_void_p(dPh_ptr)),
                  "bind_device_state")

    def device_ptr(self, which):
        return self.lib.pion_gpu_device_ptr(self.h, which)

    def set_stream(self, stream_ptr):
        self._chk(self.lib.pion_gpu_set_stream(self.h, C.c_void_p(stream_ptr)), "set_stream")

    def set_comm_stream(self, stream_ptr):
        self._chk(self.lib.pion_gpu_set_comm_stream(self.h, C.c_void_p(stream_ptr)), "set_comm_stream")

    def synchronize(self):
        self._chk(self.lib.pion_gpu_synchronize(self.h), "synchronize")

    def set_wind_cells(self, idx, states):
        idx = np.ascontiguousarray(idx, dtype=np.int64)
        states = np.ascontiguousarray(states, dtype=np.float64)
        self._chk(self.lib.pion_gpu_set_wind_cells(self.h, idx.size, idx.ctypes.data_as(C.POINTER(C.c_long)),
                                                   _p(states)), "set_wind_cells")

    def add_wind_source(self, src):
        st, keep = src.to_c()
        i = C.c_int(-1)
        self._chk(self.lib.pion_gpu_add_wind_source(self.h, C.byref(st), C.byref(i)), "add_wind_source")
        del keep
        return i.value

    def add_rotating_wind_source(self, src):
        st, keep = src.to_c()
        vcrit = keep[-1].ctypes.data_as(_dp) if src.evolution is not None else None
        i = C.c_int(-1)
        self._chk(self.lib.pion_gpu_add_rotating_wind_source(self.h, C.byref(st), vcrit, src.xi, C.byref(i)),
                  "add_rotating_wind_source")
        del keep
        return i.value

    def get_wind_cells(self, sid):
        n = C.c_long(0)
        self._chk(self.lib.pion_gpu_get_wind_cells(self.h, sid, C.byref(n), None, None), "get_wind_cells")
        idx = np.zeros(n.value, dtype=np.int64)
        st = np.zeros((n.value, self.nvar))
        self._chk(self.lib.pion_gpu_get_wind_cells(self.h, sid, C.byref(n), idx.ctypes.data_as(C.POINTER(C.c_long)),
                                                   _p(st)), "get_wind_cells")
        return idx, st

    def get_wind_source_pos(self, sid):
        out = np.zeros(3)
        self._chk(self.lib.pion_gpu_get_wind_source_pos(self.h, sid, _p(out)), "get_wind_source_pos")
        return tuple(out)

    def get_flags(self):
        out = np.zeros(self.ncell, dtype=np.uint8)
        self._chk(self.lib.pion_gpu_get_flags(self.h, out.ctypes.data), "get_flags")
        return out

    def set_jet(self, jetradius, jetstate):
        st = np.ascontiguousarray(jetstate, dtype=np.float64)
        self._chk(self.lib.pion_gpu_set_jet(self.h, int(jetradius), _p(st)), "set_jet")

    def set_cooling_tables(self, T, tabs, slopes):
        T = np.ascontiguousarray(T, dtype=np.float64)
        tabs = np.ascontiguousarray(tabs, dtype=np.float64)
        slopes = np.ascontiguousarray(slopes, dtype=np.float64)
        self._chk(self.lib.pion_gpu_set_cooling_tables(self.h, T.size, _p(T), _p(tabs), _p(slopes)),
                  "set_cooling_tables")

    def update_bcs(self, simtime=0.0, cstep=2, maxstep=2, assign=0):
        self._chk(self.lib.pion_gpu_update_bcs(self.h, simtime, cstep, maxstep, assign), "update_bcs")

    def calc_dt(self):
        a, b = C.c_double(), C.c_double()
        self._chk(self.lib.pion_gpu_calc_dt(self.h, C.byref(a), C.byref(b)), "calc_dt")
        return a.value, b.value

    def set_glm_speeds(self, dt, dx, cr):
        self._chk(self.lib.pion_gpu_set_glm_speeds(self.h, dt, dx, cr), "set_glm_speeds")

    def stage(self, dt, space_ooa, is_full):
        self._chk(self.lib.pion_gpu_stage(self.h, dt, space_ooa, is_full), "stage")

    def stage_part(self, dt, space_ooa, is_full, part):
        self._chk(self.lib.pion_gpu_stage_part(self.h, dt, space_ooa, is_full, part), "stage_part")

    def advance_time(self, dt, simtime):
        self._chk(self.lib.pion_gpu_advance_time(self.h, dt, simtime), "advance_time")

    def halo_count(self):
        return self.lib.pion_gpu_halo_count(self.h)

    def pack_halo(self, which, face, dbuf_ptr):
        self._chk(self.lib.pion_gpu_pack_halo(self.h, which, face, C.c_void_p(dbuf_ptr)), "pack_halo")

    def unpack_halo(self, which, face, dbuf_ptr):
        self._chk(self.lib.pion_gpu_unpack_halo(self.h, which, face, C.c_void_p(dbuf_ptr)), "unpack_halo")

    def interface_flux(self, axis, Pl, Pr, aux=None, dt=1.0):
        Pl = np.ascontiguousarray(Pl, dtype=np.float64)
        Pr = np.ascontiguousarray(Pr, dtype=np.float64)
        n = Pl.shape[0]
        if aux is None:
            aux = np.zeros((n, 4))
        aux = np.ascontiguousarray(aux, dtype=np.float64)
        F = np.zeros((n, self.nvar))
        Ps = np.zeros((n, self.nvar))
        self._chk(self.lib.pion_gpu_interface_flux(self.h, n, axis, dt, _p(Pl), _p(Pr), _p(aux), _p(F), _p(Ps)),
                  "interface_flux")
        return F, Ps

    def cooling_update(self, Pin, dt):
        Pin = np.ascontiguousarray(Pin, dtype=np.float64)
        out = np.zeros_like(Pin)
        self._chk(self.lib.pion_gpu_cooling_update(self.h, Pin.shape[0], dt, _p(Pin), _p(out)), "cooling_update")
        return out

    def cooling_edot(self, rho, T):
        rho = np.ascontiguousarray(rho, dtype=np.float64)
        T = np.ascontiguousarray(T, dtype=np.float64)
        out = np.zeros_like(rho)
        self._chk(self.lib.pion_gpu_cooling_edot(self.h, rho.size, _p(rho), _p(T), _p(out)), "cooling_edot")
        return out

    def cooling_timescale(self, Pin):
        Pin = np.ascontiguousarray(Pin, dtype=np.float64)
        out = np.zeros(Pin.shape[0])
        self._chk(self.lib.pion_gpu_cooling_timescale(self.h, Pin.shape[0], _p(Pin), _p(out)), "cooling_timescale")
        return out

    def enable_timing(self, on=True):
        self._chk(self.lib.pion_gpu_enable_timing(self.h, int(on)), "enable_timing")

    def get_timing(self):
        out = np.zeros(8)
        self._chk(self.lib.pion_gpu_get_timing(self.h, _p(out), 8), "get_timing")
        return {"stage_ms": out[0], "prepass_ms": out[1], "bc_ms": out[2], "dt_ms": out[3],
                "stage_n": int(out[4]), "prepass_n": int(out[5]), "bc_n": int(out[6]), "dt_n": int(out[7])}
```

Measured before the change: 6131 Mcell-updates/s.

## Screen quiet blocks from HLLD prepass using per-block pressure min/max

The stage kernel now records per-block min and max pressure via atomic keys as it writes the output state. The next prepass uses these to list only blocks whose neighbourhood pressure range exceeds a quiet threshold, and runs the HLL-switch prepass only on those blocks after zeroing the flag array. The goal is to skip most of the full-grid prepass in smooth regions. The costs are extra atomics and reductions in the stage kernel, a memset of the flag array, and the risk that the quiet criterion misses cells that need the HLL fallback.

```diff
diff --git a/include/pion_gpu.h b/include/pion_gpu.h
--- a/include/pion_gpu.h
+++ b/include/pion_gpu.h
@@ -126,6 +126,8 @@
 int pion_gpu_add_wind_source(void *handle, const pion_gpu_wind_source *src, int *id);
 int pion_gpu_get_wind_source_pos(void *handle, int id, double *pos);
 int pion_gpu_get_flags(void *handle, unsigned char *out);
+int pion_gpu_get_hll_switch(void *handle, unsigned char *out);
+int pion_gpu_get_hll_screen_counts(void *handle, int *active, int *total);
 int pion_gpu_wind_orbit_position(const pion_gpu_wind_source *src, int ndim, double simtime, double *pos);
 int pion_gpu_add_rotating_wind_source(void *handle, const pion_gpu_wind_source *src, const double *evo_vcrit,
                                       double xi, int *id);
diff --git a/pion_amd/csrc/hll_screen.h b/pion_amd/csrc/hll_screen.h
--- /dev/null
+++ b/pion_amd/csrc/hll_screen.h
@@ -0,0 +1,112 @@
+#ifndef PION_HLL_SCREEN_H
+#define PION_HLL_SCREEN_H
+
+#if defined(__HIPCC__) || defined(__CUDACC__)
+#define PION_SCR_HD __host__ __device__ inline
+#else
+#define PION_SCR_HD inline
+#endif
+
+#define PION_SCR_BX 62
+#define PION_SCR_BY 4
+#define PION_SCR_BZ 8
+
+namespace pion {
+
+struct ScrGeom {
+  int ng[3];
+  int nbc[3];
+  int nb[3];
+  int per[3];
+};
+
+PION_SCR_HD int scr_bsize(const int d) { return (d == 0) ? PION_SCR_BX : ((d == 1) ? PION_SCR_BY : PION_SCR_BZ); }
+PION_SCR_HD int scr_nblocks(const int n, const int nbc, const int d)
+{
+  const int B = scr_bsize(d), r = n % B;
+  const int nb = (r == 0 || r >= nbc) ? (n + B - 1) / B : n / B;
+  return (nb < 1) ? 1 : nb;
+}
+PION_SCR_HD int scr_block_of(const int i, const int nb, const int d)
+{
+  const int b = i / scr_bsize(d);
+  return (b < nb) ? b : nb - 1;
+}
+PION_SCR_HD bool scr_axis_ok(const int n, const int nbc) { return n >= nbc && n >= 1; }
+PION_SCR_HD ScrGeom scr_geom(const int *ng, const int *nbc, const int *per)
+{
+  ScrGeom s;
+  for (int d = 0; d < 3; d++) {
+    s.ng[d] = ng[d];
+    s.nbc[d] = nbc[d];
+    s.nb[d] = scr_nblocks(ng[d], nbc[d], d);
+    s.per[d] = per[d];
+  }
+  return s;
+}
+PION_SCR_HD long scr_total(const ScrGeom &s) { return (long)s.nb[0] * s.nb[1] * s.nb[2]; }
+PION_SCR_HD long scr_index(const ScrGeom &s, const int bx, const int by, const int bz)
+{
+  return ((long)bz * s.nb[1] + by) * s.nb[0] + bx;
+}
+PION_SCR_HD void scr_cells(const ScrGeom &s, const int d, const int b, int *lo, int *hi)
+{
+  *lo = b * scr_bsize(d);
+  *hi = (b == s.nb[d] - 1) ? s.ng[d] : *lo + scr_bsize(d);
+}
+PION_SCR_HD void scr_cells_ext(const ScrGeom &s, const int d, const int b, int *lo, int *hi)
+{
+  scr_cells(s, d, b, lo, hi);
+  *lo += (b == 0) ? 0 : s.nbc[d];
+  *hi += (b == s.nb[d] - 1) ? 2 * s.nbc[d] : s.nbc[d];
+}
+PION_SCR_HD int scr_neighbour(const ScrGeom &s, const int d, const int b, const int o)
+{
+  int n = b + o;
+  if (n < 0) n = s.per[d] ? s.nb[d] - 1 : -1;
+  else if (n >= s.nb[d]) n = s.per[d] ? 0 : -1;
+  return n;
+}
+PION_SCR_HD bool scr_quiet(const double m, const double M) { return M - m <= 1.6 * m; }
+
+PION_SCR_HD unsigned long long scr_key(const double x)
+{
+  unsigned long long b;
+  __builtin_memcpy(&b, &x, 8);
+  return (b >> 63) ? ~b : (b | 0x8000000000000000ull);
+}
+PION_SCR_HD double scr_unkey(const unsigned long long k)
+{
+  const unsigned long long b = (k >> 63) ? (k & 0x7fffffffffffffffull) : ~k;
+  double x;
+  __builtin_memcpy(&x, &b, 8);
+  return x;
+}
+PION_SCR_HD bool scr_block_quiet(const ScrGeom &s, const unsigned long long *kmax, const unsigned long long *knmin,
+                                 const int bx, const int by, const int bz)
+{
+  unsigned long long kM = 0, kN = 0;
+  bool hole = false;
+  for (int oz = -1; oz <= 1; oz++) {
+    const int z = scr_neighbour(s, 2, bz, oz);
+    if (z < 0) continue;
+    for (int oy = -1; oy <= 1; oy++) {
+      const int y = scr_neighbour(s, 1, by, oy);
+      if (y < 0) continue;
+      for (int ox = -1; ox <= 1; ox++) {
+        const int x = scr_neighbour(s, 0, bx, ox);
+        if (x < 0) continue;
+        const long i = scr_index(s, x, y, z);
+        const unsigned long long a = kmax[i], b = knmin[i];
+        if (a == 0 || b == 0) hole = true;
+        kM = (a > kM) ? a : kM;
+        kN = (b > kN) ? b : kN;
+      }
+    }
+  }
+  if (hole) return false;
+  return scr_quiet(scr_unkey(~kN), scr_unkey(kM));
+}
+
+}
+#endif
diff --git a/pion_amd/csrc/kernels.h b/pion_amd/csrc/kernels.h
--- a/pion_amd/csrc/kernels.h
+++ b/pion_amd/csrc/kernels.h
@@ -6,6 +6,7 @@
 
 #include "dev_riemann.h"
 #include "rows_tiling.h"
+#include "hll_screen.h"
 
 namespace pion {
 
@@ -65,6 +66,9 @@
   int dt_mp;
   int plain_cells;
   CoolDev cool;
+  unsigned long long *hsum;
+  long hsum_n;
+  int hsum_nbx, hsum_nby, hsum_nbz;
 };
 
 struct PrepassArgs {
@@ -77,6 +81,9 @@
   double gamma;
   long c0, c1;
   long c2, c3;
+  const unsigned long long *hsum;
+  ScrGeom scr;
+  int *scr_list, *scr_count;
 };
 
 struct DtArgs {
diff --git a/pion_amd/csrc/kernels_fp.hip b/pion_amd/csrc/kernels_fp.hip
--- a/pion_amd/csrc/kernels_fp.hip
+++ b/pion_amd/csrc/kernels_fp.hip
@@ -686,6 +686,8 @@
 }
 const char *stage_kernel_name(int, int, int) { return "k_stage"; }
 
+PDEV void prepass_hlld_cell(const PrepassArgs &a, const int *i);
+
 __global__ __launch_bounds__(256) void k_prepass_hlld(const PrepassArgs a)
 {
   const long nc = a.g.ncell;
@@ -702,6 +704,12 @@
   const unsigned pz = t / (gx * gy);
   i[2] = (pz < npl1) ? (int)(a.c0 / plane) + (int)pz : (int)(a.c2 / plane) + (int)(pz - npl1);
   if (i[0] >= a.g.nga[0] || i[1] >= a.g.nga[1]) return;
+  prepass_hlld_cell(a, i);
+}
+
+PDEV void prepass_hlld_cell(const PrepassArgs &a, const int *i)
+{
+  const long nc = a.g.ncell;
   const long c = (long)i[0] + a.g.sy * i[1] + a.g.sz * i[2];
   const double dx = a.g.dx;
   double divv = 0.0, gradp = 0.0;
@@ -877,10 +885,47 @@
   }
 }
 
+__global__ __launch_bounds__(256) void k_prepass_screen(const PrepassArgs a)
+{
+  const long nblk = scr_total(a.scr);
+  const long t = (long)blockIdx.x * blockDim.x + threadIdx.x;
+  if (t >= nblk) return;
+  const int bx = (int)(t % a.scr.nb[0]), by = (int)((t / a.scr.nb[0]) % a.scr.nb[1]);
+  const int bz = (int)(t / ((long)a.scr.nb[0] * a.scr.nb[1]));
+  if (!scr_block_quiet(a.scr, a.hsum, a.hsum + nblk, bx, by, bz)) a.scr_list[atomicAdd(a.scr_count, 1)] = (int)t;
+}
+__global__ __launch_bounds__(256) void k_prepass_hlld_blocks(const PrepassArgs a)
+{
+  const int n = *a.scr_count;
+  for (int e = (int)blockIdx.x; e < n; e += (int)gridDim.x) {
+    const int t = a.scr_list[e];
+    const int bx = t % a.scr.nb[0], by = (t / a.scr.nb[0]) % a.scr.nb[1], bz = t / (a.scr.nb[0] * a.scr.nb[1]);
+    int lo[3], hi[3];
+    scr_cells_ext(a.scr, 0, bx, &lo[0], &hi[0]);
+    scr_cells_ext(a.scr, 1, by, &lo[1], &hi[1]);
+    scr_cells_ext(a.scr, 2, bz, &lo[2], &hi[2]);
+    const int ny = hi[1] - lo[1], nrow = ny * (hi[2] - lo[2]);
+    for (int r = (int)(threadIdx.x >> 6); r < nrow; r += 4) {
+      int i[3];
+      i[1] = lo[1] + r % ny;
+      i[2] = lo[2] + r / ny;
+      for (i[0] = lo[0] + (int)(threadIdx.x & 63); i[0] < hi[0]; i[0] += 64) prepass_hlld_cell(a, i);
+    }
+  }
+}
+
 int launch_prepass(const PrepassArgs &a, hipStream_t s)
 {
   const unsigned nb = (unsigned)((a.c1 - a.c0 + 255) / 256);
-  if (a.hllflag) {
+  if (a.hllflag && a.hsum) {
+    const long nblk = scr_total(a.scr);
+    if (hipMemsetAsync(a.hllflag, 0, (size_t)a.g.ncell, s) != hipSuccess) return -1;
+    if (hipMemsetAsync(a.scr_count, 0, sizeof(int), s) != hipSuccess) return -1;
+    hipLaunchKernelGGL(k_prepass_screen, dim3((unsigned)((nblk + 255) / 256)), dim3(256), 0, s, a);
+    const unsigned ngrid = (nblk < 4096) ? (unsigned)nblk : 4096u;
+    hipLaunchKernelGGL(k_prepass_hlld_blocks, dim3(ngrid), dim3(256), 0, s, a);
+  }
+  else if (a.hllflag) {
     const long plane = (long)a.g.nga[0] * a.g.nga[1];
     const unsigned npl = (unsigned)((a.c1 - a.c0) / plane) + ((a.c3 > a.c2) ? (unsigned)((a.c3 - a.c2) / plane) : 0u);
     const unsigned ntile = (unsigned)((a.g.nga[0] + 63) / 64) * ((a.g.nga[1] + 3) / 4) * npl;
diff --git a/pion_amd/csrc/pion_gpu.hip b/pion_amd/csrc/pion_gpu.hip
--- a/pion_amd/csrc/pion_gpu.hip
+++ b/pion_amd/csrc/pion_gpu.hip
@@ -450,7 +450,22 @@
   bool dt_mp_pending = false;
   bool split_dt_mp = true;
   bool fuse_bc = true;
+  bool hll_screen = true;
+  bool screen_ok = false;
+  ScrGeom scr;
+  unsigned long long *dsum = nullptr;
+  int *dscr_list = nullptr, *dscr_count = nullptr;
+  const double *sum_arr = nullptr;
+  bool sum_bc = false;
+  bool last_prepass_screened = false;
 };
+
+static inline void state_changed(Handle *h)
+{
+  h->dt_cached = false;
+  h->sum_arr = nullptr;
+  h->sum_bc = false;
+}
 
 #define HCHECK(h, call)                                                            \
   do {                                                                             \
@@ -846,7 +861,7 @@
   if (int rc = wind_add_cells_box(h, h->wsrc.back())) return rc;
   HCHECK(h, hipGetLastError());
   HCHECK(h, hipStreamSynchronize(h->stream));
-  h->dt_cached = false;
+  state_changed(h);
   if (id) *id = (int)h->wsrc.size() - 1;
   return 0;
 }
@@ -868,7 +883,7 @@
     }
     if (int rc = wind_add_cells_box(h, W)) return rc;
   }
-  if (moved) h->dt_cached = false;
+  if (moved) state_changed(h);
   return 0;
 }
 
@@ -1067,7 +1082,7 @@
   W.off = o;
   W.n = n;
   h->wsrc.push_back(W);
-  h->dt_cached = false;
+  state_changed(h);
   if (id) *id = (int)h->wsrc.size() - 1;
   return 0;
 }
@@ -1114,6 +1129,7 @@
   if (const char *e = getenv("PION_FUSE_DT")) h->fuse_dt = (atoi(e) != 0);
   if (const char *e = getenv("PION_FUSE_BC")) h->fuse_bc = (atoi(e) != 0);
   if (const char *e = getenv("PION_UNEVEN_CHUNKS")) h->uneven_chunks = (atoi(e) != 0);
+  if (const char *e = getenv("PION_HLL_SCREEN")) h->hll_screen = (atoi(e) != 0);
   if (const char *e = getenv("PION_SPLIT_DT_MP")) h->split_dt_mp = (atoi(e) != 0);
   if (const char *e = getenv("PION_ROWS")) h->rows = h->rows1 = (atoi(e) >= 1 && atoi(e) <= 64) ? atoi(e) : 0;
   if (const char *e = getenv("PION_ROWS1")) h->rows1 = (atoi(e) >= 1 && atoi(e) <= 8) ? atoi(e) : 0;
@@ -1292,6 +1308,9 @@
   }
   hipFree(h->dflags);
   hipFree(h->dhll);
+  hipFree(h->dsum);
+  hipFree(h->dscr_list);
+  hipFree(h->dscr_count);
   hipFree(h->ddE);
   if (h->bstream) hipStreamDestroy(h->bstream);
   if (h->ev_pre) hipEventDestroy(h->ev_pre);
@@ -1346,7 +1365,7 @@
   HCHECK(h, hipMemcpyAsync(h->dPh, h->dP, nb, hipMemcpyDeviceToDevice, h->stream));
   HCHECK(h, hipStreamSynchronize(h->stream));
   h->ph_valid = false;
-  h->dt_cached = false;
+  state_changed(h);
   h->dt_requested = false;
   h->dt_mp_pending = false;
   return 0;
@@ -1376,7 +1395,7 @@
   h->dP = (double *)dP;
   h->dPh = (double *)dPh;
   h->ph_valid = false;
-  h->dt_cached = false;
+  state_changed(h);
   h->dt_requested = false;
   return 0;
 }
@@ -1384,7 +1403,7 @@
 {
   Handle *h = use(handle);
   h->xghost_fresh = nullptr;
-  h->dt_cached = false;
+  state_changed(h);
   return which == 0 ? (void *)h->dP : (void *)h->dPh;
 }
 int pion_gpu_set_stream(void *handle, void *stream)
@@ -1411,7 +1430,7 @@
 int pion_gpu_set_wind_cells(void *handle, long n, const long *idx, const double *states)
 {
   Handle *h = use(handle);
-  h->dt_cached = false;
+  state_changed(h);
   hipFree(h->dwind_idx);
   hipFree(h->dwind_state);
   h->dwind_idx = nullptr;
@@ -1660,6 +1679,28 @@
   return 0;
 }
 
+int pion_gpu_get_hll_switch(void *handle, unsigned char *out)
+{
+  Handle *h = use(handle);
+  if (!h || !out || !h->dhll) return PION_GPU_EINVAL;
+  HCHECK(h, hipMemcpyAsync(out, h->dhll, h->g.ncell, hipMemcpyDeviceToHost, h->stream));
+  HCHECK(h, hipStreamSynchronize(h->stream));
+  return 0;
+}
+
+int pion_gpu_get_hll_screen_counts(void *handle, int *active, int *total)
+{
+  Handle *h = use(handle);
+  if (!h || !active || !total) return PION_GPU_EINVAL;
+  *active = -1;
+  *total = 0;
+  if (!h->last_prepass_screened) return 0;
+  HCHECK(h, hipMemcpyAsync(active, h->dscr_count, sizeof(int), hipMemcpyDeviceToHost, h->stream));
+  HCHECK(h, hipStreamSynchronize(h->stream));
+  *total = (int)scr_total(h->scr);
+  return 0;
+}
+
 int pion_gpu_wind_orbit_position(const pion_gpu_wind_source *src, int ndim, double simtime, double *pos)
 {
   if (!src || !pos || ndim < 2 || ndim > 3) return PION_GPU_EINVAL;
@@ -1696,7 +1737,7 @@
 int pion_gpu_set_jet(void *handle, int jetradius, const double *jetstate)
 {
   Handle *h = use(handle);
-  h->dt_cached = false;
+  state_changed(h);
   const pion_gpu_config &cfg = h->cfg;
   const GridDesc &g = h->g;
   const bool cart3d = (cfg.ndim == 3 && cfg.coord_sys == 1 && cfg.eqntype == PION_EQEUL);
@@ -1749,7 +1790,7 @@
 int pion_gpu_set_cooling_tables(void *handle, int nT, const double *T, const double *tabs, const double *slopes)
 {
   Handle *h = use(handle);
-  h->dt_cached = false;
+  state_changed(h);
   if (nT < 2 || nT > PION_COOL_NT_MAX) {
     h->err = "cooling tables: 2 <= nT <= 256 required";
     return PION_GPU_EINVAL;
@@ -1795,6 +1836,8 @@
   const GridDesc &g = h->g;
   const bool full = (cstep == maxstep);
   double *T = full ? h->dP : h->dPh;
+  if (h->sum_arr == T && h->nwind == 0 && h->nws == 0) h->sum_bc = true;
+  else if (h->sum_arr == T) h->sum_arr = nullptr;
   if (h->nws > 0 && h->have_angle) {
     if (int rc = wind_angle_check(h, simtime)) return rc;
   }
@@ -2045,6 +2088,35 @@
   return 0;
 }
 
+static bool screen_admitted(Handle *h)
+{
+  const pion_gpu_config &cfg = h->cfg;
+  if (!h->hll_screen || !h->dhll || cfg.ndim != 3 || h->g.cyl != 0 || h->use_march == 0 || h->g.nbc[2] < 2) return false;
+  if (any_wind(h) || h->njet > 0 || cfg.bc_dmach2) return false;
+  if (h->g.ncell * 8L >= (1L << 32)) return false;
+  int per[3];
+  for (int d = 0; d < 3; d++) {
+    for (int f = 2 * d; f < 2 * d + 2; f++) {
+      const int t = cfg.bc_type[f];
+      if (!(t == PION_BC_PERIODIC || t == PION_BC_OUTFLOW || t == PION_BC_ONEWAY_OUT || t == PION_BC_REFLECTING
+            || t == PION_BC_AXISYMMETRIC))
+        return false;
+    }
+    if ((cfg.bc_type[2 * d] == PION_BC_PERIODIC) != (cfg.bc_type[2 * d + 1] == PION_BC_PERIODIC)) return false;
+    per[d] = (cfg.bc_type[2 * d] == PION_BC_PERIODIC) ? 1 : 0;
+    if (!scr_axis_ok(h->g.ng[d], h->g.nbc[d])) return false;
+  }
+  h->scr = scr_geom(h->g.ng, h->g.nbc, per);
+  if (!h->dsum) {
+    const size_t n = (size_t)scr_total(h->scr);
+    if (hipMalloc(&h->dsum, 2 * n * sizeof(unsigned long long)) != hipSuccess) return false;
+    if (hipMalloc(&h->dscr_list, n * sizeof(int)) != hipSuccess) return false;
+    if (hipMalloc(&h->dscr_count, sizeof(int)) != hipSuccess) return false;
+    if (hipMemset(h->dscr_count, 0, sizeof(int)) != hipSuccess) return false;
+  }
+  return true;
+}
+
 static int stage_launch(Handle *h, double dt_stage, int space_ooa, int is_full_step, int kz0, int kz1,
                         bool first, bool last, int kz2 = 0, int kz3 = 0, hipStream_t ls = 0, bool use_ls = false)
 {
@@ -2071,6 +2143,16 @@
     p.c0 = 0;
     p.c1 = h->g.ncell;
     p.c2 = p.c3 = 0;
+    p.hsum = nullptr;
+    p.scr_list = p.scr_count = nullptr;
+    h->screen_ok = screen_admitted(h);
+    if (first && last && h->screen_ok && h->sum_arr == S && h->sum_bc) {
+      p.hsum = h->dsum;
+      p.scr = h->scr;
+      p.scr_list = h->dscr_list;
+      p.scr_count = h->dscr_count;
+    }
+    h->last_prepass_screened = (p.hsum != nullptr);
     if (!(first && last)) {
       const int nb = h->g.nbc[2], nz = h->g.ng[2];
       int lo = kz0 - 1, hi = kz1 + 1;
@@ -2172,6 +2254,22 @@
                        && ((h->g.ndim == 3 && h->g.nbc[2] >= 2) || h->g.ndim == 2) && a.out == h->dP;
   a.dtres = nullptr;
   a.cfl = cfg.cfl;
+  a.hsum = nullptr;
+  a.hsum_n = 0;
+  a.hsum_nbx = a.hsum_nby = a.hsum_nbz = 0;
+  h->sum_arr = nullptr;
+  h->sum_bc = false;
+  const bool leave_sum = first && last && h->dhll && h->screen_ok && a.plain_cells && a.rows >= 1 && cfg.cooling == 0
+                         && !h->deta && !a.fc.mp.present
+                         && PION_SCR_BY % a.rows == 0 && !(is_full_step && a.out == h->dPh);
+  if (leave_sum) {
+    a.hsum = h->dsum;
+    a.hsum_n = scr_total(h->scr);
+    a.hsum_nbx = h->scr.nb[0];
+    a.hsum_nby = h->scr.nb[1];
+    a.hsum_nbz = h->scr.nb[2];
+    HCHECK(h, hipMemsetAsync(h->dsum, 0, 2 * (size_t)a.hsum_n * sizeof(unsigned long long), ls));
+  }
   const bool split_mp = fuse_dt && mp_dt_limited(cfg) && h->split_dt_mp;
   a.dt_mp = (mp_dt_limited(cfg) && !split_mp) ? 1 : 0;
   h->dt_cached = false;
@@ -2203,6 +2301,7 @@
   }
   h->ph_valid = !is_full_step;
   h->dt_cached = fuse_dt;
+  if (leave_sum) h->sum_arr = a.out;
   h->xghost_fresh = a.xwrap ? ((is_full_step && a.out == h->dPh) ? h->dP : a.out) : nullptr;
   return 0;
 }
diff --git a/pion_amd/csrc/stage_helpers.h b/pion_amd/csrc/stage_helpers.h
--- a/pion_amd/csrc/stage_helpers.h
+++ b/pion_amd/csrc/stage_helpers.h
@@ -130,5 +130,14 @@
   }
   return v;
 }
+PDEV double wave_max64(double v)
+{
+#pragma unroll
+  for (int o = 32; o > 0; o >>= 1) {
+    const double w = __shfl_xor(v, o, 64);
+    v = (w > v) ? w : v;
+  }
+  return v;
+}
 
 #endif
diff --git a/pion_amd/csrc/stage_rows2.h b/pion_amd/csrc/stage_rows2.h
--- a/pion_amd/csrc/stage_rows2.h
+++ b/pion_amd/csrc/stage_rows2.h
@@ -192,6 +192,7 @@
   constexpr bool MHD = E::MHD;
   constexpr int NZ = ZSL ? 2 * NV : NV;
   constexpr bool PF = PION_ROWS2_PF && (OAMODE == 1);
+  constexpr bool SCR = MHD && SOLVER == FLUX_RS_HLLD && !CYL && PLAIN;
   extern __shared__ double lds[];
 
   const int R = a.rows;
@@ -229,6 +230,7 @@
     writer = (seg < tl.spw && jg < nyg && pos >= 1 && pos <= tl.rem);
     if (jg >= nyg) jg = nyg - 1;
   }
+  const int scr_bx = SCR ? __builtin_amdgcn_readfirstlane(ix + 1) / PION_SCR_BX : 0;
   if (ix > a.g.ng[0]) ix = a.g.ng[0];
   const int j0 = jg * R;
   const int nrows = (jg_first * R + R <= a.g.ng[1]) ? R : a.g.ng[1] - jg_first * R;
@@ -259,6 +261,8 @@
   if (PLAIN) fc.mp.present = 0;
   int err = 0;
   double tdyn = 1.e100, tmp = 1.0e99;
+  const bool scr_on = SCR && a.hsum != nullptr && (PION_SCR_BY % R) == 0;
+  double scr_m = __builtin_inf(), scr_M = -__builtin_inf();
 
   const int zbase = wave * R * NZ * 64 + lane;
 #define ZS2(r, s) lds[zbase + ((r) * NZ + (s)) * 64]
@@ -741,6 +745,13 @@
         }
 #pragma unroll
         for (int v = 0; v < NV; v++) stu(Ob + v * ncb, off, Pf[v]);
+        if constexpr (SCR) {
+          if (scr_on) {
+            const double p = Pf[qPG], pM = (p == p) ? p : __builtin_inf();
+            scr_m = (p < scr_m) ? p : scr_m;
+            scr_M = (pM > scr_M) ? pM : scr_M;
+          }
+        }
         if (a.xwrap) {
           const long xs = (long)a.g.ng[0] * 8;
           if (ix < a.g.nbc[0]) {
@@ -763,6 +774,22 @@
             tmp = (t < tmp) ? t : tmp;
           }
         }
+      }
+    }
+    if constexpr (SCR) {
+      if (scr_on && !prime && (((k + 1) % PION_SCR_BZ) == 0 || k == k1 - 1)) {
+        const long si = ((long)scr_block_of(k, a.hsum_nbz, 2) * a.hsum_nby + scr_block_of(j0, a.hsum_nby, 1)) * a.hsum_nbx
+                        + ((scr_bx < a.hsum_nbx) ? scr_bx : a.hsum_nbx - 1);
+        if (tt < tl.nfull) {
+          scr_m = wave_min64(scr_m);
+          scr_M = wave_max64(scr_M);
+        }
+        if ((tt < tl.nfull) ? (lane == 0) : writer) {
+          atomicMax(&a.hsum[si], scr_key(scr_M));
+          atomicMax(&a.hsum[a.hsum_n + si], ~scr_key(scr_m));
+        }
+        scr_m = __builtin_inf();
+        scr_M = -__builtin_inf();
       }
     }
   }
diff --git a/pion_amd/lib.py b/pion_amd/lib.py
--- a/pion_amd/lib.py
+++ b/pion_amd/lib.py
@@ -50,6 +50,9 @@
     lib.pion_gpu_get_wind_source_pos.argtypes = [C.c_void_p, C.c_int, _dp]
     lib.pion_gpu_wind_orbit_position.argtypes = [C.c_void_p, C.c_int, C.c_double, _dp]
     lib.pion_gpu_get_flags.argtypes = [C.c_void_p, C.c_void_p]
+    if hasattr(lib, "pion_gpu_get_hll_switch"):
+        lib.pion_gpu_get_hll_switch.argtypes = [C.c_void_p, C.c_void_p]
+        lib.pion_gpu_get_hll_screen_counts.argtypes = [C.c_void_p, C.POINTER(C.c_int), C.POINTER(C.c_int)]
     lib.pion_gpu_set_cooling_tables.argtypes = [C.c_void_p, C.c_int, _dp, _dp, _dp]
     lib.pion_gpu_update_bcs.argtypes = [C.c_void_p, C.c_double, C.c_int, C.c_int, C.c_int]
     lib.pion_gpu_calc_dt.argtypes = [C.c_void_p, _dp, _dp]
@@ -83,7 +86,7 @@
     "pion_gpu_get_timing", "pion_gpu_stage_part", "pion_gpu_set_comm_stream", "pion_gpu_set_jet",
     "pion_gpu_add_wind_source", "pion_gpu_get_wind_cells", "pion_gpu_get_wind_source_pos",
     "pion_gpu_wind_orbit_position", "pion_gpu_get_flags", "pion_gpu_add_rotating_wind_source",
-    "pion_gpu_wind_angle_tables",
+    "pion_gpu_wind_angle_tables", "pion_gpu_get_hll_switch", "pion_gpu_get_hll_screen_counts",
 ]
 
 
@@ -205,6 +208,16 @@
         self._chk(self.lib.pion_gpu_get_flags(self.h, out.ctypes.data), "get_flags")
         return out
 
+    def get_hll_switch(self):
+        out = np.zeros(self.ncell, dtype=np.uint8)
+        self._chk(self.lib.pion_gpu_get_hll_switch(self.h, out.ctypes.data), "get_hll_switch")
+        return out
+
+    def get_hll_screen_counts(self):
+        a, t = C.c_int(0), C.c_int(0)
+        self._chk(self.lib.pion_gpu_get_hll_screen_counts(self.h, C.byref(a), C.byref(t)), "get_hll_screen_counts")
+        return a.value, t.value
+
     def set_jet(self, jetradius, jetstate):
         st = np.ascontiguousarray(jetstate, dtype=np.float64)
         self._chk(self.lib.pion_gpu_set_jet(self.h, int(jetradius), _p(st)), "set_jet")
```

Result: faster. 6246 Mcell-updates/s, median of 6 (+1.9%).
